# kcoost/fast_speech_enhancement_metrics

Measured on NVIDIA B200. Metric: PESQ+STOI audio-seconds scored/sec, higher is better.
Workload: dtype f32

## Files before the change

### fast_speech_enhancement_metrics_b200/csrc/fsem_api.cu

```cuda
#include <atomic>
#include <cstdarg>
#include <cstdio>
#include <cstdlib>
#include <cstring>
#include <new>
#include <vector>

#include "fsem_common.cuh"
#include "fsem_pesq.cuh"
#include "fsem_stoi.cuh"
#include "fsem_lsd.cuh"
#include "fsem_sdr.cuh"
#include "fsem_sdr_tc.cuh"
#include "fsem_ingest.cuh"

using namespace fsem;

namespace {

thread_local char g_err[512] = "";
std::atomic<int64_t> g_launches{0};

int fail(int code, const char* fmt, ...) {
    va_list ap;
// ... 161 lines not shown

extern "C" int fsem_version(void) { return FSEM_VERSION; }
extern "C" const char* fsem_last_error(void) { return g_err; }
extern "C" int64_t fsem_launch_count(void) { return g_launches.load(std::memory_order_relaxed); }
extern "C" int fsem_profile_enable(int on) { g_profile = on != 0; return FSEM_OK; }
extern "C" int fsem_profile_reset(void) {
    prof_collect();
    for (int i = 0; i < K_COUNT; ++i) { g_prof_ms[i] = 0; g_prof_launches[i] = 0; }
    return FSEM_OK;
}
extern "C" int fsem_profile_read(int index, const char** name, double* total_ms, int64_t* launches) {
    if (index < 0 || index >= K_COUNT) return FSEM_E_INVALID;
    prof_collect();
    if (name) *name = kKernelNames[index];
    if (total_ms) *total_ms = g_prof_ms[index];
    if (launches) *launches = g_prof_launches[index];
    return FSEM_OK;
}

struct fsem_pesq_ctx {
    DeviceInfo dev;
    PesqFilterCoef coef;
    int warm = 640;
    PesqTables* d_tab = nullptr;
    int rs_orig = 1, rs_neu = 1, rs_width = 0, rs_ntaps = 0;
    float* d_rs_taps = nullptr;
    int spec_ctas_per_sm = 2;
    int filt_ctas_per_sm = 4;
    int64_t plan_batch_hint = 0;
    HostPipe pipe;
};

namespace {

struct PesqPlan {
    int64_t batch, n, zstride;
    int64_t n_in, rstride;
    bool resample;
    bool tiled;
    int tmax, tpitch, chunk, nchunks;
    size_t off_rs, off_rslen, off_z, off_partial, off_bark, off_dist, off_power, off_order, off_fprefix, total;
};

PesqPlan pesq_plan(const fsem_pesq_ctx* ctx, int64_t batch, int64_t n_in) {
    constexpr int quantum = 64;
    PesqPlan p{};
    p.batch = batch;
    p.n_in = n_in;
    p.resample = ctx->rs_orig != ctx->rs_neu;
    const int64_t n = stoi_resampled_len(n_in, ctx->rs_orig, ctx->rs_neu);
    p.rstride = round_up(n > 0 ? n : 1, 4);
    p.n = n;
    p.zstride = round_up((n > 0 ? n : 1) + FSEM_PESQ_HOP, 4);
    p.tmax = pesq_num_frames(n);
    if (p.tmax < 1) p.tmax = 1;
    p.tpitch = (int)round_up(p.tmax, 4);
    const int64_t nn = n > 0 ? n : 1;
    const int64_t plan_batch = ctx->plan_batch_hint > 0 ? ctx->plan_batch_hint : batch;
    const int64_t groups = 2 * ceil_div(plan_batch > 0 ? plan_batch : 1, 32);
    const int64_t slots = (int64_t)ctx->dev.sms * ctx->filt_ctas_per_sm * kFiltWarps;
    const int64_t max_ch = ceil_div(nn, 256) < 1024 ? ceil_div(nn, 256) : 1024;
    int64_t nch = 1, chunk = round_up(nn, quantum);
    double best = 1e300;
    p.tiled = plan_batch >= 16;
    if (!p.tiled) {
        chunk = round_up(ceil_div(nn, max_ch), 64);
        nch = ceil_div(nn, chunk);
    }
    for (int64_t c = 1; p.tiled && c <= max_ch; ++c) {
        const int64_t ch = round_up(ceil_div(nn, c), quantum);
        const int64_t cc = ceil_div(nn, ch);
        const int64_t waves = ceil_div(groups * cc, slots);
        const double cost = (double)waves * (double)(ch + (cc > 1 ? ctx->warm : 0));
        if (cost < best * 0.999) { best = cost; nch = cc; chunk = ch; }
    }
    p.chunk = (int)chunk;
    p.nchunks = (int)nch;
    size_t off = 0;
    p.off_rs = off;      off = align256(off + (p.resample ? sizeof(float) * 2 * batch * p.rstride : 0));
    p.off_rslen = off;   off = align256(off + (p.resample ? sizeof(int32_t) * batch : 0));
    p.off_z = off;       off = align256(off + sizeof(float) * 2 * batch * p.zstride);
    p.off_bark = off;    off = align256(off + sizeof(float) * 2 * batch * p.tpitch * kBarkRow);
    p.off_dist = off;    off = align256(off + sizeof(float) * 2 * batch * p.tpitch);
    p.off_power = off;   off = align256(off + sizeof(double) * 2 * batch);
    p.off_order = off;   off = align256(off + sizeof(int32_t) * batch);
    p.off_fprefix = off; off = align256(off + sizeof(int64_t) * (batch + 1));
    p.off_partial = off; off = align256(off + sizeof(double) * 2 * batch * p.nchunks);
    p.total = off;
    return p;
}

}

extern "C" int fsem_pesq_create(fsem_pesq_ctx_t** out, const fsem_pesq_design_t* d) {
    if (!out || !d) return fail(FSEM_E_INVALID, "fsem_pesq_create: null argument");
    *out = nullptr;
    fsem_pesq_ctx* ctx = new (std::nothrow) fsem_pesq_ctx();
    if (!ctx) return fail(FSEM_E_INVALID, "out of host memory");
    int rc = query_device(ctx->dev);
    if (rc != FSEM_OK) { delete ctx; return rc; }
    ctx->coef.k = d->bp_direct;
    for (int s = 0; s < FSEM_BP_SECTIONS; ++s) {
        ctx->coef.c0[s] = d->bp_c0[s]; ctx->coef.c1[s] = d->bp_c1[s];
        ctx->coef.a1[s] = d->bp_a1[s]; ctx->coef.a2[s] = d->bp_a2[s];
    }
    ctx->coef.pb0 = d->pre_b[0]; ctx->coef.pb1 = d->pre_b[1]; ctx->coef.pb2 = d->pre_b[2];
    ctx->coef.pa1 = d->pre_a[0]; ctx->coef.pa2 = d->pre_a[1];
    ctx->warm = (int)round_up(d->warmup > 0 ? d->warmup : 640, 32);
    for (int k = 0; k < 15; ++k) {
        if (fabsf(d->taper[k] - (float)(k + 1) * 0.0625f) > 1e-7f) {
            delete ctx;
            return fail(FSEM_E_INVALID, "fsem_pesq_create: taper must be k/16 (PESQ.py:90)");
        }
    }
    PesqTables h{};
    memcpy(h.hann, d->hann, sizeof(h.hann));
    double wtot = 0.0;
    for (int b = 0; b < FSEM_PESQ_NBANDS; ++b) {
        h.band_first[b] = d->band_first_bin[b];
        h.band_count[b] = d->band_num_bins[b];
        const int expect_first = b == 0 ? 0 : h.band_first[b - 1] + h.band_count[b - 1];
        if (h.band_first[b] != expect_first || h.band_count[b] < 1 || h.band_count[b] > 32 ||
            h.band_first[b] + h.band_count[b] > 256) {
            delete ctx;
            return fail(FSEM_E_INVALID, "fsem_pesq_create: Bark bands must tile bins 0..255 contiguously, at most 32 bins each (band %d)", b);
        }
        {
            const int span = ((h.band_first[b] + h.band_count[b] - 1) >> 3) - (h.band_first[b] >> 3);
            if (span > (b < 32 ? kBarkPiecesLow : kBarkPiecesHigh)) {
                delete ctx;
                return fail(FSEM_E_INVALID, "fsem_pesq_create: Bark band %d spans %d groups of 8 bins (unsupported layout)", b, span + 1);
            }
        }
        h.pow_dens[b] = d->pow_dens[b];
        h.thresh[b] = d->thresh[b];
        h.zw_exp[b] = d->zwicker_exp[b];
        h.width[b] = d->width_bark[b];
        h.loud_scale[b] = (float)((double)d->sl * pow(2.0 * (double)d->thresh[b], (double)d->zwicker_exp[b]));
        if (b >= 1) wtot += (double)d->width_bark[b];
    }
    h.width_total = (float)wtot;
    cudaError_t e = cudaMalloc(&ctx->d_tab, sizeof(PesqTables));
    if (e == cudaSuccess) e = cudaMemcpy(ctx->d_tab, &h, sizeof(h), cudaMemcpyHostToDevice);
    if (e != cudaSuccess) {
        if (ctx->d_tab) cudaFree(ctx->d_tab);
        delete ctx;
        return fail(FSEM_E_CUDA, "fsem_pesq_create: %s", cudaGetErrorString(e));
    }
    if (e == cudaSuccess && d->rs_orig != d->rs_neu) {
        if (d->rs_orig <= 0 || d->rs_neu <= 0 || !d->rs_taps || d->rs_ntaps != 2 * d->rs_width + d->rs_orig) {
            cudaFree(ctx->d_tab);
            delete ctx;
            return fail(FSEM_E_INVALID, "fsem_pesq_create: bad resampling kernel (ntaps must be 2*width+orig)");
        }
        ctx->rs_orig = d->rs_orig; ctx->rs_neu = d->rs_neu; ctx->rs_width = d->rs_width; ctx->rs_ntaps = d->rs_ntaps;
        e = cudaMalloc(&ctx->d_rs_taps, sizeof(float) * d->rs_neu * d->rs_ntaps);
        if (e == cudaSuccess)
            e = cudaMemcpy(ctx->d_rs_taps, d->rs_taps, sizeof(float) * d->rs_neu * d->rs_ntaps, cudaMemcpyHostToDevice);
        if (e != cudaSuccess) {
            cudaFree(ctx->d_tab);
            if (ctx->d_rs_taps) cudaFree(ctx->d_rs_taps);
            delete ctx;
            return fail(FSEM_E_CUDA, "fsem_pesq_create: %s", cudaGetErrorString(e));
        }
    }
    e = cudaFuncSetAttribute(pesq_spectrum_kernel, cudaFuncAttributeMaxDynamicSharedMemorySize, (int)kSpecDynSmem);
    if (e == cudaSuccess)
        e = cudaFuncSetAttribute(pesq_bark_kernel<kBarkThreadsWide, kBarkTileWide>,
                                 cudaFuncAttributeMaxDynamicSharedMemorySize, (int)bark_dyn_smem(kBarkTileWide));
    if (e == cudaSuccess && bark_dyn_smem(kBarkTile) > 0)
        e = cudaFuncSetAttribute(pesq_bark_kernel<kBarkThreads, kBarkTile>,
                                 cudaFuncAttributeMaxDynamicSharedMemorySize, (int)bark_dyn_smem(kBarkTile));
    if (e != cudaSuccess) {
        cudaFree(ctx->d_tab);
        if (ctx->d_rs_taps) cudaFree(ctx->d_rs_taps);
        delete ctx;
        return fail(FSEM_E_CUDA, "fsem_pesq_create: %s", cudaGetErrorString(e));
    }
    int occ = 0;
    if (cudaOccupancyMaxActiveBlocksPerMultiprocessor(&occ, pesq_spectrum_kernel, kSpecWarps * 32, kSpecDynSmem) == cudaSuccess && occ > 0)
        ctx->spec_ctas_per_sm = occ;
    occ = 0;
    if (cudaOccupancyMaxActiveBlocksPerMultiprocessor(&occ, pesq_filter_tiled_kernel<false, float>, kFiltWarps * 32, 0) == cudaSuccess && occ > 0)
        ctx->filt_ctas_per_sm = occ;
    *out = ctx;
    return FSEM_OK;
}

extern "C" int fsem_pesq_destroy(fsem_pesq_ctx_t* ctx) {
    if (!ctx) return FSEM_OK;
    ctx->pipe.destroy();
    if (ctx->d_tab) cudaFree(ctx->d_tab);
    if (ctx->d_rs_taps) cudaFree(ctx->d_rs_taps);
    delete ctx;
    return FSEM_OK;
}

extern "C" size_t fsem_pesq_workspace_bytes(const fsem_pesq_ctx_t* ctx, int64_t batch, int64_t n) {
    if (!ctx || batch <= 0 || n <= 0) return 0;
    return pesq_plan(ctx, batch, n).total;
}

extern "C" int fsem_pesq_score_f32(fsem_pesq_ctx_t* ctx, const fsem_batch_t* in, float* mos_out,
                                   int32_t* status_out, void* workspace, size_t workspace_bytes,
                                   void* stream_v) {
    return fsem_pesq_score(ctx, in, FSEM_DTYPE_F32, mos_out, status_out, workspace, workspace_bytes, stream_v);
}

extern "C" int fsem_pesq_score(fsem_pesq_ctx_t* ctx, const fsem_batch_t* in, int dtype, float* mos_out,
                               int32_t* status_out, void* workspace, size_t workspace_bytes, void* stream_v) {
    if (!ctx || !in || !mos_out) return fail(FSEM_E_INVALID, "fsem_pesq_score_f32: null argument");
    const size_t es = dtype_size(dtype);
    if (es == 0) return fail(FSEM_E_INVALID, "fsem_pesq_score: unknown dtype %d", dtype);
    if (in->batch < 0 || in->n < 0 || in->stride < in->n)
        return fail(FSEM_E_INVALID, "fsem_pesq_score_f32: bad shape batch=%lld n=%lld stride=%lld",
                    (long long)in->batch, (long long)in->n, (long long)in->stride);
    if (in->batch == 0) return FSEM_OK;
    if (!in->clean || !in->deg) return fail(FSEM_E_INVALID, "fsem_pesq_score_f32: null input");
    if (in->n >= (int64_t(1) << 30)) return fail(FSEM_E_INVALID, "fsem_pesq_score_f32: n too large");
    const PesqPlan p = pesq_plan(ctx, in->batch, in->n);
    if (!in->lengths && pesq_num_frames(p.n) < 20)
        return fail(FSEM_E_TOO_SHORT, "PESQ needs at least 20 frames of 512/256 samples at 16 kHz; n=%lld gives %d",
                    (long long)in->n, pesq_num_frames(p.n));
    if (!workspace || workspace_bytes < p.total)
        return fail(FSEM_E_WORKSPACE, "fsem_pesq_score_f32: workspace %zu < %zu bytes", workspace_bytes, p.total);
    cudaStream_t stream = static_cast<cudaStream_t>(stream_v);
    char* ws = static_cast<char*>(workspace);
    float* z = reinterpret_cast<float*>(ws + p.off_z);
    double* partial = reinterpret_cast<double*>(ws + p.off_partial);
    float* bark = reinterpret_cast<float*>(ws + p.off_bark);
    float* dist = reinterpret_cast<float*>(ws + p.off_dist);
    double* power = reinterpret_cast<double*>(ws + p.off_power);

    fsem_batch_t rs_batch;
    if (p.resample) {
        float* y = reinterpret_cast<float*>(ws + p.off_rs);
        int32_t* rslen = reinterpret_cast<int32_t*>(ws + p.off_rslen);
        const int64_t bps = ceil_div(p.n, 256);
        if (bps * 2 * in->batch >= (int64_t(1) << 31))
            return fail(FSEM_E_INVALID, "fsem_pesq_score_f32: batch x samples too large for one launch; split the batch");
        { ProfScope prof_(K_PESQ_RESAMPLE, stream);
          dispatch_dtype(dtype, [&](auto tag) {
              using T = decltype(tag);
              stoi_resample_kernel<T><<<(unsigned)(bps * 2 * in->batch), 256, 0, stream>>>(
                  reinterpret_cast<const T*>(in->clean), reinterpret_cast<const T*>(in->deg), in->lengths, in->batch, in->n,
                  in->stride, ctx->d_rs_taps, ctx->rs_orig, ctx->rs_neu, ctx->rs_width, ctx->rs_ntaps, y, p.rstride, (int)bps);
              return FSEM_OK;
          }); }
        FSEM_LAUNCHED();
        if (in->lengths) {
            resampled_lengths_kernel<<<(unsigned)ceil_div(in->batch, 256), 256, 0, stream>>>(
                in->lengths, in->batch, in->n, ctx->rs_orig, ctx->rs_neu, rslen);
            FSEM_LAUNCHED();
        }
        rs_batch = fsem_batch_t{y, y + in->batch * p.rstride, in->lengths ? rslen : nullptr, in->batch, p.n, p.rstride};
        in = &rs_batch;
        dtype = FSEM_DTYPE_F32;
    }

    int32_t* order = nullptr;
    int64_t* fprefix = nullptr;
    if (in->lengths) {
        order = reinterpret_cast<int32_t*>(ws + p.off_order);
        fprefix = reinterpret_cast<int64_t*>(ws + p.off_fprefix);
        pesq_order_kernel<<<1, kOrderThreads, 0, stream>>>(in->lengths, in->batch, in->n, order, fprefix);
        FSEM_LAUNCHED();
    }
    {
        const bool vec4 = rows_vec4(in->clean, in->deg, in->stride, dtype_size(dtype));
        ProfScope prof_(K_PESQ_FILTER, stream);
        dispatch_dtype(dtype, [&](auto tag) {
            using T = decltype(tag);
            const T* c = reinterpret_cast<const T*>(in->clean);
            const T* d = reinterpret_cast<const T*>(in->deg);
            if (vec4 && p.tiled) {
                const int64_t units = 2 * ceil_div(in->batch, 32) * p.nchunks;
                const unsigned grid = (unsigned)ceil_div(units, kFiltWarps);
                if (in->lengths)
                    pesq_filter_tiled_kernel<true, T><<<grid, kFiltWarps * 32, 0, stream>>>(
                        c, d, in->lengths, order, in->batch, in->n, in->stride, p.chunk, p.nchunks, ctx->warm, ctx->coef, z,
                        p.zstride, partial);
                else
                    pesq_filter_tiled_kernel<false, T><<<grid, kFiltWarps * 32, 0, stream>>>(
                        c, d, nullptr, nullptr, in->batch, in->n, in->stride, p.chunk, p.nchunks, ctx->warm, ctx->coef, z,
                        p.zstride, partial);
            } else {
                const int64_t threads = 2 * in->batch * p.nchunks;
                const unsigned grid = (unsigned)ceil_div(threads, 128);
                if (vec4)
                    pesq_filter_kernel<true, T><<<grid, 128, 0, stream>>>(
                        c, d, in->lengths, in->batch, in->n, in->stride, p.chunk, p.nchunks, ctx->warm, ctx->coef, z,
                        p.zstride, partial);
                else
                    pesq_filter_kernel<false, T><<<grid, 128, 0, stream>>>(
                        c, d, in->lengths, in->batch, in->n, in->stride, p.chunk, p.nchunks, ctx->warm, ctx->coef, z,
                        p.zstride, partial);
            }
            return FSEM_OK;
        });
    }
    FSEM_LAUNCHED();
    {
        const int64_t units = in->batch * (int64_t)p.tmax;
        int64_t grid = ceil_div(units, kSpecWarps);
        const int64_t cap = (int64_t)ctx->dev.sms * ctx->spec_ctas_per_sm;
        if (grid > cap) grid = cap;
        { ProfScope prof_(K_PESQ_SPECTRUM, stream);
          pesq_spectrum_kernel<<<(unsigned)grid, kSpecWarps * 32, kSpecDynSmem, stream>>>(
              z, p.zstride, in->lengths, fprefix, in->batch, in->n, p.tmax, p.tpitch, partial, p.nchunks, ctx->d_tab, bark); }
        FSEM_LAUNCHED();
    }
    {
        { ProfScope prof_(K_PESQ_BARK, stream);
          if (in->batch <= ctx->dev.sms)
              pesq_bark_kernel<kBarkThreadsWide, kBarkTileWide>
                  <<<(unsigned)in->batch, kBarkThreadsWide, bark_dyn_smem(kBarkTileWide), stream>>>(
                      bark, partial, p.nchunks, in->lengths, order, in->batch, in->n, p.tpitch, ctx->d_tab, dist, mos_out,
                      status_out, power);
          else
              pesq_bark_kernel<kBarkThreads, kBarkTile>
                  <<<(unsigned)in->batch, kBarkThreads, bark_dyn_smem(kBarkTile), stream>>>(
                      bark, partial, p.nchunks, in->lengths, order, in->batch, in->n, p.tpitch, ctx->d_tab, dist, mos_out,
                      status_out, power); }
        FSEM_LAUNCHED();
    }
    return FSEM_OK;
}

extern "C" int fsem_pesq_debug_taps(fsem_pesq_ctx_t* ctx, int64_t batch, int64_t n, const void* workspace,
                                    float* bark_out, double* power_out, int64_t* frames_out, void* stream_v) {
    if (!ctx || !workspace) return fail(FSEM_E_INVALID, "fsem_pesq_debug_taps: null argument");
    const PesqPlan p = pesq_plan(ctx, batch, n);
    cudaStream_t stream = static_cast<cudaStream_t>(stream_v);
    const char* ws = static_cast<const char*>(workspace);
    if (frames_out) *frames_out = p.tmax;
    if (bark_out)
        for (int64_t r = 0; r < 2 * batch; ++r)
            FSEM_CUDA(cudaMemcpy2DAsync(bark_out + r * p.tmax * FSEM_PESQ_NBANDS, sizeof(float) * FSEM_PESQ_NBANDS,
                                        ws + p.off_bark + sizeof(float) * r * p.tpitch * kBarkRow, sizeof(float) * kBarkRow,
                                        sizeof(float) * FSEM_PESQ_NBANDS, (size_t)p.tmax, cudaMemcpyDeviceToDevice, stream));
    if (power_out)
        FSEM_CUDA(cudaMemcpyAsync(power_out, ws + p.off_power, sizeof(double) * 2 * batch, cudaMemcpyDeviceToDevice,
                                  stream));
    return FSEM_OK;
}

struct fsem_stoi_ctx {
    DeviceInfo dev;
    int orig = 1, neu = 1, width = 0, ntaps = 0;
    float* d_taps = nullptr;
    bool fast85 = false;
    Resample85Taps taps85;
    StoiTables* d_tab = nullptr;
    float clip = 0.f, dyn_range = 40.f;
    int tob_ctas_per_sm = 2;
    HostPipe pipe;
};

namespace {

struct StoiPlan {
    int64_t batch, n, lmax, ystride;
    int t0max, mask_words, umax, ustride, mmax, ntiles, hops_max;
    bool resample, fused_energy;
    size_t off_hops, off_y, off_energy, off_idx, off_count, off_prefix, off_mask, off_tob, off_partial, total;
};

StoiPlan stoi_plan(const fsem_stoi_ctx* ctx, int64_t batch, int64_t n) {
    StoiPlan p{};
    p.batch = batch;
    p.n = n;
    p.resample = ctx->orig != ctx->neu;
    p.lmax = stoi_resampled_len(n, ctx->orig, ctx->neu);
    p.ystride = round_up(p.lmax > 0 ? p.lmax : 1, 4);
    p.t0max = stoi_num_frames(p.lmax);
    if (p.t0max < 1) p.t0max = 1;
    p.mask_words = (int)ceil_div(p.t0max, 32);
    p.umax = p.t0max - 2 > 0 ? p.t0max - 2 : 0;
    p.ustride = (int)round_up(p.umax > 0 ? p.umax : 1, 4);
    p.mmax = p.t0max - 31 > 0 ? p.t0max - 31 : 0;
    p.ntiles = (int)ceil_div(p.mmax > 0 ? p.mmax : 1, kSegTile);
    p.fused_energy = ctx->fast85;
    p.hops_max = (int)(ceil_div(p.lmax > 0 ? p.lmax : 1, kRs85TileOut) * kRs85Hops);
    size_t off = 0;
    p.off_hops = off;    off = align256(off + (p.fused_energy ? sizeof(double2) * batch * p.hops_max : 0));
    p.off_y = off;       off = align256(off + sizeof(float) * 2 * batch * p.ystride);
    p.off_energy = off;  off = align256(off + sizeof(float) * batch * p.t0max);
    p.off_idx = off;     off = align256(off + sizeof(int32_t) * batch * p.t0max);
    p.off_count = off;   off = align256(off + sizeof(int32_t) * batch);
    p.off_prefix = off;  off = align256(off + sizeof(int32_t) * (batch + 1));
    p.off_mask = off;    off = align256(off + sizeof(uint32_t) * batch * p.mask_words);
    p.off_tob = off;     off = align256(off + sizeof(float) * 2 * batch * FSEM_STOI_NBANDS * p.ustride);
    p.off_partial = off; off = align256(off + sizeof(float2) * batch * p.ntiles);
    p.total = off;
    return p;
}

}

extern "C" int fsem_stoi_create(fsem_stoi_ctx_t** out, const fsem_stoi_design_t* d) {
    if (!out || !d) return fail(FSEM_E_INVALID, "fsem_stoi_create: null argument");
    *out = nullptr;
    if (d->orig <= 0 || d->neu <= 0) return fail(FSEM_E_INVALID, "fsem_stoi_create: bad rates");
    if (d->orig != d->neu && (!d->taps || d->ntaps != 2 * d->width + d->orig || d->width < 0))
        return fail(FSEM_E_INVALID, "fsem_stoi_create: bad resampling kernel (ntaps must be 2*width+orig)");
    for (int b = 0; b < FSEM_STOI_NBANDS; ++b)
        if (d->band_lo[b] < 0 || d->band_hi[b] < d->band_lo[b] || d->band_hi[b] > 256)
            return fail(FSEM_E_INVALID, "fsem_stoi_create: band %d outside bins 0..255", b);
    if (d->band_hi[FSEM_STOI_NBANDS - 1] - d->band_lo[FSEM_STOI_NBANDS - 1] > 48)
        return fail(FSEM_E_INVALID, "fsem_stoi_create: third-octave bands must be at most 48 bins wide");
    for (int b = 0; b + 1 < FSEM_STOI_NBANDS; ++b)
        if (d->band_hi[b] != d->band_lo[b + 1] || d->band_hi[b] - d->band_lo[b] > 48)
            return fail(FSEM_E_INVALID, "fsem_stoi_create: third-octave bands must be contiguous and at most 48 bins wide");
    fsem_stoi_ctx* ctx = new (std::nothrow) fsem_stoi_ctx();
    if (!ctx) return fail(FSEM_E_INVALID, "out of host memory");
    int rc = query_device(ctx->dev);
    if (rc != FSEM_OK) { delete ctx; return rc; }
    ctx->orig = d->orig; ctx->neu = d->neu; ctx->width = d->width; ctx->ntaps = d->ntaps;
    ctx->clip = d->clip; ctx->dyn_range = d->dyn_range;
    StoiTables h{};
    memcpy(h.window, d->window, sizeof(h.window));
    for (int b = 0; b < FSEM_STOI_NBANDS; ++b) { h.band_lo[b] = d->band_lo[b]; h.band_hi[b] = d->band_hi[b]; }
    h.clip = d->clip; h.dyn_range = d->dyn_range;
    cudaError_t e = cudaMalloc(&ctx->d_tab, sizeof(StoiTables));
    if (e == cudaSuccess) e = cudaMemcpy(ctx->d_tab, &h, sizeof(h), cudaMemcpyHostToDevice);
    if (e == cudaSuccess && d->orig != d->neu) {
        e = cudaMalloc(&ctx->d_taps, sizeof(float) * d->neu * d->ntaps);
        if (e == cudaSuccess)
            e = cudaMemcpy(ctx->d_taps, d->taps, sizeof(float) * d->neu * d->ntaps, cudaMemcpyHostToDevice);
    }
    if (e != cudaSuccess) {
        if (ctx->d_tab) cudaFree(ctx->d_tab);
        if (ctx->d_taps) cudaFree(ctx->d_taps);
        delete ctx;
        return fail(FSEM_E_CUDA, "fsem_stoi_create: %s", cudaGetErrorString(e));
    }
    if (d->orig == 8 && d->neu == 5 && d->width == 10 && d->ntaps == 28) {
        ctx->fast85 = true;
        for (int p = 0; p < 5; ++p)
            for (int j = 0; j < 28; ++j) {
                ctx->taps85.h[p][j] = d->taps[p * 28 + j];
                if ((j < rs85_lo(p) || j > rs85_hi(p)) && d->taps[p * 28 + j] != 0.f) ctx->fast85 = false;
            }
    }
    int occ = 0;
    if (cudaOccupancyMaxActiveBlocksPerMultiprocessor(&occ, stoi_tob_kernel<true>, kTobWarps * 32, 0) == cudaSuccess && occ > 0)
        ctx->tob_ctas_per_sm = occ;
    *out = ctx;
    return FSEM_OK;
}

extern "C" int fsem_stoi_destroy(fsem_stoi_ctx_t* ctx) {
    if (!ctx) return FSEM_OK;
    ctx->pipe.destroy();
    if (ctx->d_tab) cudaFree(ctx->d_tab);
    if (ctx->d_taps) cudaFree(ctx->d_taps);
    delete ctx;
    return FSEM_OK;
}

extern "C" size_t fsem_stoi_workspace_bytes(const fsem_stoi_ctx_t* ctx, int64_t batch, int64_t n) {
    if (!ctx || batch <= 0 || n <= 0) return 0;
    return stoi_plan(ctx, batch, n).total;
}

extern "C" int fsem_stoi_score_f32(fsem_stoi_ctx_t* ctx, const fsem_batch_t* in, float* stoi_out,
                                   float* estoi_out, int32_t* kept_frames_out, int32_t* status_out,
                                   void* workspace, size_t workspace_bytes, void* stream_v) {
    return fsem_stoi_score(ctx, in, FSEM_DTYPE_F32, stoi_out, estoi_out, kept_frames_out, status_out, workspace,
                           workspace_bytes, stream_v);
}

extern "C" int fsem_stoi_score(fsem_stoi_ctx_t* ctx, const fsem_batch_t* in, int dtype, float* stoi_out,
                               float* estoi_out, int32_t* kept_frames_out, int32_t* status_out,
                               void* workspace, size_t workspace_bytes, void* stream_v) {
    if (!ctx || !in || !stoi_out || !estoi_out) return fail(FSEM_E_INVALID, "fsem_stoi_score_f32: null argument");
    if (dtype_size(dtype) == 0) return fail(FSEM_E_INVALID, "fsem_stoi_score: unknown dtype %d", dtype);
    if (in->batch < 0 || in->n < 0 || in->stride < in->n)
        return fail(FSEM_E_INVALID, "fsem_stoi_score_f32: bad shape batch=%lld n=%lld stride=%lld",
                    (long long)in->batch, (long long)in->n, (long long)in->stride);
    if (in->batch == 0) return FSEM_OK;
    if (in->n == 0) return fail(FSEM_E_INVALID, "fsem_stoi_score_f32: n = 0 (empty signals)");
    if (!in->clean || !in->deg) return fail(FSEM_E_INVALID, "fsem_stoi_score_f32: null input");
    if (in->n >= (int64_t(1) << 30)) return fail(FSEM_E_INVALID, "fsem_stoi_score_f32: n too large");
    const StoiPlan p = stoi_plan(ctx, in->batch, in->n);
    if (in->batch * (int64_t)p.t0max >= (int64_t(1) << 31))
        return fail(FSEM_E_INVALID, "fsem_stoi_score_f32: batch x frames exceeds 2^31; split the batch");
    if (!workspace || workspace_bytes < p.total)
        return fail(FSEM_E_WORKSPACE, "fsem_stoi_score_f32: workspace %zu < %zu bytes", workspace_bytes, p.total);
    cudaStream_t stream = static_cast<cudaStream_t>(stream_v);
    char* ws = static_cast<char*>(workspace);
    float* y = reinterpret_cast<float*>(ws + p.off_y);
    double2* hops = reinterpret_cast<double2*>(ws + p.off_hops);
    float* energy = reinterpret_cast<float*>(ws + p.off_energy);
    int32_t* kept_idx = reinterpret_cast<int32_t*>(ws + p.off_idx);
    int32_t* kept_count = reinterpret_cast<int32_t*>(ws + p.off_count);
    int32_t* frame_prefix = reinterpret_cast<int32_t*>(ws + p.off_prefix);
    uint32_t* mask = reinterpret_cast<uint32_t*>(ws + p.off_mask);
    float* tob = reinterpret_cast<float*>(ws + p.off_tob);
    float2* partial = reinterpret_cast<float2*>(ws + p.off_partial);

    const float* c10 = in->clean;
    const float* d10 = in->deg;
    int64_t sstride = in->stride;
    if (p.resample) {
        const bool vec4 = rows_vec4(in->clean, in->deg, in->stride, dtype_size(dtype));
        if (ctx->fast85) {
            const int64_t bps = ceil_div(p.lmax, (int64_t)kRs85TileOut * kRs85TilesPerCta);
            const unsigned grid = (unsigned)(bps * 2 * in->batch);
            { ProfScope prof_(K_STOI_RESAMPLE, stream);
              dispatch_dtype(dtype, [&](auto tag) {
                  using T = decltype(tag);
                  const T* c = reinterpret_cast<const T*>(in->clean);
                  const T* d = reinterpret_cast<const T*>(in->deg);
                  if (vec4)
                      stoi_resample85_kernel<true, T><<<grid, kRs85Threads, 0, stream>>>(
                          c, d, in->lengths, in->batch, in->n, in->stride, ctx->taps85, ctx->d_tab, y, p.ystride, hops,
                          p.hops_max, (int)bps);
                  else
                      stoi_resample85_kernel<false, T><<<grid, kRs85Threads, 0, stream>>>(
                          c, d, in->lengths, in->batch, in->n, in->stride, ctx->taps85, ctx->d_tab, y, p.ystride, hops,
                          p.hops_max, (int)bps);
                  return FSEM_OK;
              }); }
        } else {
            const int64_t bps = ceil_div(p.lmax, 256);
            if (bps * 2 * in->batch >= (int64_t(1) << 31))
                return fail(FSEM_E_INVALID, "fsem_stoi_score_f32: batch x samples too large for one launch; split the batch");
            { ProfScope prof_(K_STOI_RESAMPLE, stream);
              dispatch_dtype(dtype, [&](auto tag) {
                  using T = decltype(tag);
                  stoi_resample_kernel<T><<<(unsigned)(bps * 2 * in->batch), 256, 0, stream>>>(
                      reinterpret_cast<const T*>(in->clean), reinterpret_cast<const T*>(in->deg), in->lengths, in->batch,
                      in->n, in->stride, ctx->d_taps, ctx->orig, ctx->neu, ctx->width, ctx->ntaps, y, p.ystride, (int)bps);
                  return FSEM_OK;
              }); }
        }
        FSEM_LAUNCHED();
        c10 = y;
        d10 = y + in->batch * p.ystride;
        sstride = p.ystride;
    } else if (dtype != FSEM_DTYPE_F32) {
        int rc = launch_ingest(in->clean, dtype, in->batch, in->n, in->stride, y, p.ystride, stream);
        if (rc == FSEM_OK)
            rc = launch_ingest(in->deg, dtype, in->batch, in->n, in->stride, y + in->batch * p.ystride, p.ystride, stream);
        if (rc != FSEM_OK) return rc;
        c10 = y;
        d10 = y + in->batch * p.ystride;
        sstride = p.ystride;
    }
    if (p.fused_energy) {
        const int64_t threads = in->batch * (int64_t)p.t0max;
        { ProfScope prof_(K_STOI_ENERGY, stream);
          stoi_energy_from_hops_kernel<<<(unsigned)ceil_div(threads, 256), 256, 0, stream>>>(
              hops, p.hops_max, in->lengths, in->batch, in->n, p.t0max, energy); }
        FSEM_LAUNCHED();
    } else {
        const int64_t warps = in->batch * (int64_t)p.t0max;
        { ProfScope prof_(K_STOI_ENERGY, stream);
          stoi_energy_kernel<<<(unsigned)ceil_div(warps * 32, 256), 256, 0, stream>>>(
            c10, sstride, in->lengths, in->batch, in->n, ctx->orig, ctx->neu, p.t0max, ctx->d_tab, energy); }
        FSEM_LAUNCHED();
    }
    {
        { ProfScope prof_(K_STOI_COMPACT, stream);
          stoi_compact_kernel<<<(unsigned)ceil_div(in->batch * 32, 128), 128, 0, stream>>>(
              energy, in->lengths, in->batch, in->n, ctx->orig, ctx->neu, p.t0max, p.mask_words, ctx->dyn_range,
              kept_idx, kept_count, mask); }
        FSEM_LAUNCHED();
    }
    if (p.umax > 0) {
        { ProfScope prof_(K_STOI_COMPACT, stream);
          stoi_prefix_kernel<<<1, 1024, 0, stream>>>(kept_count, in->batch, frame_prefix); }
        FSEM_LAUNCHED();
        const int64_t units = in->batch * (int64_t)p.umax;
        int64_t grid = ceil_div(units, kTobWarps);
        const int64_t cap = (int64_t)ctx->dev.sms * ctx->tob_ctas_per_sm;
        if (grid > cap) grid = cap;
        const bool vec2 = (reinterpret_cast<uintptr_t>(c10) & 7u) == 0 && (reinterpret_cast<uintptr_t>(d10) & 7u) == 0 &&
                          sstride % 2 == 0;
        { ProfScope prof_(K_STOI_TOB, stream);
          if (vec2)
              stoi_tob_kernel<true><<<(unsigned)grid, kTobWarps * 32, 0, stream>>>(
                  c10, d10, sstride, in->batch, p.t0max, p.umax, p.ustride, kept_idx, frame_prefix, ctx->d_tab, tob);
          else
              stoi_tob_kernel<false><<<(unsigned)grid, kTobWarps * 32, 0, stream>>>(
                  c10, d10, sstride, in->batch, p.t0max, p.umax, p.ustride, kept_idx, frame_prefix, ctx->d_tab, tob); }
        FSEM_LAUNCHED();
    }
    {
        { ProfScope prof_(K_STOI_SEGMENT, stream);
          stoi_segment_kernel<<<(unsigned)(in->batch * ceil_div(p.ntiles, kSegTilesPerCta)), kSegThreads, 0, stream>>>(
              tob, in->batch, p.ustride, p.ntiles, kept_count, ctx->clip, partial); }
        FSEM_LAUNCHED();
        { ProfScope prof_(K_STOI_FINALIZE, stream);
          stoi_finalize_kernel<<<(unsigned)ceil_div(in->batch, 128), 128, 0, stream>>>(
              partial, in->batch, p.ntiles, kept_count, stoi_out, estoi_out, kept_frames_out, status_out); }
        FSEM_LAUNCHED();
    }
    return FSEM_OK;
}

extern "C" int fsem_stoi_debug_taps(fsem_stoi_ctx_t* ctx, int64_t batch, int64_t n, const void* workspace,
                                    uint32_t* mask_out, float* tob_out, float* resampled_out, int64_t* dims_out,
                                    void* stream_v) {
    if (!ctx || !workspace) return fail(FSEM_E_INVALID, "fsem_stoi_debug_taps: null argument");
    const StoiPlan p = stoi_plan(ctx, batch, n);
    cudaStream_t stream = static_cast<cudaStream_t>(stream_v);
    const char* ws = static_cast<const char*>(workspace);
    if (dims_out) {
        dims_out[0] = p.mask_words;
        dims_out[1] = p.ustride;
        dims_out[2] = p.resample ? p.ystride : 0;
    }
    if (mask_out)
        FSEM_CUDA(cudaMemcpyAsync(mask_out, ws + p.off_mask, sizeof(uint32_t) * batch * p.mask_words,
                                  cudaMemcpyDeviceToDevice, stream));
    if (tob_out)
        FSEM_CUDA(cudaMemcpyAsync(tob_out, ws + p.off_tob, sizeof(float) * 2 * batch * FSEM_STOI_NBANDS * p.ustride,
                                  cudaMemcpyDeviceToDevice, stream));
    if (resampled_out && p.resample)
        FSEM_CUDA(cudaMemcpyAsync(resampled_out, ws + p.off_y, sizeof(float) * 2 * batch * p.ystride,
                                  cudaMemcpyDeviceToDevice, stream));
    return FSEM_OK;
}

extern "C" int fsem_stoi_mask_margin(fsem_stoi_ctx_t* ctx, int64_t batch, int64_t n, const int32_t* lengths,
                                     const void* workspace, float* margin_out, void* stream_v) {
    if (!ctx || !workspace || !margin_out) return fail(FSEM_E_INVALID, "fsem_stoi_mask_margin: null argument");
    if (batch <= 0 || n <= 0) return fail(FSEM_E_INVALID, "fsem_stoi_mask_margin: bad shape");
    const StoiPlan p = stoi_plan(ctx, batch, n);
    cudaStream_t stream = static_cast<cudaStream_t>(stream_v);
    const float* energy = reinterpret_cast<const float*>(static_cast<const char*>(workspace) + p.off_energy);
    { ProfScope prof_(K_STOI_MARGIN, stream);
      stoi_margin_kernel<<<(unsigned)ceil_div(batch * 32, 128), 128, 0, stream>>>(
          energy, lengths, batch, n, ctx->orig, ctx->neu, p.t0max, ctx->dyn_range, margin_out); }
    FSEM_LAUNCHED();
    return FSEM_OK;
}

namespace {

int launch_ingest(const void* src, int dtype, int64_t rows, int64_t n, int64_t sstride, float* dst, int64_t dstride,
                  cudaStream_t stream) {
    if (rows <= 0 || n <= 0) return FSEM_OK;
    if (dtype == FSEM_DTYPE_F32) {
        FSEM_CUDA(cudaMemcpy2DAsync(dst, dstride * sizeof(float), src, sstride * sizeof(float), n * sizeof(float), rows,
                                    cudaMemcpyDeviceToDevice, stream));
        return FSEM_OK;
    }
    const bool vec = aligned16(src) && aligned16(dst) && sstride % 8 == 0 && dstride % 4 == 0;
    const int64_t groups = rows * ceil_div(n, 8);
    int64_t grid = ceil_div(groups, 256);
    if (grid > (1 << 20)) grid = 1 << 20;
    { ProfScope prof_(K_INGEST, stream);
      if (dtype == FSEM_DTYPE_I16) {
          const int16_t* s = static_cast<const int16_t*>(src);
          if (vec) ingest_kernel<int16_t, true><<<(unsigned)grid, 256, 0, stream>>>(s, sstride, dst, dstride, rows, n);
          else ingest_kernel<int16_t, false><<<(unsigned)grid, 256, 0, stream>>>(s, sstride, dst, dstride, rows, n);
      } else {
          const __half* s = static_cast<const __half*>(src);
          if (vec) ingest_kernel<__half, true><<<(unsigned)grid, 256, 0, stream>>>(s, sstride, dst, dstride, rows, n);
          else ingest_kernel<__half, false><<<(unsigned)grid, 256, 0, stream>>>(s, sstride, dst, dstride, rows, n);
      } }
    FSEM_LAUNCHED();
    return FSEM_OK;
}

int score_host_any(const char* who, fsem_pesq_ctx* pctx, fsem_stoi_ctx* sctx, const void* clean, const void* deg,
                   int dtype, const int32_t* lengths, int64_t batch, int64_t n, int64_t stride, float* mos_out,
                   int32_t* pesq_status_out, float* stoi_out, float* estoi_out, int32_t* kept_frames_out,
                   int32_t* stoi_status_out) {
    if ((!pctx && !sctx) || !clean || !deg || (pctx && !mos_out) || (sctx && (!stoi_out || !estoi_out)))
        return fail(FSEM_E_INVALID, "%s: null argument", who);
    const size_t es = dtype_size(dtype);
    if (es == 0) return fail(FSEM_E_INVALID, "%s: unknown dtype %d", who, dtype);
    if (batch < 0 || n < 0 || stride < n) return fail(FSEM_E_INVALID, "%s: bad shape", who);
    if (batch == 0) return FSEM_OK;
    if (pctx && !lengths && pesq_num_frames(pesq_plan(pctx, 1, n).n) < 20)
        return fail(FSEM_E_TOO_SHORT, "PESQ needs at least 20 frames of 512/256 samples at 16 kHz; n=%lld is too short",
                    (long long)n);
    HostPipe& P = pctx ? pctx->pipe : sctx->pipe;
    int rc = P.init();
    if (rc != FSEM_OK) return rc;
    const int64_t rstride = round_up(n, 16 / (int64_t)es);
    const int64_t per = host_chunk_items(batch, n, es);
    const size_t raw_sig = align256(es * per * rstride);
    const size_t in_bytes = 2 * raw_sig + align256(sizeof(int32_t) * per);
    const size_t conv_sig = 0;
    const size_t ws_pesq = pctx ? align256(fsem_pesq_workspace_bytes(pctx, per, n)) : 0;
    const size_t ws_stoi = sctx ? align256(fsem_stoi_workspace_bytes(sctx, per, n)) : 0;
    const size_t col = align256(sizeof(float) * batch);
    rc = P.reserve(in_bytes, 2 * conv_sig + ws_pesq + ws_stoi, 6 * col);
    if (rc != FSEM_OK) return rc;
    char* const ob = static_cast<char*>(P.out);
    char* const wsb = static_cast<char*>(P.ws);
    const char* h_clean = static_cast<const char*>(clean);
    const char* h_deg = static_cast<const char*>(deg);
    auto upload = [&](void* dst, const char* src, int64_t cnt) -> cudaError_t {
        if (stride == n && rstride == n)
            return cudaMemcpyAsync(dst, src, es * n * cnt, cudaMemcpyHostToDevice, P.copy);
        return cudaMemcpy2DAsync(dst, rstride * es, src, stride * es, n * es, cnt, cudaMemcpyHostToDevice, P.copy);
    };
    auto run = [&]() -> int {
    int64_t done_chunks = 0;
    for (int64_t i0 = 0; i0 < batch; i0 += per, ++done_chunks) {
        const int slot = (int)(done_chunks & 1);
        const int64_t cnt = (batch - i0 < per) ? (batch - i0) : per;
        char* base = static_cast<char*>(P.in[slot]);
        int32_t* d_len = reinterpret_cast<int32_t*>(base + 2 * raw_sig);
        if (done_chunks >= 2) FSEM_CUDA(cudaStreamWaitEvent(P.copy, P.done[slot], 0));
        FSEM_CUDA(upload(base, h_clean + (size_t)i0 * stride * es, cnt));
        FSEM_CUDA(upload(base + raw_sig, h_deg + (size_t)i0 * stride * es, cnt));
        if (lengths)
            FSEM_CUDA(cudaMemcpyAsync(d_len, lengths + i0, sizeof(int32_t) * cnt, cudaMemcpyHostToDevice, P.copy));
        FSEM_CUDA(cudaEventRecord(P.copied[slot], P.copy));
        FSEM_CUDA(cudaStreamWaitEvent(P.compute, P.copied[slot], 0));
        fsem_batch_t dev{reinterpret_cast<const float*>(base), reinterpret_cast<const float*>(base + raw_sig),
                         lengths ? d_len : nullptr, cnt, n, rstride};
        if (rc == FSEM_OK && pctx && sctx)
            rc = fsem_pesq_stoi_score(pctx, sctx, &dev, dtype, reinterpret_cast<float*>(ob) + i0,
                                          reinterpret_cast<int32_t*>(ob + col) + i0,
                                          reinterpret_cast<float*>(ob + 2 * col) + i0,
                                          reinterpret_cast<float*>(ob + 3 * col) + i0,
                                          reinterpret_cast<int32_t*>(ob + 4 * col) + i0,
                                          reinterpret_cast<int32_t*>(ob + 5 * col) + i0, wsb + 2 * conv_sig, ws_pesq,
                                          wsb + 2 * conv_sig + ws_pesq, ws_stoi, P.compute);
        else if (rc == FSEM_OK && pctx)
            rc = fsem_pesq_score(pctx, &dev, dtype, reinterpret_cast<float*>(ob) + i0,
                                 reinterpret_cast<int32_t*>(ob + col) + i0, wsb + 2 * conv_sig, ws_pesq, P.compute);
        else if (rc == FSEM_OK && sctx)
            rc = fsem_stoi_score(sctx, &dev, dtype, reinterpret_cast<float*>(ob + 2 * col) + i0,
                                     reinterpret_cast<float*>(ob + 3 * col) + i0,
                                     reinterpret_cast<int32_t*>(ob + 4 * col) + i0,
                                     reinterpret_cast<int32_t*>(ob + 5 * col) + i0, wsb + 2 * conv_sig + ws_pesq, ws_stoi,
                                     P.compute);
        if (rc != FSEM_OK) return rc;
        FSEM_CUDA(cudaEventRecord(P.done[slot], P.compute));
    }
    const size_t nb = sizeof(float) * batch;
    auto readback = [&](void* dst, size_t column) -> cudaError_t {
        return dst ? cudaMemcpyAsync(dst, ob + column * col, nb, cudaMemcpyDeviceToHost, P.compute) : cudaSuccess;
    };
    if (pctx) {
        FSEM_CUDA(readback(mos_out, 0));
        FSEM_CUDA(readback(pesq_status_out, 1));
    }
    if (sctx) {
        FSEM_CUDA(readback(stoi_out, 2));
        FSEM_CUDA(readback(estoi_out, 3));
        FSEM_CUDA(readback(kept_frames_out, 4));
        FSEM_CUDA(readback(stoi_status_out, 5));
    }
    return FSEM_OK;
    };
    rc = run();
    const cudaError_t e_copy = cudaStreamSynchronize(P.copy);
    const cudaError_t e_comp = cudaStreamSynchronize(P.compute);
    if (rc != FSEM_OK) return rc;
    if (e_copy != cudaSuccess || e_comp != cudaSuccess)
        return fail(FSEM_E_CUDA, "%s: %s", who, cudaGetErrorString(e_copy != cudaSuccess ? e_copy : e_comp));
    return FSEM_OK;
}

}

extern "C" int fsem_ingest_f32(const void* src, int dtype, int64_t rows, int64_t n, int64_t src_stride, float* dst,
                               int64_t dst_stride, void* stream) {
    if (!src || !dst) return fail(FSEM_E_INVALID, "fsem_ingest_f32: null argument");
    if (dtype_size(dtype) == 0) return fail(FSEM_E_INVALID, "fsem_ingest_f32: unknown dtype %d", dtype);
    if (rows < 0 || n < 0 || src_stride < n || dst_stride < n) return fail(FSEM_E_INVALID, "fsem_ingest_f32: bad shape");
    return launch_ingest(src, dtype, rows, n, src_stride, dst, dst_stride, static_cast<cudaStream_t>(stream));
}

extern "C" int fsem_score_host(fsem_pesq_ctx_t* pesq, fsem_stoi_ctx_t* stoi, const void* clean, const void* deg, int dtype,
                               const int32_t* lengths, int64_t batch, int64_t n, int64_t stride, float* mos_out,
                               int32_t* pesq_status_out, float* stoi_out, float* estoi_out, int32_t* kept_frames_out,
                               int32_t* stoi_status_out) {
    return score_host_any("fsem_score_host", pesq, stoi, clean, deg, dtype, lengths, batch, n, stride, mos_out,
                          pesq_status_out, stoi_out, estoi_out, kept_frames_out, stoi_status_out);
}

extern "C" int fsem_pesq_score_host_f32(fsem_pesq_ctx_t* ctx, const fsem_batch_t* in, float* mos_out,
                                        int32_t* status_out) {
    if (!ctx || !in) return fail(FSEM_E_INVALID, "fsem_pesq_score_host_f32: null argument");
    return score_host_any("fsem_pesq_score_host_f32", ctx, nullptr, in->clean, in->deg, FSEM_DTYPE_F32, in->lengths,
                          in->batch, in->n, in->stride, mos_out, status_out, nullptr, nullptr, nullptr, nullptr);
}

extern "C" int fsem_stoi_score_host_f32(fsem_stoi_ctx_t* ctx, const fsem_batch_t* in, float* stoi_out,
                                        float* estoi_out, int32_t* kept_frames_out, int32_t* status_out) {
    if (!ctx || !in) return fail(FSEM_E_INVALID, "fsem_stoi_score_host_f32: null argument");
    return score_host_any("fsem_stoi_score_host_f32", nullptr, ctx, in->clean, in->deg, FSEM_DTYPE_F32, in->lengths,
                          in->batch, in->n, in->stride, nullptr, nullptr, stoi_out, estoi_out, kept_frames_out,
                          status_out);
}

extern "C" int fsem_pesq_stoi_score_host_f32(fsem_pesq_ctx_t* pctx, fsem_stoi_ctx_t* sctx, const fsem_batch_t* in,
                                             float* mos_out, int32_t* pesq_status_out, float* stoi_out,
                                             float* estoi_out, int32_t* kept_frames_out, int32_t* stoi_status_out) {
    if (!pctx || !sctx || !in) return fail(FSEM_E_INVALID, "fsem_pesq_stoi_score_host_f32: null argument");
    return score_host_any("fsem_pesq_stoi_score_host_f32", pctx, sctx, in->clean, in->deg, FSEM_DTYPE_F32, in->lengths,
                          in->batch, in->n, in->stride, mos_out, pesq_status_out, stoi_out, estoi_out, kept_frames_out,
                          stoi_status_out);
}

struct fsem_resampler {
    int orig = 1, neu = 1, width = 0, ntaps = 0;
    float* d_taps = nullptr;
};

extern "C" int fsem_resampler_create(fsem_resampler_t** out, int32_t orig, int32_t neu, int32_t width, int32_t ntaps,
                                     const float* taps) {
    if (!out) return fail(FSEM_E_INVALID, "fsem_resampler_create: null argument");
    *out = nullptr;
    if (orig <= 0 || neu <= 0 || width < 0 || !taps || ntaps != 2 * width + orig)
        return fail(FSEM_E_INVALID, "fsem_resampler_create: bad resampling kernel (ntaps must be 2*width+orig)");
    fsem_resampler* r = new (std::nothrow) fsem_resampler();
    if (!r) return fail(FSEM_E_INVALID, "out of host memory");
    r->orig = orig; r->neu = neu; r->width = width; r->ntaps = ntaps;
    cudaError_t e = cudaMalloc(&r->d_taps, sizeof(float) * neu * ntaps);
    if (e == cudaSuccess) e = cudaMemcpy(r->d_taps, taps, sizeof(float) * neu * ntaps, cudaMemcpyHostToDevice);
    if (e != cudaSuccess) {
        if (r->d_taps) cudaFree(r->d_taps);
        delete r;
        return fail(FSEM_E_CUDA, "fsem_resampler_create: %s", cudaGetErrorString(e));
    }
    *out = r;
    return FSEM_OK;
}

extern "C" int fsem_resampler_destroy(fsem_resampler_t* r) {
    if (!r) return FSEM_OK;
    if (r->d_taps) cudaFree(r->d_taps);
    delete r;
    return FSEM_OK;
}

extern "C" int64_t fsem_resampled_len(const fsem_resampler_t* r, int64_t n) {
    if (!r || n < 0) return 0;
    return stoi_resampled_len(n, r->orig, r->neu);
}

extern "C" int fsem_resample_f32(fsem_resampler_t* r, const fsem_batch_t* in, float* out, int64_t out_stride,
                                 int32_t* lengths_out, void* stream_v) {
    if (!r || !in || !out) return fail(FSEM_E_INVALID, "fsem_resample_f32: null argument");
    if (in->batch < 0 || in->n <= 0 || in->stride < in->n || in->n >= (int64_t(1) << 30))
        return fail(FSEM_E_INVALID, "fsem_resample_f32: bad shape");
    if (in->batch == 0) return FSEM_OK;
    if (!in->clean || !in->deg) return fail(FSEM_E_INVALID, "fsem_resample_f32: null input");
    const int64_t L = stoi_resampled_len(in->n, r->orig, r->neu);
    if (out_stride < L) return fail(FSEM_E_INVALID, "fsem_resample_f32: out_stride %lld < resampled length %lld",
                                    (long long)out_stride, (long long)L);
    if (in->lengths && !lengths_out) return fail(FSEM_E_INVALID, "fsem_resample_f32: lengths given but lengths_out is null");
    cudaStream_t stream = static_cast<cudaStream_t>(stream_v);
    const int64_t bps = ceil_div(L, 256);
    if (bps * 2 * in->batch >= (int64_t(1) << 31))
        return fail(FSEM_E_INVALID, "fsem_resample_f32: batch x samples too large for one launch; split the batch");
    { ProfScope prof_(K_PESQ_RESAMPLE, stream);
      stoi_resample_kernel<<<(unsigned)(bps * 2 * in->batch), 256, 0, stream>>>(
          in->clean, in->deg, in->lengths, in->batch, in->n, in->stride, r->d_taps, r->orig, r->neu, r->width,
          r->ntaps, out, out_stride, (int)bps); }
    FSEM_LAUNCHED();
    if (in->lengths) {
        resampled_lengths_kernel<<<(unsigned)ceil_div(in->batch, 256), 256, 0, stream>>>(
            in->lengths, in->batch, in->n, r->orig, r->neu, lengths_out);
        FSEM_LAUNCHED();
    }
    return FSEM_OK;
}

struct fsem_lsd_ctx {
    DeviceInfo dev;
    float* d_hann = nullptr;
    int ctas_per_sm = 2;
};

namespace {
struct LsdPlan { int tmax; size_t off_alpha, off_frames, total; };
LsdPlan lsd_plan(int64_t batch, int64_t n) {
    LsdPlan p{};
    p.tmax = lsd_num_frames(n);
    size_t off = 0;
    p.off_alpha = off;  off = align256(off + sizeof(float) * batch);
    p.off_frames = off; off = align256(off + sizeof(float) * batch * p.tmax);
    p.total = off;
    return p;
}
}

extern "C" int fsem_lsd_create(fsem_lsd_ctx_t** out, const float* hann512) {
    if (!out || !hann512) return fail(FSEM_E_INVALID, "fsem_lsd_create: null argument");
    *out = nullptr;
    fsem_lsd_ctx* ctx = new (std::nothrow) fsem_lsd_ctx();
    if (!ctx) return fail(FSEM_E_INVALID, "out of host memory");
    int rc = query_device(ctx->dev);
    if (rc != FSEM_OK) { delete ctx; return rc; }
    cudaError_t e = cudaMalloc(&ctx->d_hann, sizeof(float) * 512);
    if (e == cudaSuccess) e = cudaMemcpy(ctx->d_hann, hann512, sizeof(float) * 512, cudaMemcpyHostToDevice);
    if (e != cudaSuccess) {
        if (ctx->d_hann) cudaFree(ctx->d_hann);
        delete ctx;
        return fail(FSEM_E_CUDA, "fsem_lsd_create: %s", cudaGetErrorString(e));
    }
    int occ = 0;
    if (cudaOccupancyMaxActiveBlocksPerMultiprocessor(&occ, lsd_frames_kernel<true>, kLsdWarps * 32, 0) == cudaSuccess && occ > 0)
        ctx->ctas_per_sm = occ;
    *out = ctx;
    return FSEM_OK;
}

extern "C" int fsem_lsd_destroy(fsem_lsd_ctx_t* ctx) {
    if (!ctx) return FSEM_OK;
    if (ctx->d_hann) cudaFree(ctx->d_hann);
    delete ctx;
    return FSEM_OK;
}

extern "C" size_t fsem_lsd_workspace_bytes(const fsem_lsd_ctx_t* ctx, int64_t batch, int64_t n) {
    if (!ctx || batch <= 0 || n <= 0) return 0;
    return lsd_plan(batch, n).total;
}

extern "C" int fsem_lsd_score_f32(fsem_lsd_ctx_t* ctx, const fsem_batch_t* in, float* lsd_out, void* workspace,
                                  size_t workspace_bytes, void* stream_v) {
    if (!ctx || !in || !lsd_out) return fail(FSEM_E_INVALID, "fsem_lsd_score_f32: null argument");
    if (in->batch < 0 || in->n <= 0 || in->stride < in->n || in->n >= (int64_t(1) << 30))
        return fail(FSEM_E_INVALID, "fsem_lsd_score_f32: bad shape");
    if (in->batch == 0) return FSEM_OK;
    if (!in->clean || !in->deg) return fail(FSEM_E_INVALID, "fsem_lsd_score_f32: null input");
    const LsdPlan p = lsd_plan(in->batch, in->n);
    if (!workspace || workspace_bytes < p.total)
        return fail(FSEM_E_WORKSPACE, "fsem_lsd_score_f32: workspace %zu < %zu bytes", workspace_bytes, p.total);
    cudaStream_t stream = static_cast<cudaStream_t>(stream_v);
    char* ws = static_cast<char*>(workspace);
    float* alpha = reinterpret_cast<float*>(ws + p.off_alpha);
    float* frames = reinterpret_cast<float*>(ws + p.off_frames);
    lsd_scale_kernel<<<(unsigned)in->batch, 256, 0, stream>>>(in->clean, in->deg, in->lengths, in->batch, in->n,
                                                             in->stride, alpha);
    FSEM_LAUNCHED();
    const int64_t units = in->batch * (int64_t)p.tmax;
    int64_t grid = ceil_div(units, kLsdWarps);
    const int64_t cap = (int64_t)ctx->dev.sms * ctx->ctas_per_sm;
    if (grid > cap) grid = cap;
    const bool vec2 = (reinterpret_cast<uintptr_t>(in->clean) & 7u) == 0 && (reinterpret_cast<uintptr_t>(in->deg) & 7u) == 0 &&
                      in->stride % 2 == 0;
    { ProfScope prof_(K_LSD_FRAMES, stream);
      if (vec2)
          lsd_frames_kernel<true><<<(unsigned)grid, kLsdWarps * 32, 0, stream>>>(
              in->clean, in->deg, in->lengths, in->batch, in->n, in->stride, p.tmax, ctx->d_hann, alpha, frames);
      else
          lsd_frames_kernel<false><<<(unsigned)grid, kLsdWarps * 32, 0, stream>>>(
              in->clean, in->deg, in->lengths, in->batch, in->n, in->stride, p.tmax, ctx->d_hann, alpha, frames); }
    FSEM_LAUNCHED();
    lsd_finalize_kernel<<<(unsigned)ceil_div(in->batch, 128), 128, 0, stream>>>(frames, in->lengths, in->batch, in->n,
                                                                               p.tmax, lsd_out);
    FSEM_LAUNCHED();
    return FSEM_OK;
}

extern "C" int fsem_pesq_stoi_score(fsem_pesq_ctx_t* pctx, fsem_stoi_ctx_t* sctx, const fsem_batch_t* in, int dtype,
                                    float* mos_out, int32_t* pesq_status_out, float* stoi_out, float* estoi_out,
                                    int32_t* kept_frames_out, int32_t* stoi_status_out, void* ws_pesq,
                                    size_t ws_pesq_bytes, void* ws_stoi, size_t ws_stoi_bytes, void* stream) {
    if (!pctx || !sctx) return fail(FSEM_E_INVALID, "fsem_pesq_stoi_score: null context");
    int rc = fsem_pesq_score(pctx, in, dtype, mos_out, pesq_status_out, ws_pesq, ws_pesq_bytes, stream);
    if (rc == FSEM_OK)
        rc = fsem_stoi_score(sctx, in, dtype, stoi_out, estoi_out, kept_frames_out, stoi_status_out, ws_stoi,
                             ws_stoi_bytes, stream);
    return rc;
}

extern "C" int fsem_pesq_stoi_score_f32(fsem_pesq_ctx_t* pctx, fsem_stoi_ctx_t* sctx, const fsem_batch_t* in,
                                        float* mos_out, int32_t* pesq_status_out, float* stoi_out, float* estoi_out,
                                        int32_t* kept_frames_out, int32_t* stoi_status_out, void* ws_pesq,
                                        size_t ws_pesq_bytes, void* ws_stoi, size_t ws_stoi_bytes, void* stream) {
    return fsem_pesq_stoi_score(pctx, sctx, in, FSEM_DTYPE_F32, mos_out, pesq_status_out, stoi_out, estoi_out,
                                kept_frames_out, stoi_status_out, ws_pesq, ws_pesq_bytes, ws_stoi, ws_stoi_bytes, stream);
}

struct fsem_graph {
    cudaGraph_t graph = nullptr;
    cudaGraphExec_t exec = nullptr;
    void* ws = nullptr;
    int kernel_nodes = 0;
    int slices = 0;
    int device = -1;
};

namespace {
void graph_free(fsem_graph* g) {
    if (!g) return;
    if (g->exec) cudaGraphExecDestroy(g->exec);
    if (g->graph) cudaGraphDestroy(g->graph);
    if (g->ws) cudaFree(g->ws);
    delete g;
}
constexpr int kGraphMaxSlices = 16;
}

extern "C" int fsem_graph_create(fsem_graph_t** out, fsem_pesq_ctx_t* pctx, fsem_stoi_ctx_t* sctx, const fsem_batch_t* in,
                                 int dtype, float* mos_out, int32_t* pesq_status_out, float* stoi_out, float* estoi_out,
                                 int32_t* kept_frames_out, int32_t* stoi_status_out, int slices) {
    if (!out) return fail(FSEM_E_INVALID, "fsem_graph_create: null output");
    *out = nullptr;
    if (!pctx && !sctx) return fail(FSEM_E_INVALID, "fsem_graph_create: no metric selected");
    if (!in || in->batch <= 0) return fail(FSEM_E_INVALID, "fsem_graph_create: empty batch");
    if ((pctx && !mos_out) || (sctx && (!stoi_out || !estoi_out)))
        return fail(FSEM_E_INVALID, "fsem_graph_create: null output column");
    const size_t es = dtype_size(dtype);
    if (es == 0) return fail(FSEM_E_INVALID, "fsem_graph_create: unknown dtype %d", dtype);
    if (slices <= 0) slices = 1;
    if (slices > kGraphMaxSlices) slices = kGraphMaxSlices;
    if (slices > in->batch) slices = (int)in->batch;
    fsem_graph* g = new (std::nothrow) fsem_graph();
    if (!g) return fail(FSEM_E_INVALID, "fsem_graph_create: out of host memory");
    g->slices = slices;
    int64_t b0[kGraphMaxSlices + 1];
    for (int s = 0; s <= slices; ++s) b0[s] = in->batch * s / slices;
    if (pctx) pctx->plan_batch_hint = in->batch;
    size_t ws_off[2 * kGraphMaxSlices + 1];
    ws_off[0] = 0;
    for (int s = 0; s < slices; ++s) {
        const int64_t nb = b0[s + 1] - b0[s];
        ws_off[2 * s + 1] = ws_off[2 * s] + (pctx ? align256(fsem_pesq_workspace_bytes(pctx, nb, in->n)) : 0);
        ws_off[2 * s + 2] = ws_off[2 * s + 1] + (sctx ? align256(fsem_stoi_workspace_bytes(sctx, nb, in->n)) : 0);
    }
    const int nbranch = (pctx ? slices : 0) + (sctx ? slices : 0);
    cudaStream_t main_s = nullptr;
    std::vector<cudaStream_t> side(nbranch > 1 ? nbranch - 1 : 0, nullptr);
    std::vector<cudaEvent_t> join(side.size(), nullptr);
    cudaEvent_t fork_e = nullptr;
    int rc = FSEM_OK;
    cudaError_t e = cudaGetDevice(&g->device);
    if (e == cudaSuccess) e = cudaMalloc(&g->ws, ws_off[2 * slices] > 0 ? ws_off[2 * slices] : 256);
    if (e == cudaSuccess) e = cudaStreamCreateWithFlags(&main_s, cudaStreamNonBlocking);
    for (size_t i = 0; i < side.size() && e == cudaSuccess; ++i) {
        e = cudaStreamCreateWithFlags(&side[i], cudaStreamNonBlocking);
        if (e == cudaSuccess) e = cudaEventCreateWithFlags(&join[i], cudaEventDisableTiming);
    }
    if (e == cudaSuccess) e = cudaEventCreateWithFlags(&fork_e, cudaEventDisableTiming);
    const bool profile_was = g_profile;
    g_profile = false;
    const int64_t launches_before = g_launches.load(std::memory_order_relaxed);
    bool capturing = false;
    if (e == cudaSuccess) {
        e = cudaStreamBeginCapture(main_s, cudaStreamCaptureModeThreadLocal);
        capturing = (e == cudaSuccess);
    }
    if (capturing) {
        if (!side.empty()) e = cudaEventRecord(fork_e, main_s);
        for (size_t i = 0; i < side.size() && e == cudaSuccess; ++i) e = cudaStreamWaitEvent(side[i], fork_e, 0);
        int k = 0;
        auto stream_of = [&](int idx) { return idx == 0 ? main_s : side[idx - 1]; };
        const char* cb = reinterpret_cast<const char*>(in->clean);
        const char* db = reinterpret_cast<const char*>(in->deg);
        char* wsb = static_cast<char*>(g->ws);
        for (int pass = 0; pass < 2 && e == cudaSuccess && rc == FSEM_OK; ++pass) {
            if ((pass == 0 && !pctx) || (pass == 1 && !sctx)) continue;
            for (int s = 0; s < slices && rc == FSEM_OK; ++s, ++k) {
                const int64_t i0 = b0[s], nb = b0[s + 1] - b0[s];
                const fsem_batch_t sub{reinterpret_cast<const float*>(cb + (size_t)i0 * in->stride * es),
                                       reinterpret_cast<const float*>(db + (size_t)i0 * in->stride * es),
                                       in->lengths ? in->lengths + i0 : nullptr, nb, in->n, in->stride};
                if (pass == 0)
                    rc = fsem_pesq_score(pctx, &sub, dtype, mos_out + i0, pesq_status_out ? pesq_status_out + i0 : nullptr,
                                         wsb + ws_off[2 * s], ws_off[2 * s + 1] - ws_off[2 * s], stream_of(k));
                else
                    rc = fsem_stoi_score(sctx, &sub, dtype, stoi_out + i0, estoi_out + i0,
                                         kept_frames_out ? kept_frames_out + i0 : nullptr,
                                         stoi_status_out ? stoi_status_out + i0 : nullptr, wsb + ws_off[2 * s + 1],
                                         ws_off[2 * s + 2] - ws_off[2 * s + 1], stream_of(k));
            }
        }
        for (size_t i = 0; i < side.size(); ++i) {
            cudaError_t j = cudaEventRecord(join[i], side[i]);
            if (j == cudaSuccess) j = cudaStreamWaitEvent(main_s, join[i], 0);
            if (e == cudaSuccess && rc == FSEM_OK) e = j;
        }
        cudaError_t end = cudaStreamEndCapture(main_s, &g->graph);
        if (e == cudaSuccess) e = end;
    }
    if (pctx) pctx->plan_batch_hint = 0;
    g_profile = profile_was;
    if (e == cudaSuccess && rc == FSEM_OK) {
        g->kernel_nodes = (int)(g_launches.load(std::memory_order_relaxed) - launches_before);
        e = cudaGraphInstantiate(&g->exec, g->graph, 0);
    }
    g_launches.store(launches_before, std::memory_order_relaxed);
    if (main_s) cudaStreamDestroy(main_s);
    for (size_t i = 0; i < side.size(); ++i) {
        if (side[i]) cudaStreamDestroy(side[i]);
        if (join[i]) cudaEventDestroy(join[i]);
    }
    if (fork_e) cudaEventDestroy(fork_e);
    if (rc != FSEM_OK) { graph_free(g); cudaGetLastError(); return rc; }
    if (e != cudaSuccess) {
        graph_free(g);
        cudaGetLastError();
        return fail(FSEM_E_CUDA, "fsem_graph_create: %s", cudaGetErrorString(e));
    }
    *out = g;
    return FSEM_OK;
}

extern "C" int fsem_graph_launch(fsem_graph_t* g, void* stream) {
    if (!g || !g->exec) return fail(FSEM_E_INVALID, "fsem_graph_launch: null graph");
    FSEM_CUDA(cudaGraphLaunch(g->exec, static_cast<cudaStream_t>(stream)));
    g_launches.fetch_add(g->kernel_nodes, std::memory_order_relaxed);
    return FSEM_OK;
}

extern "C" int fsem_graph_nodes(const fsem_graph_t* g) { return g ? g->kernel_nodes : 0; }
extern "C" int fsem_graph_slices(const fsem_graph_t* g) { return g ? g->slices : 0; }

extern "C" int fsem_graph_destroy(fsem_graph_t* g) {
    graph_free(g);
    return FSEM_OK;
}

namespace {
typedef CUresult (*TensorMapEncodeFn)(CUtensorMap*, CUtensorMapDataType, cuuint32_t, void*, const cuuint64_t*, const cuuint64_t*,
                                      const cuuint32_t*, const cuuint32_t*, CUtensorMapInterleave, CUtensorMapSwizzle,
                                      CUtensorMapL2promotion, CUtensorMapFloatOOBfill);
TensorMapEncodeFn tensor_map_encoder() {
    static TensorMapEncodeFn fn = [] {
        void* p = nullptr;
        cudaDriverEntryPointQueryResult q;
        if (cudaGetDriverEntryPoint("cuTensorMapEncodeTiled", &p, cudaEnableDefault, &q) != cudaSuccess ||
            q != cudaDriverEntryPointSuccess)
            p = nullptr;
        return reinterpret_cast<TensorMapEncodeFn>(p);
    }();
    return fn;
}
bool make_sdr_tensor_map(CUtensorMap* map, const float* base, int64_t batch, int64_t n, int64_t stride, int box0) {
    TensorMapEncodeFn enc = tensor_map_encoder();
    if (!enc) return false;
    const int64_t rows = (n - kTcMapDim0) / kTcM + 1;
    if (rows < kTcK) return false;
    const cuuint64_t gdim[3] = {(cuuint64_t)kTcMapDim0, (cuuint64_t)rows, (cuuint64_t)batch};
    const cuuint64_t gstride[2] = {(cuuint64_t)kTcM * sizeof(float), (cuuint64_t)stride * sizeof(float)};
    const cuuint32_t box[3] = {(cuuint32_t)box0, (cuuint32_t)kTcK, 1u};
    const cuuint32_t estr[3] = {1u, 1u, 1u};
    return enc(map, CU_TENSOR_MAP_DATA_TYPE_FLOAT32, 3, const_cast<float*>(base), gdim, gstride, box, estr,
               CU_TENSOR_MAP_INTERLEAVE_NONE, CU_TENSOR_MAP_SWIZZLE_NONE, CU_TENSOR_MAP_L2_PROMOTION_L2_128B,
               CU_TENSOR_MAP_FLOAT_OOB_FILL_NONE) == CUDA_SUCCESS;
}
}

namespace {
struct SdrPlan { int nsuper; size_t off_energy, off_partial, total; };
SdrPlan sdr_plan(int64_t batch, int64_t n) {
    SdrPlan p{};
    p.nsuper = (int)ceil_div(n > 0 ? n : 1, (int64_t)kSdrSuper * kSdrTile);
    size_t off = 0;
    p.off_energy = off;  off = align256(off + sizeof(double) * 2 * batch);
    p.off_partial = off; off = align256(off + sizeof(double) * batch * p.nsuper * 2 * kSdrLags);
    p.total = off;
    return p;
}
}

extern "C" size_t fsem_sdr_workspace_bytes(int64_t batch, int64_t n) {
    if (batch <= 0 || n <= 0) return 0;
    return sdr_plan(batch, n).total;
}

extern "C" int fsem_sdr_score_f32(const fsem_batch_t* in, float* sdr_out, void* workspace, size_t workspace_bytes,
                                  void* stream_v) {
    if (!in || !sdr_out) return fail(FSEM_E_INVALID, "fsem_sdr_score_f32: null argument");
    if (in->batch < 0 || in->n <= 0 || in->stride < in->n || in->n >= (int64_t(1) << 30))
        return fail(FSEM_E_INVALID, "fsem_sdr_score_f32: bad shape");
    if (in->batch == 0) return FSEM_OK;
    if (!in->clean || !in->deg) return fail(FSEM_E_INVALID, "fsem_sdr_score_f32: null input");
    if (in->batch > 65535) return fail(FSEM_E_INVALID, "fsem_sdr_score_f32: batch > 65535; split the batch");
    const SdrPlan p = sdr_plan(in->batch, in->n);
    if (!workspace || workspace_bytes < p.total)
        return fail(FSEM_E_WORKSPACE, "fsem_sdr_score_f32: workspace %zu < %zu bytes", workspace_bytes, p.total);
    cudaStream_t stream = static_cast<cudaStream_t>(stream_v);
    char* ws = static_cast<char*>(workspace);
    double* energy = reinterpret_cast<double*>(ws + p.off_energy);
    double* partial = reinterpret_cast<double*>(ws + p.off_partial);
    sdr_norm_kernel<<<(unsigned)(2 * in->batch), 256, 0, stream>>>(in->clean, in->deg, in->lengths, in->batch, in->n,
                                                                  in->stride, energy);
    FSEM_LAUNCHED();
    static const bool simt = [] { const char* e = getenv("FSEM_SDR_SIMT"); return e && e[0] == '1'; }();
    int nsuper = p.nsuper;
    if (simt) {
        ProfScope prof_(K_SDR_CORR, stream);
        sdr_corr_kernel<<<dim3((unsigned)p.nsuper, (unsigned)in->batch), kSdrThreads, 0, stream>>>(
            in->clean, in->deg, in->lengths, in->batch, in->n, in->stride, p.nsuper, partial);
    } else {
        FSEM_CUDA(cudaFuncSetAttribute(sdr_corr_tc_kernel, cudaFuncAttributeMaxDynamicSharedMemorySize, (int)kTcDynSmem));
        CUtensorMap map_a{}, map_bc{}, map_bd{};
        static const bool no_tma = [] { const char* e = getenv("FSEM_SDR_NO_TMA"); return e && e[0] == '1'; }();
        int use_tma = !no_tma && rows_vec4(in->clean, in->deg, in->stride, sizeof(float)) && in->n >= kTcMapDim0 ? 1 : 0;
        if (use_tma) {
            use_tma = make_sdr_tensor_map(&map_a, in->clean, in->batch, in->n, in->stride, kTcBoxA) &&
                      make_sdr_tensor_map(&map_bc, in->clean, in->batch, in->n, in->stride, kTcBoxB) &&
                      make_sdr_tensor_map(&map_bd, in->deg, in->batch, in->n, in->stride, kTcBoxB) ? 1 : 0;
        }
        nsuper = 1;
        ProfScope prof_(K_SDR_CORR, stream);
        sdr_corr_tc_kernel<<<(unsigned)(4 * in->batch), kTcThreads, kTcDynSmem, stream>>>(
            in->clean, in->deg, in->lengths, in->batch, in->n, in->stride, use_tma, map_a, map_bc, map_bd, partial);
    }
    FSEM_LAUNCHED();
    { ProfScope prof_(K_SDR_SOLVE, stream);
      sdr_solve_kernel<<<(unsigned)in->batch, kSdrSolveThreads, 0, stream>>>(partial, nsuper, energy, in->batch, sdr_out); }
    FSEM_LAUNCHED();
    return FSEM_OK;
}
```

### fast_speech_enhancement_metrics_b200/csrc/fsem_fft.cuh

```cuda
#pragma once
#include <cuda_runtime.h>

namespace fsem {

constexpr int kFftN = 512;
constexpr int kFftBufElems = 752;

__device__ __forceinline__ void cmul(float& xr, float& xi, float wr, float wi) {
    float tr = xr * wr - xi * wi;
    xi = xr * wi + xi * wr;
    xr = tr;
}

__device__ __forceinline__ void dft4(float& r0, float& i0, float& r1, float& i1,
                                     float& r2, float& i2, float& r3, float& i3) {
    float c0r = r0 + r2, c0i = i0 + i2;
    float c2r = r0 - r2, c2i = i0 - i2;
    float c1r = r1 + r3, c1i = i1 + i3;
    float c3r = i1 - i3, c3i = r3 - r1;
    r0 = c0r + c1r; i0 = c0i + c1i;
    r2 = c0r - c1r; i2 = c0i - c1i;
    r1 = c2r + c3r; i1 = c2i + c3i;
    r3 = c2r - c3r; i3 = c2i - c3i;
}

template <bool kUpperZero>
__device__ __forceinline__ void dft8(float (&r)[8], float (&i)[8]) {
    constexpr float kH = 0.70710678118654752440f;
    float ar[4], ai[4], br[4], bi[4];
#pragma unroll
    for (int j = 0; j < 4; ++j) {
        if (kUpperZero) {
            ar[j] = r[j]; ai[j] = i[j];
            br[j] = r[j]; bi[j] = i[j];
        } else {
            ar[j] = r[j] + r[j + 4]; ai[j] = i[j] + i[j + 4];
            br[j] = r[j] - r[j + 4]; bi[j] = i[j] - i[j + 4];
        }
    }
    {
        float tr = (br[1] + bi[1]) * kH, ti = (bi[1] - br[1]) * kH;
        br[1] = tr; bi[1] = ti;
        tr = bi[2]; ti = -br[2];
        br[2] = tr; bi[2] = ti;
        tr = (bi[3] - br[3]) * kH; ti = -(br[3] + bi[3]) * kH;
        br[3] = tr; bi[3] = ti;
    }
    dft4(ar[0], ai[0], ar[1], ai[1], ar[2], ai[2], ar[3], ai[3]);
    dft4(br[0], bi[0], br[1], bi[1], br[2], bi[2], br[3], bi[3]);
#pragma unroll
    for (int j = 0; j < 4; ++j) {
        r[2 * j] = ar[j];     i[2 * j] = ai[j];
        r[2 * j + 1] = br[j]; i[2 * j + 1] = bi[j];
    }
}

struct FftTwiddles {
    float w1r[2][7], w1i[2][7];
    float w2r[7], w2i[7];
    __device__ __forceinline__ void init(int lane) {
#pragma unroll
        for (int h = 0; h < 2; ++h) {
            int np = 2 * lane + h;
#pragma unroll
            for (int k0 = 1; k0 < 8; ++k0) {
                float s, c;
                sincospif(-(float)(np * k0) * (1.0f / 256.0f), &s, &c);
                w1r[h][k0 - 1] = c; w1i[h][k0 - 1] = s;
            }
        }
        int n0 = lane & 7;
#pragma unroll
        for (int k1 = 1; k1 < 8; ++k1) {
            float s, c;
            sincospif(-(float)(n0 * k1) * (1.0f / 32.0f), &s, &c);
            w2r[k1 - 1] = c; w2i[k1 - 1] = s;
        }
    }
};

__device__ __forceinline__ int fft_in_index(int lane, int h, int j) { return 2 * lane + h + 64 * j; }

struct FftLaneBins {
    int base_a, base_b;
    __device__ __forceinline__ void init(int lane) {
        const int r = lane & 7, j = lane >> 3;
        if (j >= 1) { base_a = j + 8 * r; base_b = (8 - j) + 8 * (7 - r); }
        else if (r == 0) { base_a = 0; base_b = 32; }
        else if (r < 4) { base_a = 8 * r; base_b = 8 * (8 - r); }
        else { base_a = 4 + 8 * (7 - r); base_b = 4 + 8 * r; }
    }
};

template <bool kUpperZero>
__device__ __forceinline__ void warp_fft512(float (&re)[16], float (&im)[16], float2* buf, const FftTwiddles& tw, int lane,
                                            float (&ar)[8], float (&ai)[8], float (&br)[8], float (&bi)[8]) {
    float4* buf4 = reinterpret_cast<float4*>(buf);
#pragma unroll
    for (int h = 0; h < 2; ++h) {
        float r[8], i[8];
#pragma unroll
        for (int j = 0; j < 8; ++j) { r[j] = re[8 * h + j]; i[j] = im[8 * h + j]; }
        dft8<kUpperZero>(r, i);
#pragma unroll
        for (int k0 = 1; k0 < 8; ++k0) cmul(r[k0], i[k0], tw.w1r[h][k0 - 1], tw.w1i[h][k0 - 1]);
        float4* row = buf4 + 9 * lane + 4 * h;
        row[0] = make_float4(r[0], i[0], r[4], i[4]);
        row[1] = make_float4(r[1], i[1], r[7], i[7]);
        row[2] = make_float4(r[2], i[2], r[6], i[6]);
        row[3] = make_float4(r[3], i[3], r[5], i[5]);
    }
    __syncwarp();
    const int lo3 = lane & 7;
    const int jq = lane >> 3;
    float r2[2][8], i2[2][8];
    {
        const float4* src = buf4 + (lo3 >> 1) * 9 + (lo3 & 1) * 4 + jq;
#pragma unroll
        for (int n1 = 0; n1 < 8; ++n1) {
            const float4 v = src[36 * n1];
            r2[0][n1] = v.x; i2[0][n1] = v.y; r2[1][n1] = v.z; i2[1][n1] = v.w;
        }
    }
    __syncwarp();
#pragma unroll
    for (int s = 0; s < 2; ++s) {
        dft8<false>(r2[s], i2[s]);
#pragma unroll
        for (int k1 = 1; k1 < 8; ++k1) cmul(r2[s][k1], i2[s][k1], tw.w2r[k1 - 1], tw.w2i[k1 - 1]);
    }
    {
        const bool g0 = jq == 0;
        float4* dst = buf4 + jq * 72 + lo3;
        dst[0] = make_float4(r2[0][0], i2[0][0], g0 ? r2[0][4] : r2[1][7], g0 ? i2[0][4] : i2[1][7]);
        dst[9] = make_float4(r2[0][1], i2[0][1], g0 ? r2[0][7] : r2[1][6], g0 ? i2[0][7] : i2[1][6]);
        dst[18] = make_float4(r2[0][2], i2[0][2], g0 ? r2[0][6] : r2[1][5], g0 ? i2[0][6] : i2[1][5]);
        dst[27] = make_float4(r2[0][3], i2[0][3], g0 ? r2[0][5] : r2[1][4], g0 ? i2[0][5] : i2[1][4]);
#pragma unroll
        for (int r = 4; r < 8; ++r)
            dst[9 * r] = make_float4(g0 ? r2[1][7 - r] : r2[0][r], g0 ? i2[1][7 - r] : i2[0][r],
                                     g0 ? r2[1][r] : r2[1][7 - r], g0 ? i2[1][r] : i2[1][7 - r]);
    }
    __syncwarp();
    {
        const float4* src = buf4 + jq * 72 + lo3 * 9;
#pragma unroll
        for (int n0 = 0; n0 < 8; ++n0) {
            const float4 v = src[n0];
            ar[n0] = v.x; ai[n0] = v.y; br[n0] = v.z; bi[n0] = v.w;
        }
    }
    __syncwarp();
    dft8<false>(ar, ai);
    dft8<false>(br, bi);
}

constexpr float kPackedPowerScale = 0.25f;
__device__ __forceinline__ void packed_power_pair(float zr, float zi, float mr, float mi, float& pc, float& pd) {
    float sr = zr + mr, dr = zr - mr;
    float si = zi + mi, di = zi - mi;
    pc = fmaf(sr, sr, di * di);
    pd = fmaf(si, si, dr * dr);
}

__device__ __forceinline__ void packed_power_regs(const float (&ar)[8], const float (&ai)[8], const float (&br)[8],
                                                  const float (&bi)[8], int lane, float (&pc)[8], float (&pd)[8]) {
    const bool l0 = lane == 0;
#pragma unroll
    for (int q = 0; q < 4; ++q) {
        const float mar = l0 ? ar[(8 - q) & 7] : br[7 - q], mai = l0 ? ai[(8 - q) & 7] : bi[7 - q];
        const float mbr = l0 ? br[7 - q] : ar[7 - q],       mbi = l0 ? bi[7 - q] : ai[7 - q];
        packed_power_pair(ar[q], ai[q], mar, mai, pc[q], pd[q]);
        packed_power_pair(br[q], bi[q], mbr, mbi, pc[4 + q], pd[4 + q]);
    }
}

__host__ __device__ constexpr int band_s_index(int k) { return k + 4 * (k >> 5); }
constexpr int kBandSStride = 300;
constexpr int kBandPOffset = 0;
constexpr int kBandSOffset = 2 * kBandSStride;
constexpr int kBandZeroWord = 2 * kBandSStride;
constexpr int kBandBufFloats = kBandSOffset + 3 * kBandSStride + 4;

struct BandScan {
    float keep[8];
    int pa, pb;
    __device__ __forceinline__ void init(const int32_t* starts, int nbands, int lane, const FftLaneBins& bins) {
        unsigned start_mask = 1u;
        for (int b = 0; b < nbands; ++b) {
            const int f = starts[b];
            if ((f >> 3) == lane) start_mask |= 1u << (f & 7);
        }
#pragma unroll
        for (int j = 0; j < 8; ++j) keep[j] = ((start_mask >> j) & 1u) ? 0.f : 1.f;
        pa = band_s_index(bins.base_a);
        pb = band_s_index(bins.base_b);
    }
    __device__ __forceinline__ void scan_store(const float (&pc)[8], const float (&pd)[8], float* w, int lane) const {
        float* Pc = w + kBandPOffset;
        float* Pd = Pc + kBandSStride;
#pragma unroll
        for (int q = 0; q < 4; ++q) {
            Pc[pa + 72 * q] = pc[q];      Pd[pa + 72 * q] = pd[q];
            Pc[pb + 72 * q] = pc[4 + q];  Pd[pb + 72 * q] = pd[4 + q];
        }
        __syncwarp();
        const int mine = band_s_index(8 * lane);
        const float4 c0 = *reinterpret_cast<const float4*>(Pc + mine), c1 = *reinterpret_cast<const float4*>(Pc + mine + 4);
        const float4 d0 = *reinterpret_cast<const float4*>(Pd + mine), d1 = *reinterpret_cast<const float4*>(Pd + mine + 4);
        const float xc[8] = {c0.x, c0.y, c0.z, c0.w, c1.x, c1.y, c1.z, c1.w};
        const float xd[8] = {d0.x, d0.y, d0.z, d0.w, d1.x, d1.y, d1.z, d1.w};
        float sc[8], sd[8];
        sc[0] = xc[0]; sd[0] = xd[0];
#pragma unroll
        for (int j = 1; j < 8; ++j) { sc[j] = fmaf(keep[j], sc[j - 1], xc[j]); sd[j] = fmaf(keep[j], sd[j - 1], xd[j]); }
        float* S = w + kBandSOffset;
        float4* dc = reinterpret_cast<float4*>(S + mine);
        float4* dd = reinterpret_cast<float4*>(S + kBandSStride + mine);
        dc[0] = make_float4(sc[0], sc[1], sc[2], sc[3]); dc[1] = make_float4(sc[4], sc[5], sc[6], sc[7]);
        dd[0] = make_float4(sd[0], sd[1], sd[2], sd[3]); dd[1] = make_float4(sd[4], sd[5], sd[6], sd[7]);
        if (lane < 2) S[kBandZeroWord + lane * kBandSStride] = 0.f;
        __syncwarp();
    }
};

template <int kPieces>
struct BandGather {
    int last;
    int tail[kPieces];
    __device__ __forceinline__ void init(int first_bin, int end_bin , bool valid) {
        last = kBandZeroWord;
#pragma unroll
        for (int t = 0; t < kPieces; ++t) tail[t] = kBandZeroWord;
        if (valid && end_bin > first_bin) {
            last = band_s_index(end_bin - 1);
            const int l0 = first_bin >> 3, l1 = (end_bin - 1) >> 3;
#pragma unroll
            for (int t = 0; t < kPieces; ++t)
                if (l0 + t < l1) tail[t] = band_s_index(8 * (l0 + t) + 7);
        }
    }
    __device__ __forceinline__ float sum(const float* row) const {
        float acc = row[last];
#pragma unroll
        for (int t = 0; t < kPieces; ++t) acc += row[tail[t]];
        return acc;
    }
};

}
```

### fast_speech_enhancement_metrics_b200/csrc/fsem_lsd.cuh

```cuda
#pragma once
#include "fsem_common.cuh"
#include "fsem_fft.cuh"

namespace fsem {

constexpr float kLsdEps = 1e-8f;

__host__ __device__ __forceinline__ int lsd_num_frames(int64_t n) { return (int)(1 + n / 256); }

__global__ void __launch_bounds__(256)
lsd_scale_kernel(const float* __restrict__ clean, const float* __restrict__ deg, const int32_t* __restrict__ lengths,
                 int64_t batch, int64_t n, int64_t stride, float* __restrict__ alpha) {
    __shared__ double s_cd[8], s_dd[8];
    const int64_t item = blockIdx.x;
    const int len = item_length(lengths, item, n);
    const float* __restrict__ c = clean + item * stride;
    const float* __restrict__ d = deg + item * stride;
    double cd = 0.0, dd = 0.0;
    for (int i = threadIdx.x; i < len; i += 256) {
        const float x = __ldg(c + i), y = __ldg(d + i);
        cd = fma((double)x, (double)y, cd);
        dd = fma((double)y, (double)y, dd);
    }
    cd = warp_sum(cd);
    dd = warp_sum(dd);
    if ((threadIdx.x & 31) == 0) { s_cd[threadIdx.x >> 5] = cd; s_dd[threadIdx.x >> 5] = dd; }
    __syncthreads();
    if (threadIdx.x == 0) {
        double a = 0.0, b = 0.0;
        for (int i = 0; i < 8; ++i) { a += s_cd[i]; b += s_dd[i]; }
        alpha[item] = (float)a / ((float)b + kLsdEps);
    }
}

constexpr int kLsdWarps = 8;

__device__ __forceinline__ float lsd_sqrt(float x) { float y; asm("sqrt.approx.ftz.f32 %0, %1;" : "=f"(y) : "f"(x)); return y; }
__device__ __forceinline__ float lsd_rcp(float x) { float y; asm("rcp.approx.ftz.f32 %0, %1;" : "=f"(y) : "f"(x)); return y; }
__device__ __forceinline__ float lsd_lg2(float x) { float y; asm("lg2.approx.ftz.f32 %0, %1;" : "=f"(y) : "f"(x)); return y; }

template <bool kVec2>
__global__ void __launch_bounds__(kLsdWarps * 32, 2)
lsd_frames_kernel(const float* __restrict__ clean, const float* __restrict__ deg, const int32_t* __restrict__ lengths,
                  int64_t batch, int64_t n, int64_t stride, int tmax, const float* __restrict__ hann,
                  const float* __restrict__ alpha, float* __restrict__ frame_lsd ) {
    __shared__ __align__(16) float2 s_buf[kLsdWarps][kFftBufElems];
    const int lane = threadIdx.x & 31;
    const int warp = threadIdx.x >> 5;
    float2* buf = s_buf[warp];
    FftTwiddles tw;
    tw.init(lane);
    float win[16];
#pragma unroll
    for (int h = 0; h < 2; ++h)
#pragma unroll
        for (int j = 0; j < 8; ++j) win[8 * h + j] = hann[fft_in_index(lane, h, j)];

    const int64_t units = batch * (int64_t)tmax;
    const int64_t nwarps = (int64_t)gridDim.x * kLsdWarps;
    const int64_t per = (units + nwarps - 1) / nwarps;
    const int64_t u0 = ((int64_t)blockIdx.x * kLsdWarps + warp) * per;
    const int64_t u1 = min(units, u0 + per);
    if (u0 >= u1) return;
    int64_t item = u0 / tmax;
    int f = (int)(u0 - item * tmax);
    int len = item_length(lengths, item, n);
    int T = lsd_num_frames(len);
    for (int64_t u = u0; u < u1; ++u) {
        if (f < T) {
            const float* __restrict__ c = clean + item * stride;
            const float* __restrict__ d = deg + item * stride;
            const int first = f * 256 - 256;
            float re[16], im[16];
            if (kVec2 && first >= 0 && first + 512 <= len) {
                const float2* __restrict__ pc2 = reinterpret_cast<const float2*>(c + first) + lane;
                const float2* __restrict__ pd2 = reinterpret_cast<const float2*>(d + first) + lane;
#pragma unroll
                for (int j = 0; j < 8; ++j) {
                    const float2 cv = __ldg(pc2 + 32 * j), dv = __ldg(pd2 + 32 * j);
                    re[j] = cv.x * win[j];  re[8 + j] = cv.y * win[8 + j];
                    im[j] = dv.x * win[j];  im[8 + j] = dv.y * win[8 + j];
                }
            } else {
#pragma unroll
                for (int h = 0; h < 2; ++h)
#pragma unroll
                    for (int j = 0; j < 8; ++j) {
                        const int i = first + fft_in_index(lane, h, j);
                        const bool ok = i >= 0 && i < len;
                        re[8 * h + j] = ok ? __ldg(c + i) * win[8 * h + j] : 0.f;
                        im[8 * h + j] = ok ? __ldg(d + i) * win[8 * h + j] : 0.f;
                    }
            }
            float ar[8], ai[8], br[8], bi[8];
            warp_fft512<false>(re, im, buf, tw, lane, ar, ai, br, bi);
            float pc[8], pd[8];
            packed_power_regs(ar, ai, br, bi, lane, pc, pd);
            const float a = fabsf(alpha[item]);
            float acc = 0.f;
#pragma unroll
            for (int j = 0; j < 8; ++j) {
                const float den = fmaf(a, lsd_sqrt(pd[j] * kPackedPowerScale), kLsdEps);
                const float l = lsd_lg2(fmaf(pc[j] * kPackedPowerScale, lsd_rcp(den * den), kLsdEps));
                acc = fmaf(l, l, acc);
            }
            if (lane == 0) {
                const float den = fmaf(a, fabsf(ai[4]), kLsdEps);
                const float l = lsd_lg2(fmaf(ar[4] * ar[4], lsd_rcp(den * den), kLsdEps));
                acc = fmaf(l, l, acc);
            }
            acc = warp_sum(acc);
            constexpr float kLn2Sq = 0.69314718056f * 0.69314718056f;
            if (lane == 0) frame_lsd[item * tmax + f] = sqrtf(acc * (kLn2Sq / 257.f));
            __syncwarp();
        }
        if (++f == tmax) {
            f = 0;
            ++item;
            if (item < batch) { len = item_length(lengths, item, n); T = lsd_num_frames(len); }
        }
    }
}

__global__ void __launch_bounds__(128)
lsd_finalize_kernel(const float* __restrict__ frame_lsd, const int32_t* __restrict__ lengths, int64_t batch, int64_t n,
                    int tmax, float* __restrict__ out) {
    const int64_t item = (int64_t)blockIdx.x * blockDim.x + threadIdx.x;
    if (item >= batch) return;
    const int T = lsd_num_frames(item_length(lengths, item, n));
    double acc = 0.0;
    for (int f = 0; f < T; ++f) acc += (double)frame_lsd[item * tmax + f];
    out[item] = (float)(acc / (double)T);
}

}
```

### fast_speech_enhancement_metrics_b200/csrc/fsem_pesq.cuh

```cuda
#pragma once
#include "fsem_common.cuh"
#include "fsem_fft.cuh"

namespace fsem {

struct PesqTables {
    float hann[FSEM_PESQ_NFFT];
    int32_t band_first[FSEM_PESQ_NBANDS];
    int32_t band_count[FSEM_PESQ_NBANDS];
    float pow_dens[FSEM_PESQ_NBANDS];
    float thresh[FSEM_PESQ_NBANDS];
    float zw_exp[FSEM_PESQ_NBANDS];
    float width[FSEM_PESQ_NBANDS];
    float loud_scale[FSEM_PESQ_NBANDS];
    float width_total;
};

struct PesqFilterCoef {
    float k;
    float c0[FSEM_BP_SECTIONS], c1[FSEM_BP_SECTIONS], a1[FSEM_BP_SECTIONS], a2[FSEM_BP_SECTIONS];
    float pb0, pb1, pb2, pa1, pa2;
};

struct IirState {
// ... 35 lines not shown
}

template <bool kVec4, typename T>
__global__ void __launch_bounds__(128)
pesq_filter_kernel(const T* __restrict__ clean, const T* __restrict__ deg,
                   const int32_t* __restrict__ lengths, int64_t batch, int64_t n, int64_t stride,
                   int chunk, int nchunks, int warm, const __grid_constant__ PesqFilterCoef P,
                   float* __restrict__ z_out, int64_t zstride, double* __restrict__ partial) {
    const int64_t gid = (int64_t)blockIdx.x * blockDim.x + threadIdx.x;
    if (gid >= 2 * batch * nchunks) return;
    const int64_t sig = gid / nchunks;
    const int c = (int)(gid - sig * nchunks);
    const int64_t item = sig < batch ? sig : sig - batch;
    const T* __restrict__ x = (sig < batch ? clean : deg) + item * stride;
    float* __restrict__ z = z_out + sig * zstride;
    const int len = item_length(lengths, item, n);

    const int t_acc = c * chunk;
    if (t_acc >= len) { partial[gid] = 0.0; return; }
    const int t_end = min(len, t_acc + chunk);
    int t = max(0, t_acc - warm);

    IirState st;
#pragma unroll
    for (int s = 0; s < FSEM_BP_SECTIONS; ++s) { st.w1[s] = 0.f; st.w2[s] = 0.f; }
    st.s1 = 0.f; st.s2 = 0.f;

    auto load4 = [&](int tt, float (&v)[4]) {
        if (kVec4 && tt + 4 <= len) {
            float4 q = load_samples4<false>(x + tt);
            v[0] = q.x; v[1] = q.y; v[2] = q.z; v[3] = q.w;
        } else {
#pragma unroll
            for (int j = 0; j < 4; ++j) v[j] = (tt + j < len) ? load_sample(x + tt + j) : 0.f;
        }
    };

    double acc_d = 0.0;
    float acc = 0.f;
    int groups = 0;
    float cur[8][4], nxt[8][4];
    auto load_block = [&](int tb, float (&blk)[8][4]) {
#pragma unroll
        for (int g = 0; g < 8; ++g) load4(tb + 4 * g, blk[g]);
    };
    load_block(t, cur);
    for (; t < t_end; t += 32) {
        if (t + 32 < t_end) load_block(t + 32, nxt);
#pragma unroll
        for (int g = 0; g < 8; ++g) {
            const int tg = t + 4 * g;
            if (tg >= t_end) break;
            const bool edge = (tg < 16) || (tg + 4 > len - 16);
            float zz[4], yy[4];
#pragma unroll
            for (int j = 0; j < 4; ++j) {
                yy[j] = bandpass_step(P, st, cur[g][j]);
                float xv = edge ? cur[g][j] * taper_weight(tg + j, len) : cur[g][j];
                zz[j] = preemph_step(P, st, xv);
            }
            if (tg >= t_acc) {
                if (tg + 4 <= t_end) {
                    acc += (yy[0] * yy[0] + yy[1] * yy[1]) + (yy[2] * yy[2] + yy[3] * yy[3]);
                    if (kVec4) {
                        *reinterpret_cast<float4*>(z + tg) = make_float4(zz[0], zz[1], zz[2], zz[3]);
                    } else {
#pragma unroll
                        for (int j = 0; j < 4; ++j) z[tg + j] = zz[j];
                    }
                } else {
#pragma unroll
                    for (int j = 0; j < 4; ++j) {
                        if (tg + j < t_end) { acc = fmaf(yy[j], yy[j], acc); z[tg + j] = zz[j]; }
                    }
                }
                if (++groups == 16) { acc_d += (double)acc; acc = 0.f; groups = 0; }
            }
        }
#pragma unroll
        for (int g = 0; g < 8; ++g)
#pragma unroll
            for (int j = 0; j < 4; ++j) cur[g][j] = nxt[g][j];
    }
    partial[gid] = acc_d + (double)acc;
}

constexpr int kFiltWarps = 4;
#ifndef FSEM_FILTER_DRAIN32
constexpr int kFiltPitch = 68;
#else
constexpr int kFiltPitch = 36;
#endif

template <bool kHasLengths, typename T>
__global__ void __launch_bounds__(kFiltWarps * 32)
pesq_filter_tiled_kernel(const T* __restrict__ clean, const T* __restrict__ deg,
                         const int32_t* __restrict__ lengths, const int32_t* __restrict__ order, int64_t batch,
                         int64_t n, int64_t stride, int chunk, int nchunks, int warm,
                         const __grid_constant__ PesqFilterCoef P, float* __restrict__ z_out, int64_t zstride,
                         double* __restrict__ partial) {
    __shared__ __align__(16) float s_tile[kFiltWarps][32 * kFiltPitch];
    const int lane = threadIdx.x & 31;
    const int warp = threadIdx.x >> 5;
    float* tile = s_tile[warp];
    const int64_t groups = ceil_div(batch, 32);
    const int64_t unit = (int64_t)blockIdx.x * kFiltWarps + warp;
    if (unit >= 2 * groups * nchunks) return;
    const int half = (int)(unit / (groups * nchunks));
    const int64_t rem = unit - (int64_t)half * groups * nchunks;
    const int64_t grp = rem / nchunks;
    const int c = (int)(rem - grp * nchunks);
    const int64_t row0 = grp * 32;

    const bool sig_ok = row0 + lane < batch;
    const int64_t my_item = !sig_ok ? 0 : (kHasLengths && order != nullptr) ? (int64_t)order[row0 + lane] : row0 + lane;
    const int len = sig_ok ? item_length(lengths, my_item, n) : 0;
    const int col = (lane & 7) * 4;
    const int64_t trow = row0 + (lane >> 3);
    const T* __restrict__ sbase = (half ? deg : clean) + col;
    float* __restrict__ dbase = z_out + (int64_t)half * batch * zstride + col;
    const T* __restrict__ src0 = sbase + trow * stride;
    float* __restrict__ dst0 = dbase + trow * zstride;
    const int64_t sstep = 4 * stride, dstep = 4 * zstride;
    int row_len[kHasLengths ? 8 : 1];
    int row_item[kHasLengths ? 8 : 1];
    if (kHasLengths) {
#pragma unroll
        for (int i = 0; i < 8; ++i) {
            const int64_t slot = trow + 4 * i;
            const int64_t it = slot >= batch ? 0 : (order != nullptr ? (int64_t)order[slot] : slot);
            row_item[i] = (int)it;
            row_len[i] = slot < batch ? item_length(lengths, it, n) : 0;
        }
    }
    const int rows_ok = (int)min((int64_t)8, (batch - trow + 3) / 4);
    auto rlen = [&](int i) -> int { return kHasLengths ? row_len[kHasLengths ? i : 0] : (i < rows_ok ? (int)n : 0); };
    auto src_row = [&](int i) -> const T* {
        return kHasLengths ? sbase + (int64_t)row_item[kHasLengths ? i : 0] * stride : src0 + i * sstep;
    };
    auto dst_row = [&](int i) -> float* {
        return kHasLengths ? dbase + (int64_t)row_item[kHasLengths ? i : 0] * zstride : dst0 + i * dstep;
    };

    const int t_acc = c * chunk;
    const int grp_len = kHasLengths ? __reduce_max_sync(kFull, len) : (int)n;
    const int t_stop = min(grp_len, t_acc + chunk);
    const int t_end = min(len, t_stop);
    int t = max(0, t_acc - warm);
    if (t_acc >= grp_len) t = t_stop;

    IirState st;
#pragma unroll
    for (int s = 0; s < FSEM_BP_SECTIONS; ++s) { st.w1[s] = 0.f; st.w2[s] = 0.f; }
    st.s1 = 0.f; st.s2 = 0.f;
    double acc_d = 0.0;

    auto fetch = [&](int tt, RawQuad<T> (&v)[8]) {
#pragma unroll
        for (int i = 0; i < 8; ++i) {
            const int a = tt + col;
            const int rl = rlen(i);
            const T* q = src_row(i) + tt;
            if (a + 4 <= rl) {
                v[i] = load_raw4<true>(q);
            } else {
                v[i] = raw_pack(load_raw1(q, a < rl), load_raw1(q + 1, a + 1 < rl), load_raw1(q + 2, a + 2 < rl),
                                load_raw1(q + 3, a + 3 < rl), q);
            }
        }
    };
    RawQuad<T> pre[8];
    if (t < t_stop) fetch(t, pre);
    for (; t < t_stop; t += 32) {
#ifndef FSEM_FILTER_DRAIN32
        const int cs = ((t >> 5) & 1) * 32;
#else
        constexpr int cs = 0;
#endif
#pragma unroll
        for (int i = 0; i < 8; ++i)
            *reinterpret_cast<float4*>(tile + ((lane >> 3) + 4 * i) * kFiltPitch + cs + col) = raw_to_f4(pre[i]);
        __syncwarp();
        if (t + 32 < t_stop) fetch(t + 32, pre);
        float* row = tile + lane * kFiltPitch + cs;
        const bool owned = t >= t_acc;
        float acc = 0.f;
        if (t >= 16 && t + 48 <= len) {
            float acc2 = 0.f;
#pragma unroll
            for (int g = 0; g < 8; ++g) {
                float4 q = *reinterpret_cast<const float4*>(row + 4 * g);
                float y0 = bandpass_step(P, st, q.x); float z0 = preemph_step(P, st, q.x);
                float y1 = bandpass_step(P, st, q.y); float z1 = preemph_step(P, st, q.y);
                float y2 = bandpass_step(P, st, q.z); float z2 = preemph_step(P, st, q.z);
                float y3 = bandpass_step(P, st, q.w); float z3 = preemph_step(P, st, q.w);
                acc = fmaf(y0, y0, acc); acc2 = fmaf(y1, y1, acc2);
                acc = fmaf(y2, y2, acc); acc2 = fmaf(y3, y3, acc2);
                *reinterpret_cast<float4*>(row + 4 * g) = make_float4(z0, z1, z2, z3);
            }
            acc += acc2;
        } else if (t < len) {
#pragma unroll
            for (int g = 0; g < 8; ++g) {
                float4 q = *reinterpret_cast<const float4*>(row + 4 * g);
                float v[4] = {q.x, q.y, q.z, q.w};
                float zz[4];
                const int tg = t + 4 * g;
                const bool edge = (tg < 16) || (tg + 4 > len - 16);
#pragma unroll
                for (int j = 0; j < 4; ++j) {
                    float yv = bandpass_step(P, st, v[j]);
                    float xv = edge ? v[j] * taper_weight(tg + j, len) : v[j];
                    zz[j] = preemph_step(P, st, xv);
                    if (tg + j < t_end) acc = fmaf(yv, yv, acc);
                }
                *reinterpret_cast<float4*>(row + 4 * g) = make_float4(zz[0], zz[1], zz[2], zz[3]);
            }
        }
        if (owned) acc_d += (double)acc;
        __syncwarp();
        auto drain = [&](int td, int slot) {
#pragma unroll
            for (int i = 0; i < 8; ++i) {
                const int a = td + col;
                const int rl = rlen(i);
                float4 q = *reinterpret_cast<const float4*>(tile + ((lane >> 3) + 4 * i) * kFiltPitch + slot + col);
                float* d = dst_row(i) + td;
                if (a + 4 <= rl) {
                    *reinterpret_cast<float4*>(d) = q;
                } else {
                    if (a < rl) d[0] = q.x;
                    if (a + 1 < rl) d[1] = q.y;
                    if (a + 2 < rl) d[2] = q.z;
                }
            }
        };
#ifndef FSEM_FILTER_DRAIN32
        if (owned) {
            if (cs == 32) { drain(t - 32, 0); drain(t, 32); }
            else if (t + 32 >= t_stop) drain(t, 0);
        }
#else
        if (owned) drain(t, 0);
#endif
        __syncwarp();
    }
    if (sig_ok) partial[((int64_t)half * batch + my_item) * nchunks + c] = acc_d;
}

constexpr int kOrderThreads = 1024;

__device__ __forceinline__ int length_bucket(int len, int64_t n) { return (int)(((int64_t)len * 256) / (n + 1)); }

__global__ void __launch_bounds__(kOrderThreads)
pesq_order_kernel(const int32_t* __restrict__ lengths, int64_t batch, int64_t n, int32_t* __restrict__ order,
                  int64_t* __restrict__ frame_prefix) {
    __shared__ int s_hist[256];
    __shared__ long long s_warp[kOrderThreads / 32];
    __shared__ long long s_carry;
    const int tid = threadIdx.x, lane = tid & 31, warp = tid >> 5;
    if (tid < 256) s_hist[tid] = 0;
    if (tid == 0) s_carry = 0;
    __syncthreads();
    for (int64_t i = tid; i < batch; i += kOrderThreads) atomicAdd(&s_hist[length_bucket(item_length(lengths, i, n), n)], 1);
    __syncthreads();
    if (tid == 0) {
        int run = 0;
        for (int k = 0; k < 256; ++k) { const int c = s_hist[k]; s_hist[k] = run; run += c; }
    }
    __syncthreads();
    for (int64_t i = tid; i < batch; i += kOrderThreads)
        order[atomicAdd(&s_hist[length_bucket(item_length(lengths, i, n), n)], 1)] = (int32_t)i;
    for (int64_t base = 0; base < batch; base += kOrderThreads) {
        const int64_t i = base + tid;
        const long long T = i < batch ? pesq_num_frames(item_length(lengths, i, n)) : 0;
        long long v = T;
#pragma unroll
        for (int o = 1; o < 32; o <<= 1) {
            const long long up = __shfl_up_sync(kFull, v, o);
            if (lane >= o) v += up;
        }
        if (lane == 31) s_warp[warp] = v;
        __syncthreads();
        if (warp == 0) {
            long long w = s_warp[lane];
#pragma unroll
            for (int o = 1; o < 32; o <<= 1) {
                const long long up = __shfl_up_sync(kFull, w, o);
                if (lane >= o) w += up;
            }
            s_warp[lane] = w;
        }
        __syncthreads();
        const long long before = s_carry + (warp > 0 ? s_warp[warp - 1] : 0);
        if (i < batch) frame_prefix[i] = before + v - T;
        __syncthreads();
        if (tid == kOrderThreads - 1) s_carry = before + v;
        __syncthreads();
    }
    if (tid == 0) frame_prefix[batch] = s_carry;
}

#ifndef FSEM_FFT_WARPS
#define FSEM_FFT_WARPS 8
#endif
#ifndef FSEM_FFT_MINBLOCKS
#define FSEM_FFT_MINBLOCKS 2
#endif
constexpr int kSpecWarps = FSEM_FFT_WARPS;

constexpr int kBarkRow = FSEM_PESQ_NBANDS + 1;

__device__ __forceinline__ double pesq_band_power(const double* __restrict__ partial, int nchunks, int64_t batch, int sig,
                                                  int64_t item, int lane) {
    const double* p = partial + ((int64_t)sig * batch + item) * nchunks;
    double acc = 0.0;
    for (int c = lane; c < nchunks; c += 32) acc += p[c];
    return warp_sum(acc);
}
__device__ __forceinline__ float pesq_level_gain(double power, int len) {
    return (float)(1.0e7 * ((double)len + 5120.0) * 1.04684 / power);
}

struct SpecWarpSmem {
    float2 fft[kFftBufElems];
    float half_c[3][FSEM_PESQ_HOP];
    float half_d[3][FSEM_PESQ_HOP];
    unsigned long long bar[3];
    float gain[2];
};
static_assert(kBandBufFloats <= 2 * kFftBufElems, "band rows alias the FFT exchange buffer");
constexpr int kBarkPiecesLow = 1;
constexpr int kBarkPiecesHigh = 4;
constexpr size_t kSpecDynSmem = sizeof(SpecWarpSmem) * kSpecWarps;
static_assert(sizeof(SpecWarpSmem) % 16 == 0, "per-warp shared block must keep 16-byte alignment");

__global__ void __launch_bounds__(kSpecWarps * 32, FSEM_FFT_MINBLOCKS)
pesq_spectrum_kernel(const float* __restrict__ z, int64_t zstride, const int32_t* __restrict__ lengths,
                     const int64_t* __restrict__ frame_prefix, int64_t batch, int64_t n, int tmax, int tpitch,
                     const double* __restrict__ partial ,
                     int nchunks, const PesqTables* __restrict__ tab,
                     float* __restrict__ bark ) {
    extern __shared__ __align__(16) unsigned char s_raw[];
    const int lane = threadIdx.x & 31;
    const int warp = threadIdx.x >> 5;
    SpecWarpSmem& sm = reinterpret_cast<SpecWarpSmem*>(s_raw)[warp];
    float2* buf = sm.fft;
    float* wbuf = reinterpret_cast<float*>(sm.fft);
    const float* S = wbuf + kBandSOffset;
    const uint32_t bar0 = smem_u32(&sm.bar[0]);
    const uint32_t hc0 = smem_u32(&sm.half_c[0][0]), hd0 = smem_u32(&sm.half_d[0][0]);
    constexpr uint32_t kHalfBytes = FSEM_PESQ_HOP * sizeof(float);
    if (lane == 0) {
        for (int i = 0; i < 3; ++i) mbar_init(bar0 + 8 * i, 1);
        mbar_fence_init();
    }
    __syncwarp();

    FftTwiddles tw;
    tw.init(lane);
    float win[8];
#pragma unroll
    for (int h = 0; h < 2; ++h)
#pragma unroll
        for (int j = 0; j < 4; ++j) win[4 * h + j] = tab->hann[fft_in_index(lane, h, j)];
    FftLaneBins bins;
    bins.init(lane);
    BandScan scan;
    scan.init(tab->band_first, FSEM_PESQ_NBANDS, lane, bins);
    BandGather<kBarkPiecesLow> g_lo;
    BandGather<kBarkPiecesHigh> g_hi;
    g_lo.init(tab->band_first[lane], tab->band_first[lane] + tab->band_count[lane], true);
    {
        const bool has_hi = lane + 32 < FSEM_PESQ_NBANDS;
        const int bh = has_hi ? lane + 32 : 0;
        g_hi.init(tab->band_first[bh], tab->band_first[bh] + tab->band_count[bh], has_hi);
    }
    const float scale0 = tab->pow_dens[lane] * kPackedPowerScale;
    const float scale1 = (lane + 32 < FSEM_PESQ_NBANDS) ? tab->pow_dens[lane + 32] * kPackedPowerScale : 0.f;

    const int64_t units = frame_prefix ? frame_prefix[batch] : batch * (int64_t)tmax;
    const int64_t nwarps = (int64_t)gridDim.x * kSpecWarps;
    const int64_t per = (units + nwarps - 1) / nwarps;
    const int64_t v0 = ((int64_t)blockIdx.x * kSpecWarps + warp) * per;
    int remaining = (int)(min(units, v0 + per) - v0);
    if (remaining <= 0) return;
    int64_t item;
    int f;
    if (frame_prefix) {
        int64_t lo = 0, hi = batch;
        while (hi - lo > 1) {
            const int64_t mid = (lo + hi) >> 1;
            if (frame_prefix[mid] <= v0) lo = mid; else hi = mid;
        }
        item = lo;
        f = (int)(v0 - frame_prefix[lo]);
    } else {
        item = v0 / tmax;
        f = (int)(v0 - item * tmax);
    }
    int len = item_length(lengths, item, n);
    int T = pesq_num_frames(len);

    unsigned par = 7u;
    auto issue_half = [&](int slot, int64_t it, int h) {
        par ^= 1u << slot;
        if (lane == 0) {
            fence_proxy_async();
            mbar_arrive_expect_tx(bar0 + 8 * slot, 2 * kHalfBytes);
            bulk_copy_g2s(hc0 + slot * kHalfBytes, z + it * zstride + h * FSEM_PESQ_HOP, kHalfBytes, bar0 + 8 * slot);
            bulk_copy_g2s(hd0 + slot * kHalfBytes, z + (batch + it) * zstride + h * FSEM_PESQ_HOP, kHalfBytes,
                          bar0 + 8 * slot);
        }
    };
    int sa = 0, sb = 1;
    issue_half(0, item, f);
    issue_half(1, item, f + 1);
    auto set_gain = [&](int64_t it, int ln) {
        const float gc = pesq_level_gain(pesq_band_power(partial, nchunks, batch, 0, it, lane), ln);
        const float gd = pesq_level_gain(pesq_band_power(partial, nchunks, batch, 1, it, lane), ln);
        if (lane == 0) { sm.gain[0] = gc; sm.gain[1] = gd; }
        __syncwarp();
    };
    set_gain(item, len);

    while (true) {
        const int sn = 3 - sa - sb;
        const bool has_next = remaining > 1;
        const bool same_item = has_next && f + 1 < T;
        int64_t item2 = item;
        int len2 = len, T2 = T;
        if (has_next && !same_item) {
            do {
                ++item2;
                len2 = item_length(lengths, item2, n);
                T2 = pesq_num_frames(len2);
            } while (T2 == 0 && item2 + 1 < batch);
        }
        mbar_wait(bar0 + 8 * sa, (par >> sa) & 1u);
        mbar_wait(bar0 + 8 * sb, (par >> sb) & 1u);
        const float2* ac = reinterpret_cast<const float2*>(sm.half_c[sa]) + lane;
        const float2* ad = reinterpret_cast<const float2*>(sm.half_d[sa]) + lane;
        const float2* bc = reinterpret_cast<const float2*>(sm.half_c[sb]) + lane;
        const float2* bd = reinterpret_cast<const float2*>(sm.half_d[sb]) + lane;
        float re[16], im[16];
#pragma unroll
        for (int j = 0; j < 4; ++j) {
            const float2 c0 = ac[32 * j], d0 = ad[32 * j], c1 = bc[32 * j], d1 = bd[32 * j];
            re[j] = c0.x * win[j];                    re[8 + j] = c0.y * win[4 + j];
            im[j] = d0.x * win[j];                    im[8 + j] = d0.y * win[4 + j];
            re[4 + j] = fmaf(-win[j], c1.x, c1.x);    re[12 + j] = fmaf(-win[4 + j], c1.y, c1.y);
            im[4 + j] = fmaf(-win[j], d1.x, d1.x);    im[12 + j] = fmaf(-win[4 + j], d1.y, d1.y);
        }
        if (f * FSEM_PESQ_HOP + FSEM_PESQ_NFFT > len) {
            const int room = len - f * FSEM_PESQ_HOP;
#pragma unroll
            for (int h = 0; h < 2; ++h)
#pragma unroll
                for (int j = 0; j < 8; ++j)
                    if (fft_in_index(lane, h, j) >= room) { re[8 * h + j] = 0.f; im[8 * h + j] = 0.f; }
        }
        __syncwarp();
        if (has_next) {
            if (same_item) issue_half(sn, item, f + 2);
            else issue_half(sn, item2, 0);
        }
        float ar[8], ai[8], br[8], bi[8];
        warp_fft512<false>(re, im, buf, tw, lane, ar, ai, br, bi);
        float pc[8], pd[8];
        packed_power_regs(ar, ai, br, bi, lane, pc, pd);
        if (lane == 0) { pc[0] = 0.f; pd[0] = 0.f; }
        scan.scan_store(pc, pd, wbuf, lane);
        float* __restrict__ out_c = bark + (item * tpitch + f) * kBarkRow;
        float* __restrict__ out_d = bark + ((batch + item) * tpitch + f) * kBarkRow;
        const float lo_c = g_lo.sum(S), lo_d = g_lo.sum(S + kBandSStride);
        const float hi_c = g_hi.sum(S), hi_d = g_hi.sum(S + kBandSStride);
        const float2 g2 = *reinterpret_cast<const float2*>(sm.gain);
        out_c[lane] = (lo_c * scale0) * g2.x;
        out_d[lane] = (lo_d * scale0) * g2.y;
        if (lane + 32 < FSEM_PESQ_NBANDS) {
            out_c[lane + 32] = (hi_c * scale1) * g2.x;
            out_d[lane + 32] = (hi_d * scale1) * g2.y;
        }
        if (!has_next) break;
        --remaining;
        if (same_item) {
            sa = sb; sb = sn;
            ++f;
        } else {
            item = item2; f = 0; len = len2; T = T2;
            const int freed = sa;
            sa = sn; sb = freed;
            __syncwarp();
            issue_half(sb, item, f + 1);
            set_gain(item, len);
        }
    }
}

#ifndef FSEM_BARK_THREADS
#define FSEM_BARK_THREADS 128
#endif
constexpr int kBarkThreads = FSEM_BARK_THREADS;
constexpr int kBarkTile = FSEM_BARK_THREADS / 2;
constexpr int kBarkThreadsWide = 640;
constexpr int kBarkTileWide = 320;
__host__ __device__ constexpr size_t bark_dyn_smem(int tile) { return tile <= 64 ? 0 : sizeof(float) * (size_t)tile * (2 * kBarkRow + 2); }

__device__ __forceinline__ float mufu_lg2(float x) { float y; asm("lg2.approx.ftz.f32 %0, %1;" : "=f"(y) : "f"(x)); return y; }
__device__ __forceinline__ float mufu_ex2(float x) { float y; asm("ex2.approx.ftz.f32 %0, %1;" : "=f"(y) : "f"(x)); return y; }
__device__ __forceinline__ float mufu_rcp(float x) { float y; asm("rcp.approx.ftz.f32 %0, %1;" : "=f"(y) : "f"(x)); return y; }
__device__ __forceinline__ float fast_pow(float x, float y) { return mufu_ex2(y * mufu_lg2(x)); }

__device__ __forceinline__ float zwicker_loudness(float p, float thr, float inv_thr, float e, float scale) {
    float l = scale * (fast_pow(fmaf(0.5f * p, inv_thr, 0.5f), e) - 1.f);
    return (p <= thr) ? 0.f : l;
}

template <int kThreads, int kTile>
__global__ void __launch_bounds__(kThreads)
pesq_bark_kernel(const float* __restrict__ bark, const double* __restrict__ partial, int nchunks,
                 const int32_t* __restrict__ lengths, const int32_t* __restrict__ order, int64_t batch, int64_t n, int tpitch,
                 const PesqTables* __restrict__ tab, float* __restrict__ dist_ws ,
                 float* __restrict__ mos_out, int32_t* __restrict__ status_out,
                 double* __restrict__ power_out ) {
    static_assert(kThreads == 2 * kTile && kThreads % 32 == 0 && kThreads >= 2 * FSEM_PESQ_NBANDS, "two threads per frame of a tile");
    static_assert(kTile % 4 == 0, "tile rows are fetched in 16-byte units");
    constexpr bool kDyn = bark_dyn_smem(kTile) > 0;
    extern __shared__ __align__(16) float s_bark_dyn[];
    __shared__ __align__(16) float s_tile_st[kDyn ? 1 : 2][kDyn ? 1 : kTile][kBarkRow];
    __shared__ float s_live_st[kDyn ? 1 : kTile];
    __shared__ float s_fr_st[kDyn ? 1 : kTile];
    float (*s_tile)[kTile][kBarkRow] =
        kDyn ? reinterpret_cast<float (*)[kTile][kBarkRow]>(s_bark_dyn)
             : reinterpret_cast<float (*)[kTile][kBarkRow]>(&s_tile_st[0][0][0]);
    float* s_live = kDyn ? s_bark_dyn + 2 * kTile * kBarkRow : s_live_st;
    float* s_fr = kDyn ? s_bark_dyn + 2 * kTile * kBarkRow + kTile : s_fr_st;
    __shared__ float s_thr[FSEM_PESQ_NBANDS], s_thr100[FSEM_PESQ_NBANDS], s_ithr[FSEM_PESQ_NBANDS], s_exp[FSEM_PESQ_NBANDS],
        s_lsc[FSEM_PESQ_NBANDS], s_w[FSEM_PESQ_NBANDS], s_ratio[FSEM_PESQ_NBANDS];
    __shared__ float s_g2[2];
    __shared__ float s_carry[2];
    __shared__ float s_red[2][kThreads / 32];
    __shared__ __align__(8) unsigned long long s_bar;

    const int tid = threadIdx.x;
    const int64_t item = order ? (int64_t)order[batch - 1 - blockIdx.x] : (int64_t)blockIdx.x;
    const int len = item_length(lengths, item, n);
    const int T = pesq_num_frames(len);
    const uint32_t bar = smem_u32(&s_bar);

    if (tid < FSEM_PESQ_NBANDS) {
        float thr = tab->thresh[tid];
        s_thr[tid] = thr;
        s_thr100[tid] = thr * 100.f;
        s_ithr[tid] = 1.f / thr;
        s_exp[tid] = tab->zw_exp[tid];
        s_lsc[tid] = tab->loud_scale[tid];
        s_w[tid] = tab->width[tid];
    }
    if (tid < 64) {
        const int sig = tid >> 5;
        const double acc = pesq_band_power(partial, nchunks, batch, sig, item, tid & 31);
        if ((tid & 31) == 0) {
            power_out[(int64_t)sig * batch + item] = acc;
            s_g2[sig] = pesq_level_gain(acc, len);
        }
    }
    if (tid == 0) {
        mbar_init(bar, 1);
        mbar_fence_init();
    }
    __syncthreads();
    if (T < 20 || !(isfinite(s_g2[0]) && isfinite(s_g2[1]))) {
        if (tid == 0) {
            mos_out[item] = nanf("");
            if (status_out) status_out[item] = (T < 20) ? FSEM_ITEM_TOO_SHORT : FSEM_ITEM_NAN;
        }
        return;
    }
    const float* __restrict__ bc = bark + item * (int64_t)tpitch * kBarkRow;
    const float* __restrict__ bd = bark + (batch + item) * (int64_t)tpitch * kBarkRow;
    const uint32_t tile_c = smem_u32(&s_tile[0][0][0]), tile_d = smem_u32(&s_tile[1][0][0]);
    unsigned parity = 0;

    auto load_tile = [&](int f0, int nf) {
        __syncthreads();
        if (tid == 0) {
            const uint32_t bytes = (uint32_t)((nf + 3) & ~3) * (kBarkRow * sizeof(float));
            fence_proxy_async();
            mbar_arrive_expect_tx(bar, 2 * bytes);
            bulk_copy_g2s(tile_c, bc + (int64_t)f0 * kBarkRow, bytes, bar);
            bulk_copy_g2s(tile_d, bd + (int64_t)f0 * kBarkRow, bytes, bar);
        }
        mbar_wait(bar, parity);
        parity ^= 1u;
    };

    double band_acc = 0.0;
    const int my_sig = tid / FSEM_PESQ_NBANDS;
    const int my_band = tid - my_sig * FSEM_PESQ_NBANDS;
    for (int f0 = 0; f0 < T; f0 += kTile) {
        const int nf = min(kTile, T - f0);
        load_tile(f0, nf);
        {
            const int fs = tid >> 1, half = tid & 1;
            float a = 0.f;
            if (fs < nf) {
#pragma unroll 5
                for (int b = half; b < FSEM_PESQ_NBANDS; b += 2) {
                    float p = s_tile[0][fs][b];
                    a += p * ((p > s_thr100[b]) ? 1.f : 0.f);
                }
            }
            a += __shfl_xor_sync(kFull, a, 1);
            if (fs < nf && half == 0) s_live[fs] = (a < 1.0e7f) ? 0.f : 1.f;
        }
        __syncthreads();
        if (tid < 2 * FSEM_PESQ_NBANDS) {
            const float thr100 = s_thr100[my_band];
            const float* col = &s_tile[my_sig][0][my_band];
            float acc = 0.f;
#pragma unroll 4
            for (int f = 0; f < nf; ++f) {
                const float p = col[f * kBarkRow];
                acc += (p > thr100) ? p * s_live[f] : 0.f;
            }
            band_acc += (double)acc;
        }
    }
    __syncthreads();
    double* s_mean = reinterpret_cast<double*>(&s_tile[0][0][0]);
    if (tid < 2 * FSEM_PESQ_NBANDS) s_mean[tid] = band_acc / (double)T;
    __syncthreads();
    if (tid < FSEM_PESQ_NBANDS) {
        float r = (float)((s_mean[FSEM_PESQ_NBANDS + tid] + 1000.0) / (s_mean[tid] + 1000.0));
        s_ratio[tid] = fminf(fmaxf(r, 0.01f), 100.f);
    }
    if (tid == 0) s_carry[0] = 0.f;

    const float wtot = tab->width_total;
    float* __restrict__ dsym = dist_ws + item * (int64_t)tpitch;
    float* __restrict__ dasym = dist_ws + (batch + item) * (int64_t)tpitch;

    for (int f0 = 0; f0 < T; f0 += kTile) {
        const int nf = min(kTile, T - f0);
        load_tile(f0, nf);
        const int fs = tid >> 1, half = tid & 1;
        const bool live = fs < nf;
        float afp_c = 0.f, afp_d = 0.f;
        if (live) {
#pragma unroll 5
            for (int b = half; b < FSEM_PESQ_NBANDS; b += 2) {
                float c = s_ratio[b] * s_tile[0][fs][b];
                float d = s_tile[1][fs][b];
                afp_c += c * ((c > s_thr[b]) ? 1.f : 0.f);
                afp_d += d * ((d > s_thr[b]) ? 1.f : 0.f);
            }
        }
        afp_c += __shfl_xor_sync(kFull, afp_c, 1);
        afp_d += __shfl_xor_sync(kFull, afp_d, 1);
        if (live && half == 0) s_fr[fs] = (afp_c + 5.0e3f) / (afp_d + 5.0e3f);
        __syncthreads();
        float sym_acc = 0.f, asym_acc = 0.f;
        if (live) {
            const int f = f0 + fs;
            float fr = s_fr[fs];
            if (f > 0) {
                float prev = (fs == 0) ? s_carry[(f0 / kTile) & 1] : s_fr[fs - 1];
                fr = 0.8f * fr + 0.2f * prev;
            }
            fr = fminf(fmaxf(fr, 3.0e-4f), 5.f);
            for (int b = half; b < FSEM_PESQ_NBANDS; b += 2) {
                const float c = s_ratio[b] * s_tile[0][fs][b];
                const float d = fr * s_tile[1][fs][b];
                const float thr = s_thr[b], ithr = s_ithr[b], e = s_exp[b], lsc = s_lsc[b];
                const float lc = zwicker_loudness(c, thr, ithr, e, lsc);
                const float ld = zwicker_loudness(d, thr, ithr, e, lsc);
                const float dead = 0.25f * fminf(lc, ld);
                float diff = ld - lc;
                float mag = fmaxf(fabsf(diff) - dead, 0.f);
                float dist = copysignf(mag, diff);
                if (diff != diff) dist = diff;
                const float wd = (b >= 1) ? s_w[b] * dist : 0.f;
                sym_acc = fmaf(wd, wd, sym_acc);
                const float ratio = (d + 50.f) * mufu_rcp(c + 50.f);
                const float scale = (ratio < 2.49804953f) ? 0.f : fminf(fast_pow(ratio, 1.2f), 12.f);
                asym_acc += fabsf(wd * scale);
            }
        }
        sym_acc += __shfl_xor_sync(kFull, sym_acc, 1);
        asym_acc += __shfl_xor_sync(kFull, asym_acc, 1);
        if (live && half == 0) {
            const int f = f0 + fs;
            float sym = fmaxf(sqrtf(wtot * sym_acc), 1.0e-20f);
            float asym = fmaxf(asym_acc, 1.0e-20f);
            const float weight = fast_pow((afp_c + 1.0e5f) * 1.0e-7f, 0.04f);
            dsym[f] = fminf(sym / weight, 45.f);
            dasym[f] = fminf(asym / weight, 45.f);
        }
        if (tid == 2 * (nf - 1)) s_carry[(f0 / kTile + 1) & 1] = s_fr[nf - 1];
    }
    __syncthreads();

    const int W = (T - 20) / 10 + 1;
    float acc_s = 0.f, acc_a = 0.f;
    for (int w = tid; w < W; w += kThreads) {
        float s6 = 0.f, a6 = 0.f;
#pragma unroll 4
        for (int j = 0; j < 20; ++j) {
            float s = dsym[10 * w + j], a = dasym[10 * w + j];
            float s2 = s * s, a2 = a * a;
            s6 = fmaf(s2 * s2, s2, s6);
            a6 = fmaf(a2 * a2, a2, a6);
        }
        float ps = powf(s6 * 0.05f, 1.f / 6.f), pa = powf(a6 * 0.05f, 1.f / 6.f);
        acc_s = fmaf(ps, ps, acc_s);
        acc_a = fmaf(pa, pa, acc_a);
    }
    acc_s = warp_sum(acc_s);
    acc_a = warp_sum(acc_a);
    if ((tid & 31) == 0) { s_red[0][tid >> 5] = acc_s; s_red[1][tid >> 5] = acc_a; }
    __syncthreads();
    if (tid == 0) {
        float ts = 0.f, ta = 0.f;
        for (int i = 0; i < kThreads / 32; ++i) { ts += s_red[0][i]; ta += s_red[1][i]; }
        float d_sym = sqrtf(ts / (float)W), d_asym = sqrtf(ta / (float)W);
        float mos = 4.5f - 0.1f * d_sym - 0.0309f * d_asym;
        mos = 0.999f + 4.f / (1.f + expf(-1.3669f * mos + 3.8224f));
        mos_out[item] = mos;
        if (status_out) status_out[item] = (mos == mos) ? FSEM_ITEM_OK : FSEM_ITEM_NAN;
    }
}

}
```

### fast_speech_enhancement_metrics_b200/csrc/fsem_stoi.cuh

```cuda
#pragma once
#include "fsem_common.cuh"
#include "fsem_fft.cuh"

namespace fsem {

struct StoiTables {
    float window[FSEM_STOI_WIN];
    int32_t band_lo[FSEM_STOI_NBANDS];
    int32_t band_hi[FSEM_STOI_NBANDS];
    float clip;
    float dyn_range;
};

template <typename T>
__global__ void __launch_bounds__(256)
stoi_resample_kernel(const T* __restrict__ clean, const T* __restrict__ deg,
                     const int32_t* __restrict__ lengths, int64_t batch, int64_t n, int64_t stride,
                     const float* __restrict__ taps, int orig, int neu, int width, int ntaps,
                     float* __restrict__ y, int64_t ystride, int blocks_per_sig) {
    const int64_t sig = blockIdx.x / blocks_per_sig;
    const int bx = blockIdx.x - (int)sig * blocks_per_sig;
    const int64_t item = sig < batch ? sig : sig - batch;
    const int len = item_length(lengths, item, n);
    const int64_t L = stoi_resampled_len(len, orig, neu);
// ... 51 lines not shown
                       const int32_t* __restrict__ lengths, int64_t batch, int64_t n, int64_t stride,
                       const __grid_constant__ Resample85Taps taps, const StoiTables* __restrict__ tab,
                       float* __restrict__ y, int64_t ystride, double2* __restrict__ hop_energy, int hops_max,
                       int blocks_per_sig) {
    __shared__ float4 s_in[kRs85SmemQuads];
    __shared__ __align__(16) float s_out[kRs85TileOut];
    __shared__ __align__(16) float s_win[FSEM_STOI_WIN];
    const int tid = threadIdx.x;
    const int64_t sig = blockIdx.x / blocks_per_sig;
    const int bx = blockIdx.x - (int)sig * blocks_per_sig;
    const bool is_clean = sig < batch;
    const int64_t item = is_clean ? sig : sig - batch;
    const int len = item_length(lengths, item, n);
    const int L = (int)stoi_resampled_len(len, 8, 5);
    const int tile0 = bx * kRs85TilesPerCta;
    if (tile0 * kRs85TileOut >= L) return;
    const T* __restrict__ x = (is_clean ? clean : deg) + item * stride;
    float* __restrict__ yrow = y + sig * ystride;
    for (int i = tid; i < FSEM_STOI_WIN; i += kRs85Threads) s_win[i] = tab->window[i];

    constexpr int kPerThread = (kRs85Quads + kRs85Threads - 1) / kRs85Threads;
    const int fill_q = kRs85PadEvery == 4 ? (tid & ~31) + 4 * (((tid & 31) >> 3) + 4 * ((tid >> 2) & 1)) + (tid & 3) : tid;
    const int len32 = len;
    auto fetch = [&](int tile, RawQuad<T> (&v)[kPerThread]) {
        const int in0 = tile * kRs85TileIn - 12;
        if (kVec4 && in0 >= 0 && in0 + 4 * kRs85Quads <= len32) {
#pragma unroll
            for (int r = 0; r < kPerThread; ++r) {
                const int q = fill_q + r * kRs85Threads;
                if (r + 1 < kPerThread || q < kRs85Quads) v[r] = load_raw4<false>(x + in0 + 4 * q);
                else v[r] = raw_zero<T>();
            }
            return;
        }
#pragma unroll
        for (int r = 0; r < kPerThread; ++r) {
            const int q = fill_q + r * kRs85Threads;
            const int i = in0 + 4 * q;
            if (q >= kRs85Quads) { v[r] = raw_zero<T>(); continue; }
            if (kVec4 && i >= 0 && i + 4 <= len32) {
                v[r] = load_raw4<false>(x + i);
            } else {
                v[r] = raw_pack(load_raw1(x + i, i >= 0 && i < len32), load_raw1(x + i + 1, i + 1 >= 0 && i + 1 < len32),
                                load_raw1(x + i + 2, i + 2 >= 0 && i + 2 < len32),
                                load_raw1(x + i + 3, i + 3 >= 0 && i + 3 < len32), x);
            }
        }
    };
    RawQuad<T> pre[kPerThread];
    fetch(tile0, pre);
    for (int k = 0; k < kRs85TilesPerCta; ++k) {
        const int tile = tile0 + k;
        const int out0 = tile * kRs85TileOut;
        if (out0 >= L) break;
#pragma unroll
        for (int r = 0; r < kPerThread; ++r) {
            const int q = fill_q + r * kRs85Threads;
            if (q < kRs85Quads) s_in[q + q / kRs85PadEvery] = raw_to_f4(pre[r]);
        }
        __syncthreads();
        if (k + 1 < kRs85TilesPerCta && (out0 + kRs85TileOut) < L) fetch(tile + 1, pre);
        float xin[4 * kRs85ThreadQuads];
        const float4* src = s_in + (kRs85PadEvery + 1) * tid;
        auto load_quad = [&](int i) {
            float4 v = src[i + i / kRs85PadEvery];
            xin[4 * i] = v.x; xin[4 * i + 1] = v.y; xin[4 * i + 2] = v.z; xin[4 * i + 3] = v.w;
        };
#pragma unroll
        for (int i = 0; i < 8; ++i) load_quad(i);
        float out[5 * kRs85Nb];
#pragma unroll
        for (int b = 0; b < kRs85Nb; ++b) {
            if (b + 1 < kRs85Nb) { load_quad(2 * b + 8); load_quad(2 * b + 9); }
#pragma unroll
            for (int p = 0; p < 5; ++p) {
                float acc = 0.f;
#pragma unroll
                for (int j = rs85_lo(p); j <= rs85_hi(p); ++j) acc = fmaf(taps.h[p][j], xin[2 + 8 * b + j], acc);
                out[5 * b + p] = acc;
            }
        }
        if (kRs85Nb % 4 == 0) {
#pragma unroll
            for (int i = 0; i < 5 * kRs85Nb / 4; ++i)
                *reinterpret_cast<float4*>(s_out + 5 * kRs85Nb * tid + 4 * i) =
                    make_float4(out[4 * i], out[4 * i + 1], out[4 * i + 2], out[4 * i + 3]);
        } else {
#pragma unroll
            for (int i = 0; i < 5 * kRs85Nb / 2; ++i)
                *reinterpret_cast<float2*>(s_out + 5 * kRs85Nb * tid + 2 * i) = make_float2(out[2 * i], out[2 * i + 1]);
        }
        __syncthreads();
        const int valid = min(kRs85TileOut, L - out0);
        if (valid == kRs85TileOut) {
#pragma unroll
            for (int q = tid; q < kRs85TileOut / 4; q += kRs85Threads)
                *reinterpret_cast<float4*>(yrow + out0 + 4 * q) = *reinterpret_cast<const float4*>(s_out + 4 * q);
        } else {
            for (int q = tid; q < kRs85TileOut / 4; q += kRs85Threads) {
                const float4 v = *reinterpret_cast<const float4*>(s_out + 4 * q);
                float* d = yrow + out0 + 4 * q;
                if (4 * q + 4 <= valid) {
                    *reinterpret_cast<float4*>(d) = v;
                } else {
                    if (4 * q < valid) d[0] = v.x;
                    if (4 * q + 1 < valid) d[1] = v.y;
                    if (4 * q + 2 < valid) d[2] = v.z;
                }
            }
        }
        if (is_clean) {
            const int lane = tid & 31, warp = tid >> 5;
            const float4 wa = *reinterpret_cast<const float4*>(s_win + 4 * lane);
            const float4 wb = *reinterpret_cast<const float4*>(s_win + 128 + 4 * lane);
            constexpr int kWarps = kRs85Threads / 32;
            constexpr int kHopsPerWarp = (kRs85Hops + kWarps - 1) / kWarps;
            constexpr int kHopGroups = (kHopsPerWarp + 2) / 3;
#pragma unroll 1
            for (int grp = 0; grp < kHopGroups; ++grp) {
            double v[6];
#pragma unroll
            for (int i = 0; i < 3; ++i) {
                const int h = warp + kWarps * (3 * grp + i);
                double a = 0.0, b = 0.0;
                if (h < kRs85Hops && (h + 1) * FSEM_STOI_HOP <= valid) {
                    const float4 x = *reinterpret_cast<const float4*>(s_out + h * FSEM_STOI_HOP + 4 * lane);
                    float f;
                    f = __fmul_rn(x.x, wa.x); a = fma((double)f, (double)f, a);
                    f = __fmul_rn(x.y, wa.y); a = fma((double)f, (double)f, a);
                    f = __fmul_rn(x.z, wa.z); a = fma((double)f, (double)f, a);
                    f = __fmul_rn(x.w, wa.w); a = fma((double)f, (double)f, a);
                    f = __fmul_rn(x.x, wb.x); b = fma((double)f, (double)f, b);
                    f = __fmul_rn(x.y, wb.y); b = fma((double)f, (double)f, b);
                    f = __fmul_rn(x.z, wb.z); b = fma((double)f, (double)f, b);
                    f = __fmul_rn(x.w, wb.w); b = fma((double)f, (double)f, b);
                }
                v[2 * i] = a; v[2 * i + 1] = b;
            }
            const bool b16 = lane & 16, b8 = lane & 8, b4 = lane & 4;
            double u[3];
#pragma unroll
            for (int i = 0; i < 3; ++i) {
                const double send = b16 ? v[i] : v[3 + i], keep = b16 ? v[3 + i] : v[i];
                u[i] = keep + __shfl_xor_sync(kFull, send, 16);
            }
            double t2[2];
            {
                const double s0 = b8 ? u[0] : u[2], k0 = b8 ? u[2] : u[0];
                const double s1 = b8 ? u[1] : 0.0, k1 = b8 ? 0.0 : u[1];
                t2[0] = k0 + __shfl_xor_sync(kFull, s0, 8);
                t2[1] = k1 + __shfl_xor_sync(kFull, s1, 8);
            }
            double one;
            {
                const double send = b4 ? t2[0] : t2[1], keep = b4 ? t2[1] : t2[0];
                one = keep + __shfl_xor_sync(kFull, send, 4);
            }
            one += __shfl_xor_sync(kFull, one, 2);
            one += __shfl_xor_sync(kFull, one, 1);
            const int local = b8 ? 2 : (b4 ? 1 : 0);
            const int sum_idx = (b16 ? 3 : 0) + local;
            const int h = warp + kWarps * (3 * grp + (sum_idx >> 1));
            if ((lane & 3) == 0 && !(b8 && b4) && h < kRs85Hops && (h + 1) * FSEM_STOI_HOP <= valid) {
                double* dst = reinterpret_cast<double*>(hop_energy + item * hops_max + tile * kRs85Hops + h);
                dst[sum_idx & 1] = one;
            }
            }
        }
        __syncthreads();
    }
}

__global__ void __launch_bounds__(256)
stoi_energy_from_hops_kernel(const double2* __restrict__ hop_energy, int hops_max, const int32_t* __restrict__ lengths,
                             int64_t batch, int64_t n, int t0max, float* __restrict__ energy) {
    const int64_t gid = (int64_t)blockIdx.x * blockDim.x + threadIdx.x;
    if (gid >= batch * (int64_t)t0max) return;
    const int64_t item = gid / t0max;
    const int t = (int)(gid - item * t0max);
    const int64_t L = stoi_resampled_len(item_length(lengths, item, n), 8, 5);
    if (t >= stoi_num_frames(L)) return;
    const double2 h0 = hop_energy[item * hops_max + t];
    const double2 h1 = hop_energy[item * hops_max + t + 1];
    float nrm = (float)sqrt(h0.x + h1.y);
    float v = __fadd_rn(nrm, 1e-9f);
    float lg = (float)log10((double)v);
    energy[gid] = __fmul_rn(20.f, lg);
}

__global__ void __launch_bounds__(256)
stoi_energy_kernel(const float* __restrict__ sig10k, int64_t sstride, const int32_t* __restrict__ lengths,
                   int64_t batch, int64_t n, int orig, int neu, int t0max,
                   const StoiTables* __restrict__ tab, float* __restrict__ energy ) {
    const int lane = threadIdx.x & 31;
    const int64_t wid = ((int64_t)blockIdx.x * blockDim.x + threadIdx.x) >> 5;
    if (wid >= batch * (int64_t)t0max) return;
    const int64_t item = wid / t0max;
    const int t = (int)(wid - item * t0max);
    const int64_t L = stoi_resampled_len(item_length(lengths, item, n), orig, neu);
    if (t >= stoi_num_frames(L)) return;
    const float* __restrict__ x = sig10k + item * sstride + (int64_t)t * FSEM_STOI_HOP;
    double acc = 0.0;
#pragma unroll
    for (int m = 0; m < 8; ++m) {
        int q = lane + 32 * m;
        float f = __fmul_rn(__ldg(x + q), tab->window[q]);
        acc = fma((double)f, (double)f, acc);
    }
    acc = warp_sum(acc);
    if (lane == 0) {
        float nrm = (float)sqrt(acc);
        float v = __fadd_rn(nrm, 1e-9f);
        float lg = (float)log10((double)v);
        energy[item * t0max + t] = __fmul_rn(20.f, lg);
    }
}

__global__ void __launch_bounds__(128)
stoi_compact_kernel(const float* __restrict__ energy, const int32_t* __restrict__ lengths, int64_t batch,
                    int64_t n, int orig, int neu, int t0max, int mask_words, float dyn_range,
                    int32_t* __restrict__ kept_idx , int32_t* __restrict__ kept_count,
                    uint32_t* __restrict__ mask_bits ) {
    const int lane = threadIdx.x & 31;
    const int64_t item = ((int64_t)blockIdx.x * blockDim.x + threadIdx.x) >> 5;
    if (item >= batch) return;
    const int64_t L = stoi_resampled_len(item_length(lengths, item, n), orig, neu);
    const int T0 = stoi_num_frames(L);
    const float* __restrict__ e = energy + item * t0max;
    float mx = -INFINITY;
    for (int t = lane; t < T0; t += 32) mx = fmaxf(mx, e[t]);
    mx = warp_max(mx);
    const float thr = __fsub_rn(mx, dyn_range);
    int count = 0;
    for (int t0 = 0; t0 < mask_words * 32; t0 += 32) {
        const int t = t0 + lane;
        bool keep = false;
        if (t < T0) keep = __fsub_rn(thr, e[t]) < 0.f;
        const unsigned bal = __ballot_sync(kFull, keep);
        if (keep) kept_idx[item * t0max + count + __popc(bal & ((1u << lane) - 1u))] = t;
        if (lane == 0) mask_bits[item * mask_words + (t0 >> 5)] = bal;
        count += __popc(bal);
    }
    if (lane == 0) kept_count[item] = count;
}

__global__ void __launch_bounds__(128)
stoi_margin_kernel(const float* __restrict__ energy, const int32_t* __restrict__ lengths, int64_t batch, int64_t n,
                   int orig, int neu, int t0max, float dyn_range, float* __restrict__ margin_out) {
    const int lane = threadIdx.x & 31;
    const int64_t item = ((int64_t)blockIdx.x * blockDim.x + threadIdx.x) >> 5;
    if (item >= batch) return;
    const int64_t L = stoi_resampled_len(item_length(lengths, item, n), orig, neu);
    const int T0 = stoi_num_frames(L);
    const float* __restrict__ e = energy + item * t0max;
    float mx = -INFINITY;
    for (int t = lane; t < T0; t += 32) mx = fmaxf(mx, e[t]);
    mx = warp_max(mx);
    const float thr = __fsub_rn(mx, dyn_range);
    float mg = INFINITY;
    for (int t = lane; t < T0; t += 32) mg = fminf(mg, fabsf(__fsub_rn(thr, e[t])));
    mg = -warp_max(-mg);
    if (lane == 0) margin_out[item] = mg;
}

__global__ void __launch_bounds__(1024)
stoi_prefix_kernel(const int32_t* __restrict__ kept_count, int64_t batch, int32_t* __restrict__ prefix) {
    __shared__ int s_warp[32];
    __shared__ int s_carry;
    const int tid = threadIdx.x, lane = tid & 31, warp = tid >> 5;
    if (tid == 0) s_carry = 0;
    __syncthreads();
    for (int64_t base = 0; base < batch; base += 1024) {
        const int64_t i = base + tid;
        const int v = (i < batch) ? max(kept_count[i] - 2, 0) : 0;
        int x = v;
#pragma unroll
        for (int o = 1; o < 32; o <<= 1) {
            int y = __shfl_up_sync(kFull, x, o);
            if (lane >= o) x += y;
        }
        if (lane == 31) s_warp[warp] = x;
        __syncthreads();
        if (warp == 0) {
            int w = s_warp[lane];
#pragma unroll
            for (int o = 1; o < 32; o <<= 1) {
                int y = __shfl_up_sync(kFull, w, o);
                if (lane >= o) w += y;
            }
            s_warp[lane] = w;
        }
        __syncthreads();
        const int carry = s_carry;
        const int incl = carry + x + (warp > 0 ? s_warp[warp - 1] : 0);
        if (i < batch) prefix[i] = incl - v;
        __syncthreads();
        if (tid == 1023) s_carry = incl;
        __syncthreads();
    }
    if (tid == 0) prefix[batch] = s_carry;
}

#ifndef FSEM_FFT_WARPS
#define FSEM_FFT_WARPS 8
#endif
#ifndef FSEM_FFT_MINBLOCKS
#define FSEM_FFT_MINBLOCKS 2
#endif
constexpr int kTobWarps = FSEM_FFT_WARPS;

constexpr int kTobPieces = 6;
static_assert(kBandBufFloats <= 2 * kFftBufElems, "band rows alias the FFT exchange buffer");

template <bool kVec2>
__global__ void __launch_bounds__(kTobWarps * 32, FSEM_FFT_MINBLOCKS)
stoi_tob_kernel(const float* __restrict__ clean10k, const float* __restrict__ deg10k, int64_t sstride,
                int64_t batch, int t0max, int umax,
                int ustride, const int32_t* __restrict__ kept_idx, const int32_t* __restrict__ frame_prefix,
                const StoiTables* __restrict__ tab, float* __restrict__ tob ) {
    __shared__ __align__(16) float2 s_buf[kTobWarps][kFftBufElems];
    __shared__ int32_t s_starts[FSEM_STOI_NBANDS + 2];
    const int lane = threadIdx.x & 31;
    const int warp = threadIdx.x >> 5;
    float2* buf = s_buf[warp];
    float* wbuf = reinterpret_cast<float*>(buf);
    if (threadIdx.x == 0) s_starts[0] = 0;
    if (threadIdx.x < FSEM_STOI_NBANDS) s_starts[1 + threadIdx.x] = tab->band_lo[threadIdx.x];
    if (threadIdx.x == FSEM_STOI_NBANDS) s_starts[FSEM_STOI_NBANDS + 1] = tab->band_hi[FSEM_STOI_NBANDS - 1];
    __syncthreads();

    FftTwiddles tw;
    tw.init(lane);
    float win[8];
#pragma unroll
    for (int h = 0; h < 2; ++h)
#pragma unroll
        for (int j = 0; j < 4; ++j) win[4 * h + j] = tab->window[fft_in_index(lane, h, j)];
    FftLaneBins bins;
    bins.init(lane);
    BandScan scan;
    scan.init(s_starts, FSEM_STOI_NBANDS + 2, lane, bins);
    const int my_band = lane & 15;
    const bool has_band = my_band < FSEM_STOI_NBANDS;
    BandGather<kTobPieces> gather;
    gather.init(s_starts[1 + (has_band ? my_band : 0)], s_starts[2 + (has_band ? my_band : 0)], has_band);
    const float* Srow = wbuf + kBandSOffset + (lane >> 4) * kBandSStride;

    const int64_t total = frame_prefix[batch];
    const int64_t nwarps = (int64_t)gridDim.x * kTobWarps;
    const int64_t per = (total + nwarps - 1) / nwarps;
    const int64_t w0 = ((int64_t)blockIdx.x * kTobWarps + warp) * per;
    const int64_t w1 = min(total, w0 + per);
    if (w0 >= w1) return;
    int64_t lo_i = 0, hi_i = batch;
    while (hi_i - lo_i > 1) {
        const int64_t mid = (lo_i + hi_i) >> 1;
        if (frame_prefix[mid] <= w0) lo_i = mid; else hi_i = mid;
    }
    int64_t item = lo_i;
    int item_end = frame_prefix[item + 1];
    int u = (int)(w0 - frame_prefix[item]);
    for (int64_t w = w0; w < w1; ++w, ++u) {
        while (w >= item_end) { ++item; item_end = frame_prefix[item + 1]; u = 0; }
        {
            const int32_t* idx = kept_idx + item * t0max + u;
            const int ta = idx[0] * FSEM_STOI_HOP, tb = idx[1] * FSEM_STOI_HOP, tc = idx[2] * FSEM_STOI_HOP;
            if (w + 1 < item_end && lane < 16) {
                const float* p = ((lane & 8) ? deg10k : clean10k) + item * sstride + idx[3] * FSEM_STOI_HOP + 32 * (lane & 7);
                asm volatile("prefetch.global.L1 [%0];" ::"l"(p));
            }
            const float* __restrict__ xc = clean10k + item * sstride + 2 * lane;
            const float* __restrict__ xd = deg10k + item * sstride + 2 * lane;
            auto pair = [&](const float* p) -> float2 {
                if (kVec2) return __ldg(reinterpret_cast<const float2*>(p));
                return make_float2(__ldg(p), __ldg(p + 1));
            };
            float re[16], im[16];
#pragma unroll
            for (int j = 0; j < 4; ++j) {
                const int q = 64 * j;
                const int nb = (j < 2) ? (ta + q + 128) : (tc + q - 128);
                const int jn = (j < 2) ? j + 2 : j - 2;
                const float2 c0 = pair(xc + tb + q), c1 = pair(xc + nb);
                const float2 d0 = pair(xd + tb + q), d1 = pair(xd + nb);
                const float w0f = win[j], w1f = win[4 + j], n0f = win[jn], n1f = win[4 + jn];
                re[j] = __fmul_rn(w0f, __fadd_rn(__fmul_rn(w0f, c0.x), __fmul_rn(n0f, c1.x)));
                re[8 + j] = __fmul_rn(w1f, __fadd_rn(__fmul_rn(w1f, c0.y), __fmul_rn(n1f, c1.y)));
                im[j] = __fmul_rn(w0f, __fadd_rn(__fmul_rn(w0f, d0.x), __fmul_rn(n0f, d1.x)));
                im[8 + j] = __fmul_rn(w1f, __fadd_rn(__fmul_rn(w1f, d0.y), __fmul_rn(n1f, d1.y)));
            }
#pragma unroll
            for (int j = 4; j < 8; ++j) { re[j] = 0.f; im[j] = 0.f; re[8 + j] = 0.f; im[8 + j] = 0.f; }
            float ar[8], ai[8], br[8], bi[8];
            warp_fft512<true>(re, im, buf, tw, lane, ar, ai, br, bi);
            float pc[8], pd[8];
            packed_power_regs(ar, ai, br, bi, lane, pc, pd);
            scan.scan_store(pc, pd, wbuf, lane);
            const float band = gather.sum(Srow);
            if (has_band) {
                const int64_t sig = (lane >> 4) ? (batch + item) : item;
                tob[(sig * FSEM_STOI_NBANDS + my_band) * (int64_t)ustride + u] = 0.5f * sqrtf(band);
            }
            __syncwarp();
        }
    }
}

constexpr int kSegTile = 64;
constexpr int kSegThreads = 256;
constexpr int kSegCols = kSegTile + FSEM_STOI_SEG - 1;
constexpr int kSegPitch = 97;
constexpr int kSegTilesPerCta = 4;
#ifndef FSEM_SEG_RUN
#define FSEM_SEG_RUN 4
#endif
constexpr int kSegRun = FSEM_SEG_RUN;
static_assert(kSegTile % kSegRun == 0, "runs tile the segment tile");

__device__ __forceinline__ float rsqrt_or_zero(float v) { return v > 0.f ? rsqrtf(v) : 0.f; }
__device__ __forceinline__ float rsqrt_resolved(float v, float s2) { return v > 4e-6f * s2 ? rsqrtf(v) : 0.f; }

__global__ void __launch_bounds__(kSegThreads, 2)
stoi_segment_kernel(const float* __restrict__ tob, int64_t batch, int ustride, int ntiles,
                    const int32_t* __restrict__ kept_count, float clip,
                    float2* __restrict__ partial ) {
    __shared__ float s_x[FSEM_STOI_NBANDS][kSegPitch];
    __shared__ float s_y[FSEM_STOI_NBANDS][kSegPitch];
    __shared__ float4 s_row[kSegTile][FSEM_STOI_NBANDS];
    __shared__ float s_red[2][kSegThreads / 32];

    const int tid = threadIdx.x;
    const int groups = (ntiles + kSegTilesPerCta - 1) / kSegTilesPerCta;
    const int64_t item = blockIdx.x / groups;
    const int tile_first = (int)(blockIdx.x - item * groups) * kSegTilesPerCta;
    const int K = kept_count[item];
    const int M = max(K - 31, 0);
    const float* __restrict__ tx0 = tob + (item * FSEM_STOI_NBANDS) * (int64_t)ustride;
    const float* __restrict__ ty0 = tob + ((batch + item) * FSEM_STOI_NBANDS) * (int64_t)ustride;
    constexpr int kTileVals = 2 * FSEM_STOI_NBANDS * kSegCols;
    constexpr int kPerThread = (kTileVals + kSegThreads - 1) / kSegThreads;
    auto fetch = [&](int tile, float (&v)[kPerThread]) {
        const int m0f = tile * kSegTile;
        const int ncolf = min(kSegTile, M - m0f) + FSEM_STOI_SEG - 1;
#pragma unroll
        for (int r = 0; r < kPerThread; ++r) {
            const int i = tid + r * kSegThreads;
            const int sg = i / (FSEM_STOI_NBANDS * kSegCols);
            const int rem = i - sg * (FSEM_STOI_NBANDS * kSegCols);
            const int j = rem / kSegCols, c = rem - j * kSegCols;
            const bool ok = i < kTileVals && c < ncolf;
            v[r] = ok ? __ldg((sg ? ty0 : tx0) + (int64_t)j * ustride + m0f + c) : 0.f;
        }
    };
    float pre[kPerThread];
    if (tile_first * kSegTile < M) fetch(tile_first, pre);
    for (int tk = 0; tk < kSegTilesPerCta; ++tk) {
    const int tile = tile_first + tk;
    if (tile >= ntiles) break;
    const int m0 = tile * kSegTile;
    if (m0 >= M) {
        if (tid == 0) partial[item * ntiles + tile] = make_float2(0.f, 0.f);
        continue;
    }
    const int nseg = min(kSegTile, M - m0);
    __syncthreads();
#pragma unroll
    for (int r = 0; r < kPerThread; ++r) {
        const int i = tid + r * kSegThreads;
        if (i < kTileVals) {
            const int sg = i / (FSEM_STOI_NBANDS * kSegCols);
            const int rem = i - sg * (FSEM_STOI_NBANDS * kSegCols);
            const int j = rem / kSegCols, c = rem - j * kSegCols;
            (sg ? s_y : s_x)[j][c] = pre[r];
        }
    }
    __syncthreads();
    if (tk + 1 < kSegTilesPerCta && tile + 1 < ntiles && (m0 + kSegTile) < M) fetch(tile + 1, pre);

    float stoi_acc = 0.f;
    constexpr int kRunsPerBand = kSegTile / kSegRun;
    for (int id = tid; id < FSEM_STOI_NBANDS * kRunsPerBand; id += kSegThreads) {
        const int j = id / kRunsPerBand, mb = (id - j * kRunsPerBand) * kSegRun;
        if (mb >= nseg) continue;
        float x[FSEM_STOI_SEG + kSegRun - 1], y[FSEM_STOI_SEG + kSegRun - 1];
#pragma unroll
        for (int q = 0; q < FSEM_STOI_SEG + kSegRun - 1; ++q) {
            x[q] = s_x[j][mb + q];
            y[q] = s_y[j][mb + q];
        }
        float cx = 0.f, cy = 0.f, cxx = 0.f, cyy = 0.f;
#pragma unroll
        for (int q = kSegRun - 1; q < FSEM_STOI_SEG; ++q) {
            cx += x[q]; cy += y[q];
            cxx = fmaf(x[q], x[q], cxx);
            cyy = fmaf(y[q], y[q], cyy);
        }
#pragma unroll
        for (int r = 0; r < kSegRun; ++r) {
            const int m = mb + r;
            if (m < nseg) {
                float sx = cx, sy = cy, sxx = cxx, syy = cyy;
#pragma unroll
                for (int e = 0; e < kSegRun - 1; ++e) {
                    const int q = (e < kSegRun - 1 - r) ? r + e : FSEM_STOI_SEG + e - (kSegRun - 1 - r);
                    sx += x[q]; sy += y[q];
                    sxx = fmaf(x[q], x[q], sxx);
                    syy = fmaf(y[q], y[q], syy);
                }
                const float alpha = sqrtf(sxx) / (sqrtf(syy) + 1e-9f);
                const float mx = sx * (1.f / FSEM_STOI_SEG), my = sy * (1.f / FSEM_STOI_SEG);
                float syc = 0.f, sycc = 0.f, sxyc = 0.f;
#pragma unroll
                for (int q = 0; q < FSEM_STOI_SEG; ++q) {
                    const float yc = fminf(y[r + q] * alpha, x[r + q] * clip);
                    syc += yc;
                    sycc = fmaf(yc, yc, sycc);
                    sxyc = fmaf(x[r + q], yc, sxyc);
                }
                const float myc = syc * (1.f / FSEM_STOI_SEG);
                const float vxx = fmaf(-sx, mx, sxx), vyo = fmaf(-sy, my, syy);
                const float vyy = fmaf(-syc, myc, sycc), vxy = fmaf(-sx, myc, sxyc);
                const float rx = rsqrt_resolved(vxx, sxx), ry = rsqrt_resolved(vyy, sycc);
                stoi_acc += vxy * rx * ry;
                s_row[m][j] = make_float4(mx, rx, my, rsqrt_resolved(vyo, syy));
            }
        }
    }
    __syncthreads();

    float estoi_acc = 0.f;
    for (int id = tid; id < kSegTile * FSEM_STOI_SEG; id += kSegThreads) {
        const int m = id / FSEM_STOI_SEG, q = id - m * FSEM_STOI_SEG;
        if (m >= nseg) continue;
        float xh[FSEM_STOI_NBANDS], yh[FSEM_STOI_NBANDS];
        float sx = 0.f, sy = 0.f;
#pragma unroll
        for (int j = 0; j < FSEM_STOI_NBANDS; ++j) {
            const float4 r = s_row[m][j];
            xh[j] = (s_x[j][m + q] - r.x) * r.y;
            yh[j] = (s_y[j][m + q] - r.z) * r.w;
            sx += xh[j]; sy += yh[j];
        }
        const float mx = sx * (1.f / FSEM_STOI_NBANDS), my = sy * (1.f / FSEM_STOI_NBANDS);
        float vxx = 0.f, vyy = 0.f, vxy = 0.f;
#pragma unroll
        for (int j = 0; j < FSEM_STOI_NBANDS; ++j) {
            float dx = xh[j] - mx, dy = yh[j] - my;
            vxx = fmaf(dx, dx, vxx);
            vyy = fmaf(dy, dy, vyy);
            vxy = fmaf(dx, dy, vxy);
        }
        estoi_acc += vxy * rsqrt_or_zero(vxx) * rsqrt_or_zero(vyy);
    }
    stoi_acc = warp_sum(stoi_acc);
    estoi_acc = warp_sum(estoi_acc);
    if ((tid & 31) == 0) { s_red[0][tid >> 5] = stoi_acc; s_red[1][tid >> 5] = estoi_acc; }
    __syncthreads();
    if (tid == 0) {
        float a = 0.f, b = 0.f;
        for (int i = 0; i < kSegThreads / 32; ++i) { a += s_red[0][i]; b += s_red[1][i]; }
        partial[item * ntiles + tile] = make_float2(a, b);
    }
    }
}

__global__ void __launch_bounds__(128)
stoi_finalize_kernel(const float2* __restrict__ partial, int64_t batch, int ntiles,
                     const int32_t* __restrict__ kept_count, float* __restrict__ stoi_out,
                     float* __restrict__ estoi_out, int32_t* __restrict__ kept_out,
                     int32_t* __restrict__ status_out) {
    const int64_t item = (int64_t)blockIdx.x * blockDim.x + threadIdx.x;
    if (item >= batch) return;
    const int K = kept_count[item];
    const int M = max(K - 31, 0);
    double a = 0.0, b = 0.0;
    for (int t = 0; t < ntiles; ++t) {
        float2 p = partial[item * ntiles + t];
        a += (double)p.x;
        b += (double)p.y;
    }
    const float fm = (float)M;
    stoi_out[item] = (float)(a / FSEM_STOI_NBANDS) / fm;
    estoi_out[item] = (float)(b / FSEM_STOI_SEG) / fm;
    if (kept_out) kept_out[item] = K;
    if (status_out) status_out[item] = (M > 0) ? FSEM_ITEM_OK : FSEM_ITEM_TOO_SHORT;
}

}
```

Measured before the change: 4.625 million.

## Restructure warp FFT512 to process two frames per warp with half-warp FFTs

Replaces the whole-warp three-pass radix-8 FFT512 with a half-warp scheme: each 16-lane half computes one frame with a register radix-32 pass, twiddles, one shared-memory transpose and radix-16 passes. Each warp now processes two frames per iteration in the STOI TOB, LSD and PESQ spectrum kernels. Shared buffers move to dynamic shared memory, and warps per CTA and launch bounds are retuned. The aim is fewer shared-memory exchange rounds and syncs per frame, at the cost of much higher register pressure (32-element arrays per lane) and lower occupancy. Scalar loads also replace the float2 vectorized path.

New measurement: 4.767 million (median of 6 runs). 1.03x the previous value.

```diff
diff --git a/fast_speech_enhancement_metrics_b200/csrc/fsem_api.cu b/fast_speech_enhancement_metrics_b200/csrc/fsem_api.cu
--- a/fast_speech_enhancement_metrics_b200/csrc/fsem_api.cu
+++ b/fast_speech_enhancement_metrics_b200/csrc/fsem_api.cu
@@ -487,7 +487,7 @@
     FSEM_LAUNCHED();
     {
         const int64_t units = in->batch * (int64_t)p.tmax;
-        int64_t grid = ceil_div(units, kSpecWarps);
+        int64_t grid = ceil_div(units, 2 * kSpecWarps);
         const int64_t cap = (int64_t)ctx->dev.sms * ctx->spec_ctas_per_sm;
         if (grid > cap) grid = cap;
         { ProfScope prof_(K_PESQ_SPECTRUM, stream);
@@ -628,8 +628,15 @@
                 if ((j < rs85_lo(p) || j > rs85_hi(p)) && d->taps[p * 28 + j] != 0.f) ctx->fast85 = false;
             }
     }
+    e = cudaFuncSetAttribute(stoi_tob_kernel, cudaFuncAttributeMaxDynamicSharedMemorySize, (int)kTobDynSmem);
+    if (e != cudaSuccess) {
+        cudaFree(ctx->d_tab);
+        if (ctx->d_taps) cudaFree(ctx->d_taps);
+        delete ctx;
+        return fail(FSEM_E_CUDA, "fsem_stoi_create: %s", cudaGetErrorString(e));
+    }
     int occ = 0;
-    if (cudaOccupancyMaxActiveBlocksPerMultiprocessor(&occ, stoi_tob_kernel<true>, kTobWarps * 32, 0) == cudaSuccess && occ > 0)
+    if (cudaOccupancyMaxActiveBlocksPerMultiprocessor(&occ, stoi_tob_kernel, kTobWarps * 32, kTobDynSmem) == cudaSuccess && occ > 0)
         ctx->tob_ctas_per_sm = occ;
     *out = ctx;
     return FSEM_OK;
@@ -759,18 +766,12 @@
           stoi_prefix_kernel<<<1, 1024, 0, stream>>>(kept_count, in->batch, frame_prefix); }
         FSEM_LAUNCHED();
         const int64_t units = in->batch * (int64_t)p.umax;
-        int64_t grid = ceil_div(units, kTobWarps);
+        int64_t grid = ceil_div(units, 2 * kTobWarps);
         const int64_t cap = (int64_t)ctx->dev.sms * ctx->tob_ctas_per_sm;
         if (grid > cap) grid = cap;
-        const bool vec2 = (reinterpret_cast<uintptr_t>(c10) & 7u) == 0 && (reinterpret_cast<uintptr_t>(d10) & 7u) == 0 &&
-                          sstride % 2 == 0;
         { ProfScope prof_(K_STOI_TOB, stream);
-          if (vec2)
-              stoi_tob_kernel<true><<<(unsigned)grid, kTobWarps * 32, 0, stream>>>(
-                  c10, d10, sstride, in->batch, p.t0max, p.umax, p.ustride, kept_idx, frame_prefix, ctx->d_tab, tob);
-          else
-              stoi_tob_kernel<false><<<(unsigned)grid, kTobWarps * 32, 0, stream>>>(
-                  c10, d10, sstride, in->batch, p.t0max, p.umax, p.ustride, kept_idx, frame_prefix, ctx->d_tab, tob); }
+          stoi_tob_kernel<<<(unsigned)grid, kTobWarps * 32, kTobDynSmem, stream>>>(
+              c10, d10, sstride, in->batch, p.t0max, p.umax, p.ustride, kept_idx, frame_prefix, ctx->d_tab, tob); }
         FSEM_LAUNCHED();
     }
     {
@@ -1088,8 +1089,14 @@
         delete ctx;
         return fail(FSEM_E_CUDA, "fsem_lsd_create: %s", cudaGetErrorString(e));
     }
+    e = cudaFuncSetAttribute(lsd_frames_kernel, cudaFuncAttributeMaxDynamicSharedMemorySize, (int)kLsdDynSmem);
+    if (e != cudaSuccess) {
+        cudaFree(ctx->d_hann);
+        delete ctx;
+        return fail(FSEM_E_CUDA, "fsem_lsd_create: %s", cudaGetErrorString(e));
+    }
     int occ = 0;
-    if (cudaOccupancyMaxActiveBlocksPerMultiprocessor(&occ, lsd_frames_kernel<true>, kLsdWarps * 32, 0) == cudaSuccess && occ > 0)
+    if (cudaOccupancyMaxActiveBlocksPerMultiprocessor(&occ, lsd_frames_kernel, kLsdWarps * 32, kLsdDynSmem) == cudaSuccess && occ > 0)
         ctx->ctas_per_sm = occ;
     *out = ctx;
     return FSEM_OK;
@@ -1125,18 +1132,12 @@
                                                              in->stride, alpha);
     FSEM_LAUNCHED();
     const int64_t units = in->batch * (int64_t)p.tmax;
-    int64_t grid = ceil_div(units, kLsdWarps);
+    int64_t grid = ceil_div(units, 2 * kLsdWarps);
     const int64_t cap = (int64_t)ctx->dev.sms * ctx->ctas_per_sm;
     if (grid > cap) grid = cap;
-    const bool vec2 = (reinterpret_cast<uintptr_t>(in->clean) & 7u) == 0 && (reinterpret_cast<uintptr_t>(in->deg) & 7u) == 0 &&
-                      in->stride % 2 == 0;
     { ProfScope prof_(K_LSD_FRAMES, stream);
-      if (vec2)
-          lsd_frames_kernel<true><<<(unsigned)grid, kLsdWarps * 32, 0, stream>>>(
-              in->clean, in->deg, in->lengths, in->batch, in->n, in->stride, p.tmax, ctx->d_hann, alpha, frames);
-      else
-          lsd_frames_kernel<false><<<(unsigned)grid, kLsdWarps * 32, 0, stream>>>(
-              in->clean, in->deg, in->lengths, in->batch, in->n, in->stride, p.tmax, ctx->d_hann, alpha, frames); }
+      lsd_frames_kernel<<<(unsigned)grid, kLsdWarps * 32, kLsdDynSmem, stream>>>(
+          in->clean, in->deg, in->lengths, in->batch, in->n, in->stride, p.tmax, ctx->d_hann, alpha, frames); }
     FSEM_LAUNCHED();
     lsd_finalize_kernel<<<(unsigned)ceil_div(in->batch, 128), 128, 0, stream>>>(frames, in->lengths, in->batch, in->n,
                                                                                p.tmax, lsd_out);
diff --git a/fast_speech_enhancement_metrics_b200/csrc/fsem_fft.cuh b/fast_speech_enhancement_metrics_b200/csrc/fsem_fft.cuh
--- a/fast_speech_enhancement_metrics_b200/csrc/fsem_fft.cuh
+++ b/fast_speech_enhancement_metrics_b200/csrc/fsem_fft.cuh
@@ -4,7 +4,9 @@
 namespace fsem {
 
 constexpr int kFftN = 512;
-constexpr int kFftBufElems = 752;
+constexpr int kFftRowF4 = 17;
+constexpr int kFftHalfF4 = 16 * kFftRowF4 + 4;
+constexpr int kFftBufFloats = 2 * 4 * kFftHalfF4;
 
 __device__ __forceinline__ void cmul(float& xr, float& xi, float wr, float wi) {
     float tr = xr * wr - xi * wi;
@@ -55,104 +57,97 @@
     }
 }
 
+__host__ __device__ constexpr float cos32(int j) {
+    j &= 31;
+    constexpr float c[9] = {1.0f, 0.98078528040323043058f, 0.92387953251128673848f, 0.83146961230254523567f,
+                            0.70710678118654757274f, 0.55557023301960228867f, 0.38268343236508983729f,
+                            0.19509032201612833135f, 0.0f};
+    return j <= 8 ? c[j] : j <= 16 ? -c[16 - j] : j <= 24 ? -c[j - 16] : c[32 - j];
+}
+__device__ __forceinline__ void rot32(int j, float& xr, float& xi) {
+    j &= 31;
+    if (j == 0) return;
+    if (j == 8) { const float t = xr; xr = xi; xi = -t; return; }
+    if (j == 16) { xr = -xr; xi = -xi; return; }
+    if (j == 24) { const float t = xr; xr = -xi; xi = t; return; }
+    cmul(xr, xi, cos32(j), -cos32(j - 8));
+}
+
+template <bool kUpperZero>
+__device__ __forceinline__ void dft32(float (&r)[32], float (&i)[32]) {
+    float yr[4][8], yi[4][8];
+#pragma unroll
+    for (int a = 0; a < 4; ++a) {
+#pragma unroll
+        for (int b = 0; b < 8; ++b) { yr[a][b] = r[a + 4 * b]; yi[a][b] = i[a + 4 * b]; }
+        dft8<kUpperZero>(yr[a], yi[a]);
+#pragma unroll
+        for (int c = 1; c < 8; ++c) rot32(a * c, yr[a][c], yi[a][c]);
+    }
+#pragma unroll
+    for (int c = 0; c < 8; ++c) {
+        dft4(yr[0][c], yi[0][c], yr[1][c], yi[1][c], yr[2][c], yi[2][c], yr[3][c], yi[3][c]);
+#pragma unroll
+        for (int d = 0; d < 4; ++d) { r[c + 8 * d] = yr[d][c]; i[c + 8 * d] = yi[d][c]; }
+    }
+}
+
+__device__ __forceinline__ void dft16(float (&r)[16], float (&i)[16]) {
+    float yr[4][4], yi[4][4];
+#pragma unroll
+    for (int a = 0; a < 4; ++a) {
+        dft4(r[a], i[a], r[a + 4], i[a + 4], r[a + 8], i[a + 8], r[a + 12], i[a + 12]);
+#pragma unroll
+        for (int c = 0; c < 4; ++c) { yr[a][c] = r[a + 4 * c]; yi[a][c] = i[a + 4 * c]; rot32(2 * a * c, yr[a][c], yi[a][c]); }
+    }
+#pragma unroll
+    for (int c = 0; c < 4; ++c) {
+        dft4(yr[0][c], yi[0][c], yr[1][c], yi[1][c], yr[2][c], yi[2][c], yr[3][c], yi[3][c]);
+#pragma unroll
+        for (int d = 0; d < 4; ++d) { r[c + 4 * d] = yr[d][c]; i[c + 4 * d] = yi[d][c]; }
+    }
+}
+
 struct FftTwiddles {
-    float w1r[2][7], w1i[2][7];
-    float w2r[7], w2i[7];
+    float wr[16], wi[16];
     __device__ __forceinline__ void init(int lane) {
-#pragma unroll
-        for (int h = 0; h < 2; ++h) {
-            int np = 2 * lane + h;
-#pragma unroll
-            for (int k0 = 1; k0 < 8; ++k0) {
-                float s, c;
-                sincospif(-(float)(np * k0) * (1.0f / 256.0f), &s, &c);
-                w1r[h][k0 - 1] = c; w1i[h][k0 - 1] = s;
-            }
-        }
-        int n0 = lane & 7;
-#pragma unroll
-        for (int k1 = 1; k1 < 8; ++k1) {
+        const int n1 = lane & 15;
+#pragma unroll
+        for (int q = 1; q <= 16; ++q) {
             float s, c;
-            sincospif(-(float)(n0 * k1) * (1.0f / 32.0f), &s, &c);
-            w2r[k1 - 1] = c; w2i[k1 - 1] = s;
+            sincospif(-(float)(n1 * q) * (1.0f / 256.0f), &s, &c);
+            wr[q - 1] = c; wi[q - 1] = s;
         }
     }
 };
 
-__device__ __forceinline__ int fft_in_index(int lane, int h, int j) { return 2 * lane + h + 64 * j; }
-
-struct FftLaneBins {
-    int base_a, base_b;
-    __device__ __forceinline__ void init(int lane) {
-        const int r = lane & 7, j = lane >> 3;
-        if (j >= 1) { base_a = j + 8 * r; base_b = (8 - j) + 8 * (7 - r); }
-        else if (r == 0) { base_a = 0; base_b = 32; }
-        else if (r < 4) { base_a = 8 * r; base_b = 8 * (8 - r); }
-        else { base_a = 4 + 8 * (7 - r); base_b = 4 + 8 * r; }
-    }
-};
+__device__ __forceinline__ int fft_in_index(int lane, int n2) { return (lane & 15) + 16 * n2; }
 
 template <bool kUpperZero>
-__device__ __forceinline__ void warp_fft512(float (&re)[16], float (&im)[16], float2* buf, const FftTwiddles& tw, int lane,
-                                            float (&ar)[8], float (&ai)[8], float (&br)[8], float (&bi)[8]) {
-    float4* buf4 = reinterpret_cast<float4*>(buf);
-#pragma unroll
-    for (int h = 0; h < 2; ++h) {
-        float r[8], i[8];
-#pragma unroll
-        for (int j = 0; j < 8; ++j) { r[j] = re[8 * h + j]; i[j] = im[8 * h + j]; }
-        dft8<kUpperZero>(r, i);
-#pragma unroll
-        for (int k0 = 1; k0 < 8; ++k0) cmul(r[k0], i[k0], tw.w1r[h][k0 - 1], tw.w1i[h][k0 - 1]);
-        float4* row = buf4 + 9 * lane + 4 * h;
-        row[0] = make_float4(r[0], i[0], r[4], i[4]);
-        row[1] = make_float4(r[1], i[1], r[7], i[7]);
-        row[2] = make_float4(r[2], i[2], r[6], i[6]);
-        row[3] = make_float4(r[3], i[3], r[5], i[5]);
-    }
+__device__ __forceinline__ void fft512_half(float (&re)[32], float (&im)[32], float* buf, const FftTwiddles& tw, int lane,
+                                            float (&ar)[16], float (&ai)[16], float (&br)[16], float (&bi)[16]) {
+    dft32<kUpperZero>(re, im);
+#pragma unroll
+    for (int q = 1; q < 16; ++q) {
+        cmul(re[q], im[q], tw.wr[q - 1], tw.wi[q - 1]);
+        cmul(re[32 - q], im[32 - q], tw.wr[q - 1], -tw.wi[q - 1]);
+    }
+    cmul(re[16], im[16], tw.wr[15], -tw.wi[15]);
+    float4* half = reinterpret_cast<float4*>(buf) + (lane >> 4) * kFftHalfF4;
+    float4* row = half + (lane & 15) * kFftRowF4;
+    row[0] = make_float4(re[0], im[0], re[16], im[16]);
+#pragma unroll
+    for (int q = 1; q < 16; ++q) row[q] = make_float4(re[q], im[q], re[32 - q], im[32 - q]);
     __syncwarp();
-    const int lo3 = lane & 7;
-    const int jq = lane >> 3;
-    float r2[2][8], i2[2][8];
-    {
-        const float4* src = buf4 + (lo3 >> 1) * 9 + (lo3 & 1) * 4 + jq;
-#pragma unroll
-        for (int n1 = 0; n1 < 8; ++n1) {
-            const float4 v = src[36 * n1];
-            r2[0][n1] = v.x; i2[0][n1] = v.y; r2[1][n1] = v.z; i2[1][n1] = v.w;
-        }
+    const float4* col = half + (lane & 15);
+#pragma unroll
+    for (int n1 = 0; n1 < 16; ++n1) {
+        const float4 v = col[n1 * kFftRowF4];
+        ar[n1] = v.x; ai[n1] = v.y; br[n1] = v.z; bi[n1] = v.w;
     }
     __syncwarp();
-#pragma unroll
-    for (int s = 0; s < 2; ++s) {
-        dft8<false>(r2[s], i2[s]);
-#pragma unroll
-        for (int k1 = 1; k1 < 8; ++k1) cmul(r2[s][k1], i2[s][k1], tw.w2r[k1 - 1], tw.w2i[k1 - 1]);
-    }
-    {
-        const bool g0 = jq == 0;
-        float4* dst = buf4 + jq * 72 + lo3;
-        dst[0] = make_float4(r2[0][0], i2[0][0], g0 ? r2[0][4] : r2[1][7], g0 ? i2[0][4] : i2[1][7]);
-        dst[9] = make_float4(r2[0][1], i2[0][1], g0 ? r2[0][7] : r2[1][6], g0 ? i2[0][7] : i2[1][6]);
-        dst[18] = make_float4(r2[0][2], i2[0][2], g0 ? r2[0][6] : r2[1][5], g0 ? i2[0][6] : i2[1][5]);
-        dst[27] = make_float4(r2[0][3], i2[0][3], g0 ? r2[0][5] : r2[1][4], g0 ? i2[0][5] : i2[1][4]);
-#pragma unroll
-        for (int r = 4; r < 8; ++r)
-            dst[9 * r] = make_float4(g0 ? r2[1][7 - r] : r2[0][r], g0 ? i2[1][7 - r] : i2[0][r],
-                                     g0 ? r2[1][r] : r2[1][7 - r], g0 ? i2[1][r] : i2[1][7 - r]);
-    }
-    __syncwarp();
-    {
-        const float4* src = buf4 + jq * 72 + lo3 * 9;
-#pragma unroll
-        for (int n0 = 0; n0 < 8; ++n0) {
-            const float4 v = src[n0];
-            ar[n0] = v.x; ai[n0] = v.y; br[n0] = v.z; bi[n0] = v.w;
-        }
-    }
-    __syncwarp();
-    dft8<false>(ar, ai);
-    dft8<false>(br, bi);
+    dft16(ar, ai);
+    dft16(br, bi);
 }
 
 constexpr float kPackedPowerScale = 0.25f;
@@ -163,29 +158,32 @@
     pd = fmaf(si, si, dr * dr);
 }
 
-__device__ __forceinline__ void packed_power_regs(const float (&ar)[8], const float (&ai)[8], const float (&br)[8],
-                                                  const float (&bi)[8], int lane, float (&pc)[8], float (&pd)[8]) {
-    const bool l0 = lane == 0;
-#pragma unroll
-    for (int q = 0; q < 4; ++q) {
-        const float mar = l0 ? ar[(8 - q) & 7] : br[7 - q], mai = l0 ? ai[(8 - q) & 7] : bi[7 - q];
-        const float mbr = l0 ? br[7 - q] : ar[7 - q],       mbi = l0 ? bi[7 - q] : ai[7 - q];
-        packed_power_pair(ar[q], ai[q], mar, mai, pc[q], pd[q]);
-        packed_power_pair(br[q], bi[q], mbr, mbi, pc[4 + q], pd[4 + q]);
+__device__ __forceinline__ void packed_power_regs(const float (&ar)[16], const float (&ai)[16], const float (&br)[16],
+                                                  const float (&bi)[16], int lane, float (&pc)[16], float (&pd)[16]) {
+    const bool l0 = (lane & 15) == 0;
+#pragma unroll
+    for (int s = 0; s < 8; ++s) {
+        const int ms = (16 - s) & 15;
+        const float mar = l0 ? ar[ms] : br[ms],     mai = l0 ? ai[ms] : bi[ms];
+        const float mbr = l0 ? br[ms] : ar[15 - s], mbi = l0 ? bi[ms] : ai[15 - s];
+        packed_power_pair(ar[s], ai[s], mar, mai, pc[s], pd[s]);
+        packed_power_pair(br[s + 1], bi[s + 1], mbr, mbi, pc[8 + s], pd[8 + s]);
     }
 }
 
 __host__ __device__ constexpr int band_s_index(int k) { return k + 4 * (k >> 5); }
 constexpr int kBandSStride = 300;
-constexpr int kBandPOffset = 0;
-constexpr int kBandSOffset = 2 * kBandSStride;
+constexpr int kBandPFrame = 624;
+constexpr int kBandSOffset = 2 * kBandPFrame;
 constexpr int kBandZeroWord = 2 * kBandSStride;
 constexpr int kBandBufFloats = kBandSOffset + 3 * kBandSStride + 4;
+static_assert(kBandBufFloats <= kFftBufFloats, "band rows alias the FFT exchange buffer");
+static_assert(kBandPFrame % 32 == 16 && kBandPFrame >= kBandSStride + 288, "frame 1's P rows: 16 banks on, no overlap");
 
 struct BandScan {
     float keep[8];
     int pa, pb;
-    __device__ __forceinline__ void init(const int32_t* starts, int nbands, int lane, const FftLaneBins& bins) {
+    __device__ __forceinline__ void init(const int32_t* starts, int nbands, int lane) {
         unsigned start_mask = 1u;
         for (int b = 0; b < nbands; ++b) {
             const int f = starts[b];
@@ -193,18 +191,21 @@
         }
 #pragma unroll
         for (int j = 0; j < 8; ++j) keep[j] = ((start_mask >> j) & 1u) ? 0.f : 1.f;
-        pa = band_s_index(bins.base_a);
-        pb = band_s_index(bins.base_b);
-    }
-    __device__ __forceinline__ void scan_store(const float (&pc)[8], const float (&pd)[8], float* w, int lane) const {
-        float* Pc = w + kBandPOffset;
-        float* Pd = Pc + kBandSStride;
-#pragma unroll
-        for (int q = 0; q < 4; ++q) {
-            Pc[pa + 72 * q] = pc[q];      Pd[pa + 72 * q] = pd[q];
-            Pc[pb + 72 * q] = pc[4 + q];  Pd[pb + 72 * q] = pd[4 + q];
+        const int p = lane & 15, row = (lane >> 4) * kBandPFrame;
+        pa = row + band_s_index(p);
+        pb = row + band_s_index(32 - (p ? p : 16));
+    }
+    __device__ __forceinline__ void scatter(const float (&pc)[16], const float (&pd)[16], float* w) const {
+#pragma unroll
+        for (int s = 0; s < 8; ++s) {
+            w[pa + 36 * s] = pc[s];      w[kBandSStride + pa + 36 * s] = pd[s];
+            w[pb + 36 * s] = pc[8 + s];  w[kBandSStride + pb + 36 * s] = pd[8 + s];
         }
         __syncwarp();
+    }
+    __device__ __forceinline__ void scan_store(float* w, int fr, int lane) const {
+        const float* Pc = w + fr * kBandPFrame;
+        const float* Pd = Pc + kBandSStride;
         const int mine = band_s_index(8 * lane);
         const float4 c0 = *reinterpret_cast<const float4*>(Pc + mine), c1 = *reinterpret_cast<const float4*>(Pc + mine + 4);
         const float4 d0 = *reinterpret_cast<const float4*>(Pd + mine), d1 = *reinterpret_cast<const float4*>(Pd + mine + 4);
diff --git a/fast_speech_enhancement_metrics_b200/csrc/fsem_lsd.cuh b/fast_speech_enhancement_metrics_b200/csrc/fsem_lsd.cuh
--- a/fast_speech_enhancement_metrics_b200/csrc/fsem_lsd.cuh
+++ b/fast_speech_enhancement_metrics_b200/csrc/fsem_lsd.cuh
@@ -33,28 +33,27 @@
     }
 }
 
-constexpr int kLsdWarps = 8;
+constexpr int kLsdWarps = 6;
+constexpr size_t kLsdDynSmem = sizeof(float) * kFftBufFloats * kLsdWarps;
 
 __device__ __forceinline__ float lsd_sqrt(float x) { float y; asm("sqrt.approx.ftz.f32 %0, %1;" : "=f"(y) : "f"(x)); return y; }
 __device__ __forceinline__ float lsd_rcp(float x) { float y; asm("rcp.approx.ftz.f32 %0, %1;" : "=f"(y) : "f"(x)); return y; }
 __device__ __forceinline__ float lsd_lg2(float x) { float y; asm("lg2.approx.ftz.f32 %0, %1;" : "=f"(y) : "f"(x)); return y; }
 
-template <bool kVec2>
 __global__ void __launch_bounds__(kLsdWarps * 32, 2)
 lsd_frames_kernel(const float* __restrict__ clean, const float* __restrict__ deg, const int32_t* __restrict__ lengths,
                   int64_t batch, int64_t n, int64_t stride, int tmax, const float* __restrict__ hann,
                   const float* __restrict__ alpha, float* __restrict__ frame_lsd ) {
-    __shared__ __align__(16) float2 s_buf[kLsdWarps][kFftBufElems];
+    extern __shared__ __align__(16) float s_lsd_buf[];
     const int lane = threadIdx.x & 31;
     const int warp = threadIdx.x >> 5;
-    float2* buf = s_buf[warp];
+    const int hw = lane >> 4;
+    float* buf = s_lsd_buf + warp * kFftBufFloats;
     FftTwiddles tw;
     tw.init(lane);
     float win[16];
 #pragma unroll
-    for (int h = 0; h < 2; ++h)
-#pragma unroll
-        for (int j = 0; j < 8; ++j) win[8 * h + j] = hann[fft_in_index(lane, h, j)];
+    for (int j = 0; j < 16; ++j) win[j] = hann[fft_in_index(lane, j)];
 
     const int64_t units = batch * (int64_t)tmax;
     const int64_t nwarps = (int64_t)gridDim.x * kLsdWarps;
@@ -64,61 +63,62 @@
     if (u0 >= u1) return;
     int64_t item = u0 / tmax;
     int f = (int)(u0 - item * tmax);
-    int len = item_length(lengths, item, n);
-    int T = lsd_num_frames(len);
-    for (int64_t u = u0; u < u1; ++u) {
-        if (f < T) {
-            const float* __restrict__ c = clean + item * stride;
-            const float* __restrict__ d = deg + item * stride;
-            const int first = f * 256 - 256;
-            float re[16], im[16];
-            if (kVec2 && first >= 0 && first + 512 <= len) {
-                const float2* __restrict__ pc2 = reinterpret_cast<const float2*>(c + first) + lane;
-                const float2* __restrict__ pd2 = reinterpret_cast<const float2*>(d + first) + lane;
+    for (int64_t u = u0; u < u1; u += 2) {
+        int64_t my_item = item;
+        int my_f = f + hw;
+        if (my_f == tmax) { my_f = 0; ++my_item; }
+        const bool mine = u + hw < u1;
+        const int len = mine ? item_length(lengths, my_item, n) : 0;
+        const bool valid = mine && my_f < lsd_num_frames(len);
+        if (__any_sync(kFull, valid)) {
+            const float* __restrict__ c = clean + my_item * stride + (lane & 15);
+            const float* __restrict__ d = deg + my_item * stride + (lane & 15);
+            const int first = my_f * 256 - 256;
+            float re[32], im[32];
+            if (valid && first >= 0 && first + 512 <= len) {
 #pragma unroll
-                for (int j = 0; j < 8; ++j) {
-                    const float2 cv = __ldg(pc2 + 32 * j), dv = __ldg(pd2 + 32 * j);
-                    re[j] = cv.x * win[j];  re[8 + j] = cv.y * win[8 + j];
-                    im[j] = dv.x * win[j];  im[8 + j] = dv.y * win[8 + j];
+                for (int j = 0; j < 16; ++j) {
+                    const float c0 = __ldg(c + first + 16 * j), d0 = __ldg(d + first + 16 * j);
+                    const float c1 = __ldg(c + first + 256 + 16 * j), d1 = __ldg(d + first + 256 + 16 * j);
+                    re[j] = c0 * win[j];                 im[j] = d0 * win[j];
+                    re[16 + j] = fmaf(-win[j], c1, c1);  im[16 + j] = fmaf(-win[j], d1, d1);
                 }
             } else {
 #pragma unroll
-                for (int h = 0; h < 2; ++h)
-#pragma unroll
-                    for (int j = 0; j < 8; ++j) {
-                        const int i = first + fft_in_index(lane, h, j);
-                        const bool ok = i >= 0 && i < len;
-                        re[8 * h + j] = ok ? __ldg(c + i) * win[8 * h + j] : 0.f;
-                        im[8 * h + j] = ok ? __ldg(d + i) * win[8 * h + j] : 0.f;
-                    }
+                for (int j = 0; j < 16; ++j) {
+                    const int i0 = first + 16 * j, i1 = i0 + 256;
+                    const int s0 = i0 + (lane & 15), s1 = i1 + (lane & 15);
+                    const bool ok0 = valid && s0 >= 0 && s0 < len, ok1 = valid && s1 >= 0 && s1 < len;
+                    const float c0 = ok0 ? __ldg(c + i0) : 0.f, d0 = ok0 ? __ldg(d + i0) : 0.f;
+                    const float c1 = ok1 ? __ldg(c + i1) : 0.f, d1 = ok1 ? __ldg(d + i1) : 0.f;
+                    re[j] = c0 * win[j];                 im[j] = d0 * win[j];
+                    re[16 + j] = fmaf(-win[j], c1, c1);  im[16 + j] = fmaf(-win[j], d1, d1);
+                }
             }
-            float ar[8], ai[8], br[8], bi[8];
-            warp_fft512<false>(re, im, buf, tw, lane, ar, ai, br, bi);
-            float pc[8], pd[8];
+            float ar[16], ai[16], br[16], bi[16];
+            fft512_half<false>(re, im, buf, tw, lane, ar, ai, br, bi);
+            float pc[16], pd[16];
             packed_power_regs(ar, ai, br, bi, lane, pc, pd);
-            const float a = fabsf(alpha[item]);
+            const float a = valid ? fabsf(alpha[my_item]) : 0.f;
             float acc = 0.f;
 #pragma unroll
-            for (int j = 0; j < 8; ++j) {
+            for (int j = 0; j < 16; ++j) {
                 const float den = fmaf(a, lsd_sqrt(pd[j] * kPackedPowerScale), kLsdEps);
                 const float l = lsd_lg2(fmaf(pc[j] * kPackedPowerScale, lsd_rcp(den * den), kLsdEps));
                 acc = fmaf(l, l, acc);
             }
-            if (lane == 0) {
-                const float den = fmaf(a, fabsf(ai[4]), kLsdEps);
-                const float l = lsd_lg2(fmaf(ar[4] * ar[4], lsd_rcp(den * den), kLsdEps));
+            if ((lane & 15) == 0) {
+                const float den = fmaf(a, fabsf(ai[8]), kLsdEps);
+                const float l = lsd_lg2(fmaf(ar[8] * ar[8], lsd_rcp(den * den), kLsdEps));
                 acc = fmaf(l, l, acc);
             }
-            acc = warp_sum(acc);
+#pragma unroll
+            for (int o = 8; o > 0; o >>= 1) acc += __shfl_xor_sync(kFull, acc, o);
             constexpr float kLn2Sq = 0.69314718056f * 0.69314718056f;
-            if (lane == 0) frame_lsd[item * tmax + f] = sqrtf(acc * (kLn2Sq / 257.f));
-            __syncwarp();
+            if ((lane & 15) == 0 && valid) frame_lsd[my_item * tmax + my_f] = sqrtf(acc * (kLn2Sq / 257.f));
         }
-        if (++f == tmax) {
-            f = 0;
-            ++item;
-            if (item < batch) { len = item_length(lengths, item, n); T = lsd_num_frames(len); }
-        }
+        f += 2;
+        while (f >= tmax) { f -= tmax; ++item; }
     }
 }
 
diff --git a/fast_speech_enhancement_metrics_b200/csrc/fsem_pesq.cuh b/fast_speech_enhancement_metrics_b200/csrc/fsem_pesq.cuh
--- a/fast_speech_enhancement_metrics_b200/csrc/fsem_pesq.cuh
+++ b/fast_speech_enhancement_metrics_b200/csrc/fsem_pesq.cuh
@@ -361,10 +361,10 @@
 }
 
 #ifndef FSEM_FFT_WARPS
-#define FSEM_FFT_WARPS 8
+#define FSEM_FFT_WARPS 4
 #endif
 #ifndef FSEM_FFT_MINBLOCKS
-#define FSEM_FFT_MINBLOCKS 2
+#define FSEM_FFT_MINBLOCKS 3
 #endif
 constexpr int kSpecWarps = FSEM_FFT_WARPS;
 
@@ -381,18 +381,34 @@
     return (float)(1.0e7 * ((double)len + 5120.0) * 1.04684 / power);
 }
 
+constexpr int kSpecSlot = FSEM_PESQ_HOP + 16;
 struct SpecWarpSmem {
-    float2 fft[kFftBufElems];
-    float half_c[3][FSEM_PESQ_HOP];
-    float half_d[3][FSEM_PESQ_HOP];
-    unsigned long long bar[3];
-    float gain[2];
+    float fft[kFftBufFloats];
+    float half_c[4 * kSpecSlot];
+    float half_d[4 * kSpecSlot];
+    unsigned long long bar[4];
 };
-static_assert(kBandBufFloats <= 2 * kFftBufElems, "band rows alias the FFT exchange buffer");
 constexpr int kBarkPiecesLow = 1;
 constexpr int kBarkPiecesHigh = 4;
 constexpr size_t kSpecDynSmem = sizeof(SpecWarpSmem) * kSpecWarps;
 static_assert(sizeof(SpecWarpSmem) % 16 == 0, "per-warp shared block must keep 16-byte alignment");
+static_assert((kSpecSlot * sizeof(float)) % 16 == 0 && kSpecSlot % 32 == 16, "ring slots: bulk-copy aligned, 16 banks apart");
+
+struct SpecFrame {
+    int64_t item;
+    int f, len, T, c;
+};
+__device__ __forceinline__ SpecFrame spec_next(SpecFrame a, const int32_t* __restrict__ lengths, int64_t batch, int64_t n) {
+    if (a.f + 1 < a.T) { ++a.f; ++a.c; return a; }
+    a.f = 0;
+    a.c += 2;
+    do {
+        ++a.item;
+        a.len = item_length(lengths, a.item, n);
+        a.T = pesq_num_frames(a.len);
+    } while (a.T == 0 && a.item + 1 < batch);
+    return a;
+}
 
 __global__ void __launch_bounds__(kSpecWarps * 32, FSEM_FFT_MINBLOCKS)
 pesq_spectrum_kernel(const float* __restrict__ z, int64_t zstride, const int32_t* __restrict__ lengths,
@@ -403,30 +419,27 @@
     extern __shared__ __align__(16) unsigned char s_raw[];
     const int lane = threadIdx.x & 31;
     const int warp = threadIdx.x >> 5;
+    const int hw = lane >> 4;
     SpecWarpSmem& sm = reinterpret_cast<SpecWarpSmem*>(s_raw)[warp];
-    float2* buf = sm.fft;
-    float* wbuf = reinterpret_cast<float*>(sm.fft);
+    float* wbuf = sm.fft;
     const float* S = wbuf + kBandSOffset;
     const uint32_t bar0 = smem_u32(&sm.bar[0]);
-    const uint32_t hc0 = smem_u32(&sm.half_c[0][0]), hd0 = smem_u32(&sm.half_d[0][0]);
+    const uint32_t hc0 = smem_u32(&sm.half_c[0]), hd0 = smem_u32(&sm.half_d[0]);
     constexpr uint32_t kHalfBytes = FSEM_PESQ_HOP * sizeof(float);
+    constexpr uint32_t kSlotBytes = kSpecSlot * sizeof(float);
     if (lane == 0) {
-        for (int i = 0; i < 3; ++i) mbar_init(bar0 + 8 * i, 1);
+        for (int i = 0; i < 4; ++i) mbar_init(bar0 + 8 * i, 1);
         mbar_fence_init();
     }
     __syncwarp();
 
     FftTwiddles tw;
     tw.init(lane);
-    float win[8];
-#pragma unroll
-    for (int h = 0; h < 2; ++h)
-#pragma unroll
-        for (int j = 0; j < 4; ++j) win[4 * h + j] = tab->hann[fft_in_index(lane, h, j)];
-    FftLaneBins bins;
-    bins.init(lane);
+    float win[16];
+#pragma unroll
+    for (int j = 0; j < 16; ++j) win[j] = tab->hann[fft_in_index(lane, j)];
     BandScan scan;
-    scan.init(tab->band_first, FSEM_PESQ_NBANDS, lane, bins);
+    scan.init(tab->band_first, FSEM_PESQ_NBANDS, lane);
     BandGather<kBarkPiecesLow> g_lo;
     BandGather<kBarkPiecesHigh> g_hi;
     g_lo.init(tab->band_first[lane], tab->band_first[lane] + tab->band_count[lane], true);
@@ -444,116 +457,120 @@
     const int64_t v0 = ((int64_t)blockIdx.x * kSpecWarps + warp) * per;
     int remaining = (int)(min(units, v0 + per) - v0);
     if (remaining <= 0) return;
-    int64_t item;
-    int f;
+    SpecFrame p0;
     if (frame_prefix) {
         int64_t lo = 0, hi = batch;
         while (hi - lo > 1) {
             const int64_t mid = (lo + hi) >> 1;
             if (frame_prefix[mid] <= v0) lo = mid; else hi = mid;
         }
-        item = lo;
-        f = (int)(v0 - frame_prefix[lo]);
+        p0.item = lo;
+        p0.f = (int)(v0 - frame_prefix[lo]);
     } else {
-        item = v0 / tmax;
-        f = (int)(v0 - item * tmax);
-    }
-    int len = item_length(lengths, item, n);
-    int T = pesq_num_frames(len);
-
-    unsigned par = 7u;
-    auto issue_half = [&](int slot, int64_t it, int h) {
-        par ^= 1u << slot;
+        p0.item = v0 / tmax;
+        p0.f = (int)(v0 - p0.item * tmax);
+    }
+    p0.len = item_length(lengths, p0.item, n);
+    p0.T = pesq_num_frames(p0.len);
+    p0.c = 0;
+
+    auto issue_half = [&](int c, int64_t it, int h) {
         if (lane == 0) {
+            const uint32_t slot = c & 3;
             fence_proxy_async();
             mbar_arrive_expect_tx(bar0 + 8 * slot, 2 * kHalfBytes);
-            bulk_copy_g2s(hc0 + slot * kHalfBytes, z + it * zstride + h * FSEM_PESQ_HOP, kHalfBytes, bar0 + 8 * slot);
-            bulk_copy_g2s(hd0 + slot * kHalfBytes, z + (batch + it) * zstride + h * FSEM_PESQ_HOP, kHalfBytes,
+            bulk_copy_g2s(hc0 + slot * kSlotBytes, z + it * zstride + h * FSEM_PESQ_HOP, kHalfBytes, bar0 + 8 * slot);
+            bulk_copy_g2s(hd0 + slot * kSlotBytes, z + (batch + it) * zstride + h * FSEM_PESQ_HOP, kHalfBytes,
                           bar0 + 8 * slot);
         }
     };
-    int sa = 0, sb = 1;
-    issue_half(0, item, f);
-    issue_half(1, item, f + 1);
-    auto set_gain = [&](int64_t it, int ln) {
-        const float gc = pesq_level_gain(pesq_band_power(partial, nchunks, batch, 0, it, lane), ln);
-        const float gd = pesq_level_gain(pesq_band_power(partial, nchunks, batch, 1, it, lane), ln);
-        if (lane == 0) { sm.gain[0] = gc; sm.gain[1] = gd; }
+    auto wait_half = [&](int c) { mbar_wait(bar0 + 8 * (c & 3), (c >> 2) & 1); };
+    auto issue_pair = [&](const SpecFrame& a, const SpecFrame& b, bool two, int resident) {
+        if (a.c > resident) issue_half(a.c, a.item, a.f);
+        issue_half(a.c + 1, a.item, a.f + 1);
+        if (two) {
+            if (b.c > a.c + 1) issue_half(b.c, b.item, b.f);
+            issue_half(b.c + 1, b.item, b.f + 1);
+        }
+    };
+    auto item_gain = [&](int64_t it, int ln) -> float2 {
+        return make_float2(pesq_level_gain(pesq_band_power(partial, nchunks, batch, 0, it, lane), ln),
+                           pesq_level_gain(pesq_band_power(partial, nchunks, batch, 1, it, lane), ln));
+    };
+
+    SpecFrame p1 = remaining > 1 ? spec_next(p0, lengths, batch, n) : p0;
+    issue_pair(p0, p1, remaining > 1, -1);
+    float2 g0 = item_gain(p0.item, p0.len);
+    float2 g1 = p1.item == p0.item ? g0 : item_gain(p1.item, p1.len);
+
+    while (true) {
+        const bool two = remaining > 1;
+        wait_half(p0.c);
+        wait_half(p0.c + 1);
+        if (two) {
+            if (p1.c > p0.c + 1) wait_half(p1.c);
+            wait_half(p1.c + 1);
+        }
+        const int fc = hw ? p1.c : p0.c;
+        const float* ac = sm.half_c + (fc & 3) * kSpecSlot + (lane & 15);
+        const float* ad = sm.half_d + (fc & 3) * kSpecSlot + (lane & 15);
+        const float* bc = sm.half_c + ((fc + 1) & 3) * kSpecSlot + (lane & 15);
+        const float* bd = sm.half_d + ((fc + 1) & 3) * kSpecSlot + (lane & 15);
+        float re[32], im[32];
+#pragma unroll
+        for (int j = 0; j < 16; ++j) {
+            const float c0 = ac[16 * j], d0 = ad[16 * j], c1 = bc[16 * j], d1 = bd[16 * j];
+            re[j] = c0 * win[j];                   im[j] = d0 * win[j];
+            re[16 + j] = fmaf(-win[j], c1, c1);    im[16 + j] = fmaf(-win[j], d1, d1);
+        }
+        {
+            const int f = hw ? p1.f : p0.f, len = hw ? p1.len : p0.len;
+            if (f * FSEM_PESQ_HOP + FSEM_PESQ_NFFT > len) {
+                const int room = len - f * FSEM_PESQ_HOP;
+#pragma unroll
+                for (int j = 0; j < 32; ++j)
+                    if (fft_in_index(lane, j) >= room) { re[j] = 0.f; im[j] = 0.f; }
+            }
+        }
         __syncwarp();
-    };
-    set_gain(item, len);
-
-    while (true) {
-        const int sn = 3 - sa - sb;
-        const bool has_next = remaining > 1;
-        const bool same_item = has_next && f + 1 < T;
-        int64_t item2 = item;
-        int len2 = len, T2 = T;
-        if (has_next && !same_item) {
-            do {
-                ++item2;
-                len2 = item_length(lengths, item2, n);
-                T2 = pesq_num_frames(len2);
-            } while (T2 == 0 && item2 + 1 < batch);
-        }
-        mbar_wait(bar0 + 8 * sa, (par >> sa) & 1u);
-        mbar_wait(bar0 + 8 * sb, (par >> sb) & 1u);
-        const float2* ac = reinterpret_cast<const float2*>(sm.half_c[sa]) + lane;
-        const float2* ad = reinterpret_cast<const float2*>(sm.half_d[sa]) + lane;
-        const float2* bc = reinterpret_cast<const float2*>(sm.half_c[sb]) + lane;
-        const float2* bd = reinterpret_cast<const float2*>(sm.half_d[sb]) + lane;
-        float re[16], im[16];
-#pragma unroll
-        for (int j = 0; j < 4; ++j) {
-            const float2 c0 = ac[32 * j], d0 = ad[32 * j], c1 = bc[32 * j], d1 = bd[32 * j];
-            re[j] = c0.x * win[j];                    re[8 + j] = c0.y * win[4 + j];
-            im[j] = d0.x * win[j];                    im[8 + j] = d0.y * win[4 + j];
-            re[4 + j] = fmaf(-win[j], c1.x, c1.x);    re[12 + j] = fmaf(-win[4 + j], c1.y, c1.y);
-            im[4 + j] = fmaf(-win[j], d1.x, d1.x);    im[12 + j] = fmaf(-win[4 + j], d1.y, d1.y);
-        }
-        if (f * FSEM_PESQ_HOP + FSEM_PESQ_NFFT > len) {
-            const int room = len - f * FSEM_PESQ_HOP;
-#pragma unroll
-            for (int h = 0; h < 2; ++h)
-#pragma unroll
-                for (int j = 0; j < 8; ++j)
-                    if (fft_in_index(lane, h, j) >= room) { re[8 * h + j] = 0.f; im[8 * h + j] = 0.f; }
-        }
-        __syncwarp();
-        if (has_next) {
-            if (same_item) issue_half(sn, item, f + 2);
-            else issue_half(sn, item2, 0);
-        }
-        float ar[8], ai[8], br[8], bi[8];
-        warp_fft512<false>(re, im, buf, tw, lane, ar, ai, br, bi);
-        float pc[8], pd[8];
-        packed_power_regs(ar, ai, br, bi, lane, pc, pd);
-        if (lane == 0) { pc[0] = 0.f; pd[0] = 0.f; }
-        scan.scan_store(pc, pd, wbuf, lane);
-        float* __restrict__ out_c = bark + (item * tpitch + f) * kBarkRow;
-        float* __restrict__ out_d = bark + ((batch + item) * tpitch + f) * kBarkRow;
-        const float lo_c = g_lo.sum(S), lo_d = g_lo.sum(S + kBandSStride);
-        const float hi_c = g_hi.sum(S), hi_d = g_hi.sum(S + kBandSStride);
-        const float2 g2 = *reinterpret_cast<const float2*>(sm.gain);
-        out_c[lane] = (lo_c * scale0) * g2.x;
-        out_d[lane] = (lo_d * scale0) * g2.y;
-        if (lane + 32 < FSEM_PESQ_NBANDS) {
-            out_c[lane + 32] = (hi_c * scale1) * g2.x;
-            out_d[lane + 32] = (hi_d * scale1) * g2.y;
-        }
-        if (!has_next) break;
-        --remaining;
-        if (same_item) {
-            sa = sb; sb = sn;
-            ++f;
-        } else {
-            item = item2; f = 0; len = len2; T = T2;
-            const int freed = sa;
-            sa = sn; sb = freed;
+        const int left = remaining - (two ? 2 : 1);
+        SpecFrame n0 = p1, n1 = p1;
+        if (left > 0) {
+            n0 = spec_next(p1, lengths, batch, n);
+            n1 = left > 1 ? spec_next(n0, lengths, batch, n) : n0;
+            issue_pair(n0, n1, left > 1, p1.c + 1);
+        }
+        float ar[16], ai[16], br[16], bi[16];
+        fft512_half<false>(re, im, wbuf, tw, lane, ar, ai, br, bi);
+        {
+            float pc[16], pd[16];
+            packed_power_regs(ar, ai, br, bi, lane, pc, pd);
+            if ((lane & 15) == 0) { pc[0] = 0.f; pd[0] = 0.f; }
+            scan.scatter(pc, pd, wbuf);
+        }
+#pragma unroll 1
+        for (int fr = 0; fr < (two ? 2 : 1); ++fr) {
+            const SpecFrame& q = fr ? p1 : p0;
+            const float2 g2 = fr ? g1 : g0;
+            scan.scan_store(wbuf, fr, lane);
+            float* __restrict__ out_c = bark + (q.item * tpitch + q.f) * kBarkRow;
+            float* __restrict__ out_d = bark + ((batch + q.item) * tpitch + q.f) * kBarkRow;
+            const float lo_c = g_lo.sum(S), lo_d = g_lo.sum(S + kBandSStride);
+            const float hi_c = g_hi.sum(S), hi_d = g_hi.sum(S + kBandSStride);
+            out_c[lane] = (lo_c * scale0) * g2.x;
+            out_d[lane] = (lo_d * scale0) * g2.y;
+            if (lane + 32 < FSEM_PESQ_NBANDS) {
+                out_c[lane + 32] = (hi_c * scale1) * g2.x;
+                out_d[lane + 32] = (hi_d * scale1) * g2.y;
+            }
             __syncwarp();
-            issue_half(sb, item, f + 1);
-            set_gain(item, len);
-        }
+        }
+        if (left <= 0) break;
+        remaining = left;
+        g0 = n0.item == p1.item ? g1 : item_gain(n0.item, n0.len);
+        g1 = n1.item == n0.item ? g0 : item_gain(n1.item, n1.len);
+        p0 = n0;
+        p1 = n1;
     }
 }
 
diff --git a/fast_speech_enhancement_metrics_b200/csrc/fsem_stoi.cuh b/fast_speech_enhancement_metrics_b200/csrc/fsem_stoi.cuh
--- a/fast_speech_enhancement_metrics_b200/csrc/fsem_stoi.cuh
+++ b/fast_speech_enhancement_metrics_b200/csrc/fsem_stoi.cuh
@@ -377,28 +377,27 @@
 }
 
 #ifndef FSEM_FFT_WARPS
-#define FSEM_FFT_WARPS 8
+#define FSEM_FFT_WARPS 4
 #endif
 #ifndef FSEM_FFT_MINBLOCKS
-#define FSEM_FFT_MINBLOCKS 2
+#define FSEM_FFT_MINBLOCKS 3
 #endif
 constexpr int kTobWarps = FSEM_FFT_WARPS;
+constexpr size_t kTobDynSmem = sizeof(float) * kFftBufFloats * kTobWarps;
 
 constexpr int kTobPieces = 6;
-static_assert(kBandBufFloats <= 2 * kFftBufElems, "band rows alias the FFT exchange buffer");
-
-template <bool kVec2>
+
 __global__ void __launch_bounds__(kTobWarps * 32, FSEM_FFT_MINBLOCKS)
 stoi_tob_kernel(const float* __restrict__ clean10k, const float* __restrict__ deg10k, int64_t sstride,
                 int64_t batch, int t0max, int umax,
                 int ustride, const int32_t* __restrict__ kept_idx, const int32_t* __restrict__ frame_prefix,
                 const StoiTables* __restrict__ tab, float* __restrict__ tob ) {
-    __shared__ __align__(16) float2 s_buf[kTobWarps][kFftBufElems];
+    extern __shared__ __align__(16) float s_tob_buf[];
     __shared__ int32_t s_starts[FSEM_STOI_NBANDS + 2];
     const int lane = threadIdx.x & 31;
     const int warp = threadIdx.x >> 5;
-    float2* buf = s_buf[warp];
-    float* wbuf = reinterpret_cast<float*>(buf);
+    const int hw = lane >> 4;
+    float* wbuf = s_tob_buf + warp * kFftBufFloats;
     if (threadIdx.x == 0) s_starts[0] = 0;
     if (threadIdx.x < FSEM_STOI_NBANDS) s_starts[1 + threadIdx.x] = tab->band_lo[threadIdx.x];
     if (threadIdx.x == FSEM_STOI_NBANDS) s_starts[FSEM_STOI_NBANDS + 1] = tab->band_hi[FSEM_STOI_NBANDS - 1];
@@ -406,20 +405,16 @@
 
     FftTwiddles tw;
     tw.init(lane);
-    float win[8];
-#pragma unroll
-    for (int h = 0; h < 2; ++h)
-#pragma unroll
-        for (int j = 0; j < 4; ++j) win[4 * h + j] = tab->window[fft_in_index(lane, h, j)];
-    FftLaneBins bins;
-    bins.init(lane);
+    float win[16];
+#pragma unroll
+    for (int j = 0; j < 16; ++j) win[j] = tab->window[fft_in_index(lane, j)];
     BandScan scan;
-    scan.init(s_starts, FSEM_STOI_NBANDS + 2, lane, bins);
+    scan.init(s_starts, FSEM_STOI_NBANDS + 2, lane);
     const int my_band = lane & 15;
     const bool has_band = my_band < FSEM_STOI_NBANDS;
     BandGather<kTobPieces> gather;
     gather.init(s_starts[1 + (has_band ? my_band : 0)], s_starts[2 + (has_band ? my_band : 0)], has_band);
-    const float* Srow = wbuf + kBandSOffset + (lane >> 4) * kBandSStride;
+    const float* Srow = wbuf + kBandSOffset + hw * kBandSStride;
 
     const int64_t total = frame_prefix[batch];
     const int64_t nwarps = (int64_t)gridDim.x * kTobWarps;
@@ -432,52 +427,57 @@
         const int64_t mid = (lo_i + hi_i) >> 1;
         if (frame_prefix[mid] <= w0) lo_i = mid; else hi_i = mid;
     }
-    int64_t item = lo_i;
-    int item_end = frame_prefix[item + 1];
-    int u = (int)(w0 - frame_prefix[item]);
-    for (int64_t w = w0; w < w1; ++w, ++u) {
-        while (w >= item_end) { ++item; item_end = frame_prefix[item + 1]; u = 0; }
+    int64_t item0 = lo_i;
+    int start0 = frame_prefix[item0], end0 = frame_prefix[item0 + 1];
+    for (int64_t w = w0; w < w1; w += 2) {
+        while (w >= end0) { ++item0; start0 = end0; end0 = frame_prefix[item0 + 1]; }
+        const bool two = w + 1 < w1;
+        int64_t item1 = item0;
+        int start1 = start0, end1 = end0;
+        if (two) while (w + 1 >= end1) { ++item1; start1 = end1; end1 = frame_prefix[item1 + 1]; }
+        const int u0 = (int)(w - start0), u1 = two ? (int)(w + 1 - start1) : u0;
         {
+            const int64_t item = hw ? item1 : item0;
+            const int u = hw ? u1 : u0;
             const int32_t* idx = kept_idx + item * t0max + u;
             const int ta = idx[0] * FSEM_STOI_HOP, tb = idx[1] * FSEM_STOI_HOP, tc = idx[2] * FSEM_STOI_HOP;
-            if (w + 1 < item_end && lane < 16) {
-                const float* p = ((lane & 8) ? deg10k : clean10k) + item * sstride + idx[3] * FSEM_STOI_HOP + 32 * (lane & 7);
+            if ((int64_t)(hw ? w + 1 : w) + 2 < (hw ? end1 : end0)) {
+                const float* p = ((lane & 8) ? deg10k : clean10k) + item * sstride + idx[4] * FSEM_STOI_HOP + 32 * (lane & 7);
                 asm volatile("prefetch.global.L1 [%0];" ::"l"(p));
             }
-            const float* __restrict__ xc = clean10k + item * sstride + 2 * lane;
-            const float* __restrict__ xd = deg10k + item * sstride + 2 * lane;
-            auto pair = [&](const float* p) -> float2 {
-                if (kVec2) return __ldg(reinterpret_cast<const float2*>(p));
-                return make_float2(__ldg(p), __ldg(p + 1));
-            };
-            float re[16], im[16];
-#pragma unroll
-            for (int j = 0; j < 4; ++j) {
-                const int q = 64 * j;
-                const int nb = (j < 2) ? (ta + q + 128) : (tc + q - 128);
-                const int jn = (j < 2) ? j + 2 : j - 2;
-                const float2 c0 = pair(xc + tb + q), c1 = pair(xc + nb);
-                const float2 d0 = pair(xd + tb + q), d1 = pair(xd + nb);
-                const float w0f = win[j], w1f = win[4 + j], n0f = win[jn], n1f = win[4 + jn];
-                re[j] = __fmul_rn(w0f, __fadd_rn(__fmul_rn(w0f, c0.x), __fmul_rn(n0f, c1.x)));
-                re[8 + j] = __fmul_rn(w1f, __fadd_rn(__fmul_rn(w1f, c0.y), __fmul_rn(n1f, c1.y)));
-                im[j] = __fmul_rn(w0f, __fadd_rn(__fmul_rn(w0f, d0.x), __fmul_rn(n0f, d1.x)));
-                im[8 + j] = __fmul_rn(w1f, __fadd_rn(__fmul_rn(w1f, d0.y), __fmul_rn(n1f, d1.y)));
-            }
-#pragma unroll
-            for (int j = 4; j < 8; ++j) { re[j] = 0.f; im[j] = 0.f; re[8 + j] = 0.f; im[8 + j] = 0.f; }
-            float ar[8], ai[8], br[8], bi[8];
-            warp_fft512<true>(re, im, buf, tw, lane, ar, ai, br, bi);
-            float pc[8], pd[8];
+            const float* __restrict__ xc = clean10k + item * sstride + (lane & 15);
+            const float* __restrict__ xd = deg10k + item * sstride + (lane & 15);
+            float re[32], im[32];
+#pragma unroll
+            for (int j = 0; j < 16; ++j) {
+                const int q = 16 * j;
+                const int nb = (j < 8) ? (ta + q + 128) : (tc + q - 128);
+                const float c0 = __ldg(xc + tb + q), c1 = __ldg(xc + nb);
+                const float d0 = __ldg(xd + tb + q), d1 = __ldg(xd + nb);
+                const float wf = win[j], nf = win[j ^ 8];
+                re[j] = __fmul_rn(wf, __fadd_rn(__fmul_rn(wf, c0), __fmul_rn(nf, c1)));
+                im[j] = __fmul_rn(wf, __fadd_rn(__fmul_rn(wf, d0), __fmul_rn(nf, d1)));
+            }
+#pragma unroll
+            for (int j = 16; j < 32; ++j) { re[j] = 0.f; im[j] = 0.f; }
+            float ar[16], ai[16], br[16], bi[16];
+            fft512_half<true>(re, im, wbuf, tw, lane, ar, ai, br, bi);
+            float pc[16], pd[16];
             packed_power_regs(ar, ai, br, bi, lane, pc, pd);
-            scan.scan_store(pc, pd, wbuf, lane);
+            scan.scatter(pc, pd, wbuf);
+        }
+#pragma unroll 1
+        for (int fr = 0; fr < (two ? 2 : 1); ++fr) {
+            scan.scan_store(wbuf, fr, lane);
             const float band = gather.sum(Srow);
             if (has_band) {
-                const int64_t sig = (lane >> 4) ? (batch + item) : item;
-                tob[(sig * FSEM_STOI_NBANDS + my_band) * (int64_t)ustride + u] = 0.5f * sqrtf(band);
+                const int64_t item = fr ? item1 : item0;
+                const int64_t sig = hw ? (batch + item) : item;
+                tob[(sig * FSEM_STOI_NBANDS + my_band) * (int64_t)ustride + (fr ? u1 : u0)] = 0.5f * sqrtf(band);
             }
             __syncwarp();
         }
+        item0 = item1; start0 = start1; end0 = end1;
     }
 }
 
```
